# argumentcomputer/multi-stark

Hardware: AMD Instinct MI355X
Metric: prove_trace_rows_per_sec (higher is better)
Workload: dtype u64; 1 GPU; U32-add + byte-table lookup (benches/multi_stark.rs), 2^20 additions per proof, bench_config(): log_blowup 2, 100 queries, 10+10 PoW bits, GoldilocksBlake3Config; witness (traces + claims, 64-bit words) in pinned host memory at step start: upload, from_stage_1 on the device and read-back inside the timed region; the library narrows byte-valued traces on host threads INSIDE the step before they cro; rows_per_proof=1048832, proof_bytes=1100053, parallelism=single GPU

## Files before the change

bindings/rust/mstark_sys.rs:

```rust
#![allow(non_camel_case_types, dead_code)]

use std::os::raw::{c_char, c_void};

#[repr(C)] pub struct ms_ctx { _p: [u8; 0] }
#[repr(C)] pub struct ms_system { _p: [u8; 0] }
#[repr(C)] pub struct ms_witness { _p: [u8; 0] }
#[repr(C)] pub struct ms_mmcs { _p: [u8; 0] }
#[repr(C)] pub struct ms_challenger { _p: [u8; 0] }
#[repr(C)] pub struct ms_comm_rccl { _p: [u8; 0] }
#[repr(C)] pub struct ms_comm_local_group { _p: [u8; 0] }
#[repr(C)] pub struct ms_comm_local { _p: [u8; 0] }
#[repr(C)] pub struct ms_trace { _p: [u8; 0] }
#[repr(C)] pub struct msbb_system { _p: [u8; 0] }
#[repr(C)] pub struct msbb_witness { _p: [u8; 0] }
#[repr(C)] pub struct msbb_mmcs { _p: [u8; 0] }
#[repr(C)] pub struct msbb_challenger { _p: [u8; 0] }
#[repr(C)] pub struct msbb_trace { _p: [u8; 0] }

pub const MS_OK: i32 = 0;
pub const MS_ERR: i32 = -1;
pub const MS_ERR_NO_DEVICE: i32 = -2;
pub const MS_ERR_BUFFER: i32 = -3;
pub const MS_VERDICT_ACCEPT: i32 = 0;
pub const MS_VERDICT_INVALID_OPENING: i32 = 2;
pub const MS_VERDICT_INVALID_SHAPE: i32 = 3;
pub const MS_VERDICT_INVALID_SYSTEM: i32 = 4;
pub const MS_VERDICT_OOD_MISMATCH: i32 = 5;
pub const MS_VERDICT_UNBALANCED: i32 = 6;
pub const MS_CHECK_CONSTRAINT: u32 = 0x1;
pub const MS_CHECK_LOOKUPS: u32 = 0x2;
pub const MS_CHECK_CIRCUIT_WORDS: usize = 10;
pub const MS_LB_ENTRY_WORDS: usize = 8;
pub const MS_LB_CLAIMS: u64 = !0;
pub const MSBB_CHECK_CIRCUIT_WORDS: usize = 12;

#[repr(C)]
#[derive(Clone, Copy)]
pub struct ms_dev_matrix {
    pub ptr: *const c_void,
    pub height: u64,
    pub elem_bytes: u32,
    pub row_stride: i64,
    pub col_stride: i64,
}

#[repr(C)]
pub struct ms_comm {
    pub size: u32,
    pub rank: i32,
    pub world: i32,
    pub user: *mut c_void,
    pub all_to_all: Option<unsafe extern "C" fn(user: *mut c_void, send_dev: *const c_void, recv_dev: *mut c_void, bytes_per_peer: usize) -> i32>,
    pub all_gather: Option<unsafe extern "C" fn(user: *mut c_void, send_dev: *const c_void, recv_dev: *mut c_void, bytes: usize) -> i32>,
    pub all_to_all_start: Option<unsafe extern "C" fn(user: *mut c_void, send_dev: *const c_void, send_stride: usize, recv_dev: *mut c_void,
                                                      recv_stride: usize, bytes_per_peer: usize) -> i32>,
    pub all_to_all_wait: Option<unsafe extern "C" fn(user: *mut c_void) -> i32>,
    pub all_to_all_cols_start: Option<unsafe extern "C" fn(user: *mut c_void, send_dev: *const c_void, send_peer_stride: usize, send_col_stride: usize,
                                                           recv_dev: *mut c_void, recv_peer_stride: usize, recv_col_stride: usize, ncols: usize,
                                                           seg_bytes: usize) -> i32>,
    pub set_stream_ordered: Option<unsafe extern "C" fn(user: *mut c_void, hip_stream: *mut c_void) -> i32>,
    pub all_to_all_cols_start2: Option<unsafe extern "C" fn(user: *mut c_void, send_dev: *const c_void, send_peer_stride: usize, send_col_stride: usize,
                                                            recv_dev: *mut c_void, recv_peer_stride: usize, recv_col_stride: usize, ncols: usize,
                                                            seg_bytes: usize, flags: u32) -> i32>,
    pub scatter_cols_start: Option<unsafe extern "C" fn(user: *mut c_void, root: i32, send_dev: *const c_void, send_peer_stride: usize,
                                                        send_col_stride: usize, recv_dev: *mut c_void, recv_col_stride: usize, ncols: usize,
                                                        seg_bytes: usize) -> i32>,
    pub abort: Option<unsafe extern "C" fn(user: *mut c_void, why: *const c_char)>,
}
pub const MS_COMM_SKIP_SELF: u32 = 1;
pub const MS_KERNEL_QUOTIENT: u32 = 0x1;
pub const MS_KERNEL_QUOTIENT_INLINE: u32 = 0x2;
pub const MS_KERNEL_STAGE2: u32 = 0x4;
pub const MS_KERNEL_STAGE2_GROUPED: u32 = 0x8;
pub const MS_KERNEL_STAGE2_TRACE: u32 = 0x10;
pub const MS_KERNEL_STAGE2_GROUPS_SHIFT: u32 = 8;
pub const MS_KERNEL_STAGE2_GROUPS_MASK: u32 = 0x1f;

extern "C" {
    pub fn ms_last_error() -> *const c_char;
    pub fn ms_device_count() -> i32;
    pub fn ms_ctx_create(device: i32, out: *mut *mut ms_ctx) -> i32;
    pub fn ms_ctx_destroy(ctx: *mut ms_ctx);
    pub fn ms_ctx_sync(ctx: *mut ms_ctx) -> i32;
    pub fn ms_ctx_sync_count(ctx: *mut ms_ctx, out: *mut u64) -> i32;
    pub fn ms_ctx_trim(ctx: *mut ms_ctx) -> i32;
    pub fn ms_ctx_set_profile_mask(ctx: *mut ms_ctx, mask: u32) -> i32;
    pub fn ms_ctx_kernel_stats(ctx: *mut ms_ctx, kernel_id: i32, launches: *mut u64, ms: *mut f64, alg_bytes: *mut f64) -> i32;
    pub fn ms_ctx_reset_stats(ctx: *mut ms_ctx) -> i32;
    pub fn ms_ctx_kernel_units(ctx: *mut ms_ctx, kernel_id: i32, units: *mut f64) -> i32;
    pub fn ms_ctx_debug_fail_alloc(ctx: *mut ms_ctx, nth: i32) -> i32;
    pub fn ms_kernel_count() -> i32;
    pub fn ms_kernel_name(kernel_id: i32) -> *const c_char;
    pub fn ms_system_create(ctx: *mut ms_ctx, blob: *const u8, len: usize, out: *mut *mut ms_system) -> i32;
    pub fn ms_system_destroy(sys: *mut ms_system);
    pub fn ms_system_preprocessed_commit(sys: *const ms_system, out: *mut u8, cap: usize, n_digests: *mut usize) -> i32;
    pub fn ms_system_circuit_info(sys: *const ms_system, circuit: usize, out9: *mut u64) -> i32;
    pub fn ms_system_circuit_kernels(sys: *const ms_system, circuit: usize, flags: *mut u32) -> i32;
    pub fn ms_witness_create(sys: *mut ms_system, traces: *const *const u64, heights: *const u64, mult: *const *const u64,
                             args: *const *const u64, n_claims: usize, claim_offsets: *const u64, claim_data: *const u64,
                             out: *mut *mut ms_witness) -> i32;
    pub fn ms_witness_create_host(sys: *mut ms_system, traces: *const *const u64, heights: *const u64, n_claims: usize,
                                  claim_offsets: *const u64, claim_data: *const u64, pinned: *mut i32,
                                  out: *mut *mut ms_witness) -> i32;
    pub fn ms_claims_slice_range(sys: *mut ms_system, heights: *const u64, n_claims: usize, claim_offsets: *const u64, rank: i32, world: i32,
                                 first_elem: *mut u64, n_elems: *mut u64) -> i32;
    pub fn ms_witness_create_host_sliced(sys: *mut ms_system, traces: *const *const u64, heights: *const u64, n_claims: usize,
                                         claim_offsets: *const u64, data_first: u64, data_count: u64, data_slice: *const u64,
                                         head: *const u64, n_head: usize, pinned: *mut i32, out: *mut *mut ms_witness) -> i32;
    pub fn ms_witness_prefetch(w: *mut ms_witness, on: i32) -> i32;
    pub fn ms_witness_create_device(sys: *mut ms_system, traces: *const ms_dev_matrix, n_claims: usize, claim_offsets: *const u64,
                                    claim_data: *const u64, claims_on_device: i32, producer_stream: *mut c_void,
                                    out: *mut *mut ms_witness) -> i32;
    pub fn ms_witness_u32_add_bench(sys: *mut ms_system, num_adds: usize, a0: u32, b0: u32, out: *mut *mut ms_witness) -> i32;
    pub fn ms_witness_blake3_compressions(sys: *mut ms_system, n: usize, states_in: *const u32, states_out: *mut u32,
                                          out: *mut *mut ms_witness) -> i32;
    pub fn ms_blake3_compressions(data: *const u8, len: usize, states_in: *mut u32, cap_rows: usize, n: *mut usize, digest32: *mut u8) -> i32;
    pub fn ms_witness_trace(w: *mut ms_witness, circuit: usize, out: *mut u64, cap_words: usize, n_words: *mut usize) -> i32;
    pub fn ms_witness_destroy(w: *mut ms_witness);
    pub fn ms_prove(sys: *mut ms_system, w: *mut ms_witness, proof_out: *mut u8, cap: usize, proof_len: *mut usize, stage_ms: *mut f64) -> i32;
    pub fn ms_verify(sys: *mut ms_system, n_claims: usize, claim_offsets: *const u64, claim_data: *const u64, proof: *const u8,
                     proof_len: usize, verdict: *mut i32) -> i32;
    pub fn ms_verify_batch(sys: *mut ms_system, n_proofs: usize, n_claims: *const u64, claim_offsets: *const *const u64,
                           claim_data: *const *const u64, proofs: *const *const u8, proof_lens: *const u64, verdicts: *mut i32) -> i32;
    pub fn ms_prove_sharded(sys: *mut ms_system, w: *mut ms_witness, comm: *const ms_comm, owners: *const i32, proof_out: *mut u8,
                            cap: usize, proof_len: *mut usize, stage_ms: *mut f64) -> i32;
    pub fn ms_ctx_comm_progress(ctx: *mut ms_ctx, out: *mut c_char, cap: usize, seq: *mut u64, in_flight: *mut i32) -> i32;
    pub fn ms_comm_rccl_unique_id(out: *mut u8) -> i32;
    pub fn ms_comm_rccl_create(ctx: *mut ms_ctx, unique_id: *const u8, rank: i32, world: i32, out: *mut *mut ms_comm_rccl) -> i32;
    pub fn ms_comm_rccl_table(c: *mut ms_comm_rccl) -> *const ms_comm;
    pub fn ms_comm_rccl_bytes_moved(c: *mut ms_comm_rccl) -> u64;
    pub fn ms_comm_rccl_destroy(c: *mut ms_comm_rccl);
    pub fn ms_comm_local_group_create(world: i32, out: *mut *mut ms_comm_local_group) -> i32;
    pub fn ms_comm_local_group_abort(g: *mut ms_comm_local_group);
    pub fn ms_comm_local_group_destroy(g: *mut ms_comm_local_group);
    pub fn ms_comm_local_create(g: *mut ms_comm_local_group, ctx: *mut ms_ctx, rank: i32, out: *mut *mut ms_comm_local) -> i32;
    pub fn ms_comm_local_table(c: *mut ms_comm_local) -> *const ms_comm;
    pub fn ms_comm_local_bytes_moved(c: *mut ms_comm_local) -> u64;
    pub fn ms_comm_local_destroy(c: *mut ms_comm_local);
    pub fn ms_dft_batch(ctx: *mut ms_ctx, input: *const u64, h: usize, w: usize, inverse: i32, out: *mut u64) -> i32;
    pub fn ms_coset_lde_batch(ctx: *mut ms_ctx, input: *const u64, h: usize, w: usize, log_blowup: u32, out: *mut u64) -> i32;
    pub fn ms_quotient_lde(ctx: *mut ms_ctx, input: *const u64, log_n: u32, log_q: u32, log_blowup: u32, d: usize, out: *mut u64) -> i32;
    pub fn ms_mmcs_commit(ctx: *mut ms_ctx, n: usize, mats: *const *const u64, heights: *const u64, widths: *const u64, cap_height: u32,
                          cap_out: *mut u8, out: *mut *mut ms_mmcs) -> i32;
    pub fn ms_mmcs_open(m: *mut ms_mmcs, index: usize, vals_out: *mut u64, proof_out: *mut u8, n_siblings: *mut usize) -> i32;
    pub fn ms_mmcs_verify_batch(ctx: *mut ms_ctx, n_mats: usize, heights: *const u64, widths: *const u64, cap: *const u8, cap_height: u32,
                                n_openings: usize, indices: *const u64, vals: *const u64, siblings: *const u8, ok_out: *mut u8) -> i32;
    pub fn ms_mmcs_destroy(m: *mut ms_mmcs);
    pub fn ms_blake3(ctx: *mut ms_ctx, bytes: *const u8, len: usize, out32: *mut u8) -> i32;
    pub fn ms_challenger_create(params7: *const u64, out: *mut *mut ms_challenger) -> i32;
    pub fn ms_challenger_destroy(ch: *mut ms_challenger);
    pub fn ms_challenger_observe(ch: *mut ms_challenger, elems: *const u64, n: usize) -> i32;
    pub fn ms_challenger_observe_digests(ch: *mut ms_challenger, digests: *const u8, n: usize) -> i32;
    pub fn ms_challenger_sample_ext(ch: *mut ms_challenger, out2: *mut u64) -> i32;
    pub fn ms_challenger_sample_bits(ch: *mut ms_challenger, bits: u32, out: *mut u64) -> i32;
    pub fn ms_pcs_commit(ctx: *mut ms_ctx, log_blowup: u32, cap_height: u32, n: usize, evals: *const *const u64, heights: *const u64,
                         widths: *const u64, cap_out: *mut u8, out: *mut *mut ms_mmcs) -> i32;
    pub fn ms_pcs_open(ctx: *mut ms_ctx, params7: *const u64, n_rounds: usize, rounds: *const *mut ms_mmcs, n_points: *const u64,
                       points: *const u64, ch: *mut ms_challenger, opened_out: *mut u64, opened_cap_words: usize, fri_out: *mut u8,
                       fri_cap: usize, fri_len: *mut usize) -> i32;
    pub fn ms_pcs_verify(params7: *const u64, n_rounds: usize, caps: *const *const u8, cap_sizes: *const u64, n_mats: *const u64,
                         log_n: *const u64, widths: *const u64, n_points: *const u64, points: *const u64, opened: *const u64,
                         fri: *const u8, fri_len: usize, ch: *mut ms_challenger, accepted: *mut i32) -> i32;
    pub fn ms_trace_destroy(t: *mut ms_trace);
    pub fn ms_trace_info(t: *const ms_trace, out3: *mut u64) -> i32;
    pub fn ms_system_preprocessed_mmcs(sys: *mut ms_system, out: *mut *mut ms_mmcs) -> i32;
    pub fn ms_witness_commit_stage1(w: *mut ms_witness, cap_out: *mut u8, out: *mut *mut ms_mmcs) -> i32;
    pub fn ms_challenger_observe_claims(ch: *mut ms_challenger, w: *mut ms_witness) -> i32;
    pub fn ms_witness_check(w: *mut ms_witness, beta: *const u64, gamma: *const u64, verdict: *mut u32, circuits: *mut u64,
                            root_counts: *mut u64, root_first: *mut u64, roots_cap: usize) -> i32;
    pub fn ms_system_check_info(sys: *const ms_system, circuit: usize, out4: *mut u64) -> i32;
    pub fn ms_witness_lookup_balance(w: *mut ms_witness, summary: *mut u64, entries: *mut u64, entries_cap: usize, args_out: *mut u64,
                                     args_cap: usize, slot_counts: *mut u64, slots_cap: usize) -> i32;
    pub fn ms_witness_claims_accumulator(w: *mut ms_witness, beta: *const u64, gamma: *const u64, acc_out: *mut u64) -> i32;
    pub fn ms_stage2_build(w: *mut ms_witness, beta: *const u64, gamma: *const u64, acc_in: *const u64, accs_out: *mut u64,
                           traces_out: *mut *mut ms_trace) -> i32;
    pub fn ms_pcs_commit_traces(ctx: *mut ms_ctx, log_blowup: u32, cap_height: u32, n: usize, evals: *const *mut ms_trace,
                                cap_out: *mut u8, out: *mut *mut ms_mmcs) -> i32;
    pub fn ms_quotient(sys: *mut ms_system, circuit: usize, log_n: u32, s1: *mut ms_mmcs, s1_idx: usize, s2: *mut ms_mmcs,
                       s2_idx: usize, publics8: *const u64, alpha: *const u64, q_lde_out: *mut *mut ms_trace) -> i32;
    pub fn ms_pcs_commit_ldes(ctx: *mut ms_ctx, cap_height: u32, n: usize, ldes: *const *mut ms_trace, cap_out: *mut u8,
                              out: *mut *mut ms_mmcs) -> i32;
    pub fn ms_stage2_trace(ctx: *mut ms_ctx, height: usize, num_lookups: usize, mult: *const u64, arg_offsets: *const u64,
                           args: *const u64, beta: *const u64, gamma: *const u64, acc_in: *const u64, trace_out: *mut u64,
                           acc_out: *mut u64) -> i32;
    pub fn ms_claims_accumulator(ctx: *mut ms_ctx, n_claims: usize, claim_offsets: *const u64, claim_data: *const u64, beta: *const u64,
                                 gamma: *const u64, acc_out: *mut u64) -> i32;
    pub fn ms_quotient_values(sys: *mut ms_system, circuit: usize, publics8: *const u64, log_n: u32, log_q: u32, pre_q: *const u64,
                              s1_q: *const u64, s2_q: *const u64, alpha: *const u64, out: *mut u64) -> i32;
    pub fn ms_field_op(ctx: *mut ms_ctx, op: i32, a: *const u64, b: *const u64, n: usize, out: *mut u64) -> i32;

    pub fn msbb_system_create(ctx: *mut ms_ctx, blob: *const u8, len: usize, out: *mut *mut msbb_system) -> i32;
    pub fn msbb_system_destroy(sys: *mut msbb_system);
    pub fn msbb_system_preprocessed_commit(sys: *const msbb_system, out: *mut u32, cap_words: usize, n_digests: *mut usize) -> i32;
    pub fn msbb_system_circuit_info(sys: *const msbb_system, circuit: usize, out9: *mut u64) -> i32;
    pub fn msbb_system_circuit_kernels(sys: *const msbb_system, circuit: usize, flags: *mut u32) -> i32;
    pub fn msbb_witness_create(sys: *mut msbb_system, traces: *const *const u32, heights: *const u64, n_claims: usize,
                               claim_offsets: *const u64, claim_data: *const u32, out: *mut *mut msbb_witness) -> i32;
    pub fn msbb_witness_create_host(sys: *mut msbb_system, traces: *const *const u32, heights: *const u64, n_claims: usize,
                                    claim_offsets: *const u64, claim_data: *const u32, pinned: *mut i32, out: *mut *mut msbb_witness) -> i32;
    pub fn msbb_witness_create_device(sys: *mut msbb_system, traces: *const ms_dev_matrix, n_claims: usize, claim_offsets: *const u64,
                                      claim_data: *const u32, producer_stream: *mut c_void, out: *mut *mut msbb_witness) -> i32;
    pub fn msbb_witness_destroy(w: *mut msbb_witness);
    pub fn msbb_witness_check(w: *mut msbb_witness, beta: *const u32, gamma: *const u32, verdict: *mut u32, circuits: *mut u64,
                              root_counts: *mut u64, root_first: *mut u64, roots_cap: usize) -> i32;
    pub fn msbb_system_check_info(sys: *const msbb_system, circuit: usize, out4: *mut u64) -> i32;
    pub fn msbb_prove(sys: *mut msbb_system, w: *mut msbb_witness, proof_out: *mut u8, cap: usize, proof_len: *mut usize,
                      stage_ms: *mut f64) -> i32;
    pub fn msbb_verify(sys: *mut msbb_system, n_claims: usize, claim_offsets: *const u64, claim_data: *const u32, proof: *const u8,
                       proof_len: usize, verdict: *mut i32) -> i32;
    pub fn msbb_verify_batch(sys: *mut msbb_system, n_proofs: usize, n_claims: *const u64, claim_offsets: *const *const u64,
                             claim_data: *const *const u32, proofs: *const *const u8, proof_lens: *const u64, verdicts: *mut i32) -> i32;
    pub fn msbb_set_poseidon2(ctx: *mut ms_ctx, constants141: *const u32) -> i32;
    pub fn msbb_poseidon2_permute(ctx: *mut ms_ctx, states: *mut u32, n: usize) -> i32;
    pub fn msbb_dft_batch(ctx: *mut ms_ctx, input: *const u32, h: usize, w: usize, inverse: i32, out: *mut u32) -> i32;
    pub fn msbb_coset_lde_batch(ctx: *mut ms_ctx, input: *const u32, h: usize, w: usize, log_blowup: u32, out: *mut u32) -> i32;
    pub fn msbb_mmcs_commit(ctx: *mut ms_ctx, n: usize, mats: *const *const u32, heights: *const u64, widths: *const u64,
                            cap_height: u32, cap_out: *mut u32, out: *mut *mut msbb_mmcs) -> i32;
    pub fn msbb_mmcs_open(m: *mut msbb_mmcs, index: usize, vals_out: *mut u32, proof_out: *mut u32, n_siblings: *mut usize) -> i32;
    pub fn msbb_mmcs_verify_batch(ctx: *mut ms_ctx, n_mats: usize, heights: *const u64, widths: *const u64, cap: *const u32, cap_height: u32,
                                  n_openings: usize, indices: *const u64, vals: *const u32, siblings: *const u32, ok_out: *mut u8) -> i32;
    pub fn msbb_mmcs_destroy(m: *mut msbb_mmcs);
    pub fn msbb_field_op(ctx: *mut ms_ctx, op: i32, a: *const u32, b: *const u32, n: usize, out: *mut u32) -> i32;
    pub fn msbb_challenger_create(sys: *mut msbb_system, out: *mut *mut msbb_challenger) -> i32;
    pub fn msbb_challenger_destroy(ch: *mut msbb_challenger);
    pub fn msbb_challenger_observe(ch: *mut msbb_challenger, elems: *const u32, n: usize) -> i32;
    pub fn msbb_challenger_observe_digests(ch: *mut msbb_challenger, digests: *const u32, n: usize) -> i32;
    pub fn msbb_challenger_sample_ext(ch: *mut msbb_challenger, out4: *mut u32) -> i32;
    pub fn msbb_challenger_sample_bits(ch: *mut msbb_challenger, bits: u32, out: *mut u64) -> i32;
    pub fn msbb_challenger_observe_claims(ch: *mut msbb_challenger, w: *mut msbb_witness) -> i32;
    pub fn msbb_trace_destroy(t: *mut msbb_trace);
    pub fn msbb_trace_info(t: *const msbb_trace, out3: *mut u64) -> i32;
    pub fn msbb_system_preprocessed_mmcs(sys: *mut msbb_system, out: *mut *mut msbb_mmcs) -> i32;
    pub fn msbb_witness_commit_stage1(w: *mut msbb_witness, cap_out: *mut u32, out: *mut *mut msbb_mmcs) -> i32;
    pub fn msbb_witness_claims_accumulator(w: *mut msbb_witness, beta: *const u32, gamma: *const u32, acc_out: *mut u32) -> i32;
    pub fn msbb_stage2_build(w: *mut msbb_witness, beta: *const u32, gamma: *const u32, acc_in: *const u32, accs_out: *mut u32,
                             traces_out: *mut *mut msbb_trace) -> i32;
    pub fn msbb_pcs_commit_traces(sys: *mut msbb_system, n: usize, evals: *const *mut msbb_trace, cap_out: *mut u32, out: *mut *mut msbb_mmcs) -> i32;
    pub fn msbb_quotient(sys: *mut msbb_system, circuit: usize, log_n: u32, s1: *mut msbb_mmcs, s1_idx: usize, s2: *mut msbb_mmcs, s2_idx: usize,
                         publics16: *const u32, alpha: *const u32, q_lde_out: *mut *mut msbb_trace) -> i32;
    pub fn msbb_pcs_commit_ldes(sys: *mut msbb_system, n: usize, ldes: *const *mut msbb_trace, cap_out: *mut u32, out: *mut *mut msbb_mmcs) -> i32;
    pub fn msbb_pcs_open(sys: *mut msbb_system, n_rounds: usize, rounds: *const *mut msbb_mmcs, n_points: *const u64, points: *const u32,
                         ch: *mut msbb_challenger, opened_out: *mut u32, opened_cap_words: usize, fri_out: *mut u8, fri_cap: usize,
                         fri_len: *mut usize) -> i32;
}
```

include/mstark.h:

```cpp
#ifndef MSTARK_H
#define MSTARK_H

#include <stddef.h>
#include <stdint.h>

#ifdef __cplusplus
extern "C" {
#endif

typedef struct ms_ctx ms_ctx;
typedef struct ms_system ms_system;
typedef struct ms_witness ms_witness;
typedef struct ms_mmcs ms_mmcs;

enum {
  MS_OK = 0,
  MS_ERR = -1,
  MS_ERR_NO_DEVICE = -2,
  MS_ERR_BUFFER = -3
};

const char* ms_last_error(void);

int32_t ms_device_count(void);
int32_t ms_ctx_create(int32_t device, ms_ctx** out);
void ms_ctx_destroy(ms_ctx* ctx);
int32_t ms_ctx_sync(ms_ctx* ctx);
int32_t ms_ctx_sync_count(ms_ctx* ctx, uint64_t* out);
int32_t ms_ctx_trim(ms_ctx* ctx);
int32_t ms_ctx_set_profile_mask(ms_ctx* ctx, uint32_t mask);
int32_t ms_ctx_kernel_stats(ms_ctx* ctx, int32_t kernel_id, uint64_t* launches, double* ms, double* alg_bytes);
int32_t ms_ctx_kernel_units(ms_ctx* ctx, int32_t kernel_id, double* units);
int32_t ms_ctx_reset_stats(ms_ctx* ctx);
int32_t ms_ctx_debug_fail_alloc(ms_ctx* ctx, int32_t nth);
int32_t ms_kernel_count(void);
const char* ms_kernel_name(int32_t kernel_id);

int32_t ms_system_create(ms_ctx* ctx, const uint8_t* blob, size_t len, ms_system** out);
void ms_system_destroy(ms_system* sys);
int32_t ms_system_preprocessed_commit(const ms_system* sys, uint8_t* out, size_t cap, size_t* n_digests);
int32_t ms_system_circuit_info(const ms_system* sys, size_t circuit, uint64_t out9[9]);
#define MS_KERNEL_QUOTIENT 0x1u
#define MS_KERNEL_QUOTIENT_INLINE 0x2u
#define MS_KERNEL_STAGE2 0x4u
#define MS_KERNEL_STAGE2_GROUPED 0x8u
#define MS_KERNEL_STAGE2_TRACE 0x10u
#define MS_KERNEL_STAGE2_GROUPS_SHIFT 8
#define MS_KERNEL_STAGE2_GROUPS_MASK 0x1fu
int32_t ms_system_circuit_kernels(const ms_system* sys, size_t circuit, uint32_t* flags);

int32_t ms_witness_create(ms_system* sys, const uint64_t* const* traces, const uint64_t* heights,
                          const uint64_t* const* mult, const uint64_t* const* args, size_t n_claims,
                          const uint64_t* claim_offsets, const uint64_t* claim_data, ms_witness** out);
int32_t ms_witness_create_host(ms_system* sys, const uint64_t* const* traces, const uint64_t* heights, size_t n_claims,
                               const uint64_t* claim_offsets, const uint64_t* claim_data, int32_t* pinned ,
                               ms_witness** out);
int32_t ms_witness_prefetch(ms_witness* w, int32_t on);
typedef struct ms_dev_matrix {
  const void* ptr;
  uint64_t height;
  uint32_t elem_bytes;
  int64_t row_stride, col_stride;
} ms_dev_matrix;
int32_t ms_witness_create_device(ms_system* sys, const ms_dev_matrix* traces , size_t n_claims,
                                 const uint64_t* claim_offsets, const uint64_t* claim_data, int32_t claims_on_device,
                                 void* producer_stream , ms_witness** out);
int32_t ms_witness_u32_add_bench(ms_system* sys, size_t num_adds, uint32_t a0, uint32_t b0, ms_witness** out);
int32_t ms_witness_blake3_compressions(ms_system* sys, size_t n, const uint32_t* states_in, uint32_t* states_out, ms_witness** out);
int32_t ms_blake3_compressions(const uint8_t* data, size_t len, uint32_t* states_in, size_t cap_rows, size_t* n, uint8_t* digest32);
int32_t ms_witness_trace(ms_witness* w, size_t circuit, uint64_t* out, size_t cap_words, size_t* n_words);
void ms_witness_destroy(ms_witness* w);

#define MS_CHECK_CONSTRAINT 0x1u
#define MS_CHECK_LOOKUPS 0x2u
#define MS_CHECK_CIRCUIT_WORDS 10
int32_t ms_witness_check(ms_witness* w, const uint64_t beta[2], const uint64_t gamma[2], uint32_t* verdict,
                         uint64_t* circuits , uint64_t* root_counts ,
                         uint64_t* root_first , size_t roots_cap);
int32_t ms_system_check_info(const ms_system* sys, size_t circuit, uint64_t out4[4]);

#define MS_LB_ENTRY_WORDS 8
#define MS_LB_CLAIMS (~(uint64_t)0)
int32_t ms_witness_lookup_balance(ms_witness* w, uint64_t summary[4], uint64_t* entries, size_t entries_cap ,
                                  uint64_t* args_out, size_t args_cap , uint64_t* slot_counts ,
                                  size_t slots_cap);

int32_t ms_prove(ms_system* sys, ms_witness* w, uint8_t* proof_out, size_t cap, size_t* proof_len, double* stage_ms);

#define MS_VERDICT_ACCEPT 0
#define MS_VERDICT_INVALID_OPENING 2
#define MS_VERDICT_INVALID_SHAPE 3
#define MS_VERDICT_INVALID_SYSTEM 4
#define MS_VERDICT_OOD_MISMATCH 5
#define MS_VERDICT_UNBALANCED 6
int32_t ms_verify(ms_system* sys, size_t n_claims, const uint64_t* claim_offsets, const uint64_t* claim_data,
                  const uint8_t* proof, size_t proof_len, int32_t* verdict);
int32_t ms_verify_batch(ms_system* sys, size_t n_proofs, const uint64_t* n_claims, const uint64_t* const* claim_offsets,
                        const uint64_t* const* claim_data, const uint8_t* const* proofs, const uint64_t* proof_lens,
                        int32_t* verdicts);

typedef struct ms_comm {
  uint32_t size;
  int32_t rank, world;
  void* user;
  int32_t (*all_to_all)(void* user, const void* send_dev, void* recv_dev, size_t bytes_per_peer);
  int32_t (*all_gather)(void* user, const void* send_dev, void* recv_dev, size_t bytes);
  int32_t (*all_to_all_start)(void* user, const void* send_dev, size_t send_stride, void* recv_dev, size_t recv_stride,
                              size_t bytes_per_peer);
  int32_t (*all_to_all_wait)(void* user);
  int32_t (*all_to_all_cols_start)(void* user, const void* send_dev, size_t send_peer_stride, size_t send_col_stride, void* recv_dev,
                                   size_t recv_peer_stride, size_t recv_col_stride, size_t ncols, size_t seg_bytes);
  int32_t (*set_stream_ordered)(void* user, void* hip_stream);
  int32_t (*all_to_all_cols_start2)(void* user, const void* send_dev, size_t send_peer_stride, size_t send_col_stride, void* recv_dev,
                                    size_t recv_peer_stride, size_t recv_col_stride, size_t ncols, size_t seg_bytes, uint32_t flags);
  int32_t (*scatter_cols_start)(void* user, int32_t root, const void* send_dev, size_t send_peer_stride, size_t send_col_stride,
                                void* recv_dev, size_t recv_col_stride, size_t ncols, size_t seg_bytes);
  void (*abort)(void* user, const char* why);
} ms_comm;
#define MS_COMM_SKIP_SELF 1u
int32_t ms_prove_sharded(ms_system* sys, ms_witness* w, const ms_comm* comm, const int32_t* owners, uint8_t* proof_out, size_t cap,
                         size_t* proof_len, double* stage_ms);
int32_t ms_claims_slice_range(ms_system* sys, const uint64_t* heights, size_t n_claims, const uint64_t* claim_offsets, int32_t rank,
                              int32_t world, uint64_t* first_elem, uint64_t* n_elems);
int32_t ms_witness_create_host_sliced(ms_system* sys, const uint64_t* const* traces, const uint64_t* heights, size_t n_claims,
                                      const uint64_t* claim_offsets, uint64_t data_first, uint64_t data_count,
                                      const uint64_t* data_slice, const uint64_t* head, size_t n_head, int32_t* pinned,
                                      ms_witness** out);

int32_t ms_ctx_comm_progress(ms_ctx* ctx, char* out, size_t cap, uint64_t* seq, int32_t* in_flight);

#define MS_RCCL_UNIQUE_ID_BYTES 128
typedef struct ms_comm_rccl ms_comm_rccl;
int32_t ms_comm_rccl_unique_id(uint8_t out[MS_RCCL_UNIQUE_ID_BYTES]);
int32_t ms_comm_rccl_create(ms_ctx* ctx, const uint8_t unique_id[MS_RCCL_UNIQUE_ID_BYTES], int32_t rank, int32_t world,
                            ms_comm_rccl** out);
const ms_comm* ms_comm_rccl_table(ms_comm_rccl* c);
uint64_t ms_comm_rccl_bytes_moved(ms_comm_rccl* c);
void ms_comm_rccl_destroy(ms_comm_rccl* c);

typedef struct ms_comm_local_group ms_comm_local_group;
typedef struct ms_comm_local ms_comm_local;
int32_t ms_comm_local_group_create(int32_t world, ms_comm_local_group** out);
void ms_comm_local_group_abort(ms_comm_local_group* g);
void ms_comm_local_group_destroy(ms_comm_local_group* g);
int32_t ms_comm_local_create(ms_comm_local_group* g, ms_ctx* ctx, int32_t rank, ms_comm_local** out);
const ms_comm* ms_comm_local_table(ms_comm_local* c);
uint64_t ms_comm_local_bytes_moved(ms_comm_local* c);
void ms_comm_local_destroy(ms_comm_local* c);

int32_t ms_dft_batch(ms_ctx* ctx, const uint64_t* in, size_t h, size_t w, int32_t inverse, uint64_t* out);
int32_t ms_coset_lde_batch(ms_ctx* ctx, const uint64_t* in, size_t h, size_t w, uint32_t log_blowup, uint64_t* out);
int32_t ms_quotient_lde(ms_ctx* ctx, const uint64_t* in, uint32_t log_n, uint32_t log_q, uint32_t log_blowup, size_t D,
                        uint64_t* out);
int32_t ms_mmcs_commit(ms_ctx* ctx, size_t n, const uint64_t* const* mats, const uint64_t* heights,
                       const uint64_t* widths, uint32_t cap_height, uint8_t* cap_out, ms_mmcs** out);
int32_t ms_mmcs_open(ms_mmcs* m, size_t index, uint64_t* vals_out, uint8_t* proof_out, size_t* n_siblings);
void ms_mmcs_destroy(ms_mmcs* m);
int32_t ms_mmcs_verify_batch(ms_ctx* ctx, size_t n_mats, const uint64_t* heights, const uint64_t* widths, const uint8_t* cap,
                             uint32_t cap_height, size_t n_openings, const uint64_t* indices, const uint64_t* vals,
                             const uint8_t* siblings, uint8_t* ok_out);
int32_t ms_blake3(ms_ctx* ctx, const uint8_t* bytes, size_t len, uint8_t out32[32]);

typedef struct ms_challenger ms_challenger;
int32_t ms_challenger_create(const uint64_t params7[7], ms_challenger** out);
void ms_challenger_destroy(ms_challenger* ch);
int32_t ms_challenger_observe(ms_challenger* ch, const uint64_t* elems, size_t n);
int32_t ms_challenger_observe_digests(ms_challenger* ch, const uint8_t* digests, size_t n);
int32_t ms_challenger_sample_ext(ms_challenger* ch, uint64_t out2[2]);
int32_t ms_challenger_sample_bits(ms_challenger* ch, uint32_t bits, uint64_t* out);
int32_t ms_pcs_commit(ms_ctx* ctx, uint32_t log_blowup, uint32_t cap_height, size_t n, const uint64_t* const* evals,
                      const uint64_t* heights, const uint64_t* widths, uint8_t* cap_out, ms_mmcs** out);
int32_t ms_pcs_open(ms_ctx* ctx, const uint64_t params7[7], size_t n_rounds, ms_mmcs* const* rounds, const uint64_t* n_points,
                    const uint64_t* points, ms_challenger* ch, uint64_t* opened_out, size_t opened_cap_words, uint8_t* fri_out,
                    size_t fri_cap, size_t* fri_len);
int32_t ms_pcs_verify(const uint64_t params7[7], size_t n_rounds, const uint8_t* const* caps, const uint64_t* cap_sizes,
                      const uint64_t* n_mats, const uint64_t* log_n, const uint64_t* widths, const uint64_t* n_points,
                      const uint64_t* points, const uint64_t* opened, const uint8_t* fri, size_t fri_len, ms_challenger* ch,
                      int32_t* accepted);

typedef struct ms_trace ms_trace;
void ms_trace_destroy(ms_trace* t);
int32_t ms_trace_info(const ms_trace* t, uint64_t out3[3]);
int32_t ms_system_preprocessed_mmcs(ms_system* sys, ms_mmcs** out);
int32_t ms_witness_commit_stage1(ms_witness* w, uint8_t* cap_out, ms_mmcs** out);
int32_t ms_challenger_observe_claims(ms_challenger* ch, ms_witness* w);
int32_t ms_witness_claims_accumulator(ms_witness* w, const uint64_t beta[2], const uint64_t gamma[2], uint64_t acc_out[2]);
int32_t ms_stage2_build(ms_witness* w, const uint64_t beta[2], const uint64_t gamma[2], const uint64_t acc_in[2], uint64_t* accs_out,
                        ms_trace** traces_out);
int32_t ms_pcs_commit_traces(ms_ctx* ctx, uint32_t log_blowup, uint32_t cap_height, size_t n, ms_trace* const* evals, uint8_t* cap_out,
                             ms_mmcs** out);
int32_t ms_quotient(ms_system* sys, size_t circuit, uint32_t log_n, ms_mmcs* s1, size_t s1_idx, ms_mmcs* s2, size_t s2_idx,
                    const uint64_t publics8[8], const uint64_t alpha[2], ms_trace** q_lde_out);
int32_t ms_pcs_commit_ldes(ms_ctx* ctx, uint32_t cap_height, size_t n, ms_trace* const* ldes, uint8_t* cap_out, ms_mmcs** out);

int32_t ms_stage2_trace(ms_ctx* ctx, size_t height, size_t num_lookups, const uint64_t* mult,
                        const uint64_t* arg_offsets, const uint64_t* args, const uint64_t beta[2],
                        const uint64_t gamma[2], const uint64_t acc_in[2], uint64_t* trace_out, uint64_t acc_out[2]);
int32_t ms_claims_accumulator(ms_ctx* ctx, size_t n_claims, const uint64_t* claim_offsets, const uint64_t* claim_data,
                              const uint64_t beta[2], const uint64_t gamma[2], uint64_t acc_out[2]);
int32_t ms_quotient_values(ms_system* sys, size_t circuit, const uint64_t publics8[8], uint32_t log_n, uint32_t log_q,
                           const uint64_t* pre_q, const uint64_t* s1_q, const uint64_t* s2_q, const uint64_t alpha[2],
                           uint64_t* out);
int32_t ms_field_op(ms_ctx* ctx, int32_t op, const uint64_t* a, const uint64_t* b, size_t n, uint64_t* out);

#ifdef __cplusplus
}
#endif
#endif
```

multi-stark_amd/__init__.py:

```python
import ctypes as C
import os

import numpy as np

from . import frontend
from . import babybear
from .frontend import Params, bench_params, test_params, compile_circuit, system_blob, pack_claims

HERE = os.path.dirname(os.path.abspath(__file__))
LIB_PATH = os.path.join(HERE, "libmstark_hip.so")

u64p = C.POINTER(C.c_uint64)
u8p = C.POINTER(C.c_uint8)
_lib = None


class MstarkError(RuntimeError):
    pass


def lib():
    global _lib
    if _lib is None:
        if not os.path.exists(LIB_PATH):
            raise MstarkError("libmstark_hip.so is missing: run `python multi-stark_amd/build.py` (needs hipcc)")
        L = C.CDLL(LIB_PATH)
        L.ms_last_error.restype = C.c_char_p
        L.ms_kernel_name.restype = C.c_char_p
        _lib = L
    return _lib


def exported_symbols():
    return ["ms_last_error", "ms_device_count", "ms_ctx_create", "ms_ctx_destroy", "ms_ctx_sync", "ms_ctx_sync_count", "ms_ctx_trim", "ms_ctx_set_profile_mask",
            "ms_ctx_kernel_stats", "ms_ctx_kernel_units", "ms_ctx_reset_stats", "ms_ctx_debug_fail_alloc", "ms_kernel_count", "ms_kernel_name", "ms_system_create",
            "ms_system_destroy", "ms_system_preprocessed_commit", "ms_system_circuit_info", "ms_system_circuit_kernels", "ms_witness_create", "ms_witness_create_host", "ms_claims_slice_range", "ms_witness_create_host_sliced", "ms_witness_prefetch",
            "ms_witness_create_device", "ms_witness_u32_add_bench", "ms_witness_blake3_compressions", "ms_blake3_compressions", "ms_witness_trace", "ms_witness_destroy", "ms_prove", "ms_prove_sharded", "ms_ctx_comm_progress", "ms_comm_rccl_unique_id", "ms_comm_rccl_create",
            "ms_comm_rccl_table", "ms_comm_rccl_bytes_moved", "ms_comm_rccl_destroy", "ms_comm_local_group_create", "ms_comm_local_group_abort",
            "ms_comm_local_group_destroy", "ms_comm_local_create", "ms_comm_local_table", "ms_comm_local_bytes_moved", "ms_comm_local_destroy", "ms_verify", "ms_verify_batch", "ms_dft_batch", "ms_coset_lde_batch", "ms_quotient_lde", "ms_mmcs_commit",
            "ms_mmcs_open", "ms_mmcs_destroy", "ms_mmcs_verify_batch", "ms_blake3", "ms_pcs_commit", "ms_pcs_open", "ms_pcs_verify", "ms_challenger_create",
            "ms_challenger_destroy", "ms_challenger_observe", "ms_challenger_observe_digests", "ms_challenger_sample_ext",
            "ms_challenger_sample_bits", "ms_stage2_trace", "ms_claims_accumulator",
            "ms_quotient_values", "ms_field_op", "ms_trace_destroy", "ms_trace_info", "ms_system_preprocessed_mmcs",
            "ms_witness_commit_stage1", "ms_challenger_observe_claims", "ms_witness_claims_accumulator", "ms_stage2_build",
            "ms_pcs_commit_traces", "ms_quotient", "ms_pcs_commit_ldes", "ms_witness_check", "ms_system_check_info", "ms_witness_lookup_balance"]


KERNEL_QUOTIENT, KERNEL_QUOTIENT_INLINE, KERNEL_STAGE2, KERNEL_STAGE2_GROUPED, KERNEL_STAGE2_TRACE = 0x1, 0x2, 0x4, 0x8, 0x10


def kernel_groups(flags):
    return (flags >> 8) & 0x1F


def _check(rc):
    if rc != 0:
        raise MstarkError(lib().ms_last_error().decode() or ("mstark error %d" % rc))


def _p(a):
    return a.ctypes.data_as(u64p)


def _b(a):
    return a.ctypes.data_as(u8p)


def _u64(a):
    return np.ascontiguousarray(a, dtype=np.uint64)


class DevMatrix(C.Structure):
    _fields_ = [("ptr", C.c_void_p), ("height", C.c_uint64), ("elem_bytes", C.c_uint32), ("row_stride", C.c_int64), ("col_stride", C.c_int64)]


def _is_torch(obj):
    return type(obj).__module__.split(".")[0] == "torch" and hasattr(obj, "data_ptr")


def _device_array(obj, what):
    if _is_torch(obj):
        if not obj.is_cuda:
            raise MstarkError("%s: a CPU tensor has no device pointer (use System.witness)" % what)
        return int(obj.data_ptr()), tuple(int(x) for x in obj.shape), tuple(int(x) for x in obj.stride()), int(obj.element_size()), True
    cai = getattr(obj, "__cuda_array_interface__", None)
    if cai is None:
        raise MstarkError("%s: %s has no device pointer (expected a torch tensor on the GPU or __cuda_array_interface__)" % (what, type(obj).__name__))
    shape = tuple(int(x) for x in cai["shape"])
    item = np.dtype(cai["typestr"]).itemsize
    strides = cai.get("strides")
    if strides is None:
        strides, acc = [], item
        for n in reversed(shape):
            strides.insert(0, acc)
            acc *= max(n, 1)
    if any(int(b) % item for b in strides):
        raise MstarkError("%s: strides are not whole elements" % what)
    return int(cai["data"][0] or 0), shape, tuple(int(b) // item for b in strides), item, False


def _device_traces(traces, n_circuits, widths_of):
    if len(traces) != n_circuits:
        raise MstarkError("expected one trace per circuit")
    desc, seen_torch = [], None
    for i, t in enumerate(traces):
        what = "trace of circuit %d" % i
        if t is None or (not _is_torch(t) and not hasattr(t, "__cuda_array_interface__") and hasattr(t, "__len__") and len(t) == 0):
            desc.append(None)
            continue
        ptr, shape, strides, item, is_torch = _device_array(t, what)
        if len(shape) != 2:
            raise MstarkError("%s: expected a 2-D matrix, got %d dimension(s)" % (what, len(shape)))
        if is_torch and seen_torch is None:
            seen_torch = t
        desc.append((ptr, shape, strides, item))
    arr = (DevMatrix * max(n_circuits, 1))()
    heights = []
    for i, d in enumerate(desc):
        if d is None or d[1][0] == 0:
            arr[i] = DevMatrix(None, 0, 1, 1, 1)
            heights.append(0)
            continue
        ptr, (h, w), (rs, cs), item = d
        width = widths_of(i)
        if w != width:
            raise MstarkError("trace of circuit %d: width %d, the circuit's main_width is %d" % (i, w, width))
        arr[i] = DevMatrix(ptr or None, h, item, rs if h > 1 else max(w, 1), cs if w > 1 else 1)
        heights.append(h)
    return arr, heights, seen_torch


def _producer_stream(stream, torch_tensor):
    if stream is None:
        if torch_tensor is None:
            return None
        import torch

        stream = torch.cuda.current_stream(torch_tensor.device)
    handle = int(getattr(stream, "cuda_stream", stream))
    return C.c_void_p(handle) if handle else None


def device_count() -> int:
    return int(lib().ms_device_count())


class Context:

    def __init__(self, device=0):
        self.h = C.c_void_p()
        rc = lib().ms_ctx_create(C.c_int32(device), C.byref(self.h))
        if rc != 0:
            raise MstarkError("cannot create a HIP context: " + lib().ms_last_error().decode())

    def close(self):
        if getattr(self, "h", None):
            lib().ms_ctx_destroy(self.h)
            self.h = None

    def __del__(self):
        try:
            self.close()
        except Exception:
            pass

    def sync(self):
        _check(lib().ms_ctx_sync(self.h))

    def sync_count(self):
        n = C.c_uint64()
        _check(lib().ms_ctx_sync_count(self.h, C.byref(n)))
        return int(n.value)

    def trim(self):
        _check(lib().ms_ctx_trim(self.h))

    def comm_progress(self):
        buf = C.create_string_buffer(256)
        seq, fl = C.c_uint64(), C.c_int32()
        _check(lib().ms_ctx_comm_progress(self.h, buf, C.c_size_t(256), C.byref(seq), C.byref(fl)))
        return buf.value.decode(), int(seq.value), bool(fl.value)

    def debug_fail_alloc(self, nth):
        _check(lib().ms_ctx_debug_fail_alloc(self.h, C.c_int32(nth)))

    def kernel_names(self):
        return [lib().ms_kernel_name(C.c_int32(i)).decode() for i in range(lib().ms_kernel_count())]

    def set_profile(self, names):
        all_names = self.kernel_names()
        mask = 0
        for n in names:
            mask |= 1 << all_names.index(n)
        _check(lib().ms_ctx_set_profile_mask(self.h, C.c_uint32(mask)))

    def reset_stats(self):
        _check(lib().ms_ctx_reset_stats(self.h))

    def kernel_stats(self):
        out = {}
        for i, n in enumerate(self.kernel_names()):
            launches, ms, byts = C.c_uint64(), C.c_double(), C.c_double()
            _check(lib().ms_ctx_kernel_stats(self.h, C.c_int32(i), C.byref(launches), C.byref(ms), C.byref(byts)))
            units = C.c_double()
            _check(lib().ms_ctx_kernel_units(self.h, C.c_int32(i), C.byref(units)))
            out[n] = {"launches": launches.value, "ms": ms.value, "alg_bytes": byts.value, "units": units.value}
        return out

    def dft_batch(self, m, inverse=False):
        m = _u64(m)
        out = np.empty_like(m)
        _check(lib().ms_dft_batch(self.h, _p(m), C.c_size_t(m.shape[0]), C.c_size_t(m.shape[1]), C.c_int32(int(inverse)), _p(out)))
        return out

    def coset_lde_batch(self, m, log_blowup):
        m = _u64(m)
        out = np.empty((m.shape[0] << log_blowup, m.shape[1]), dtype=np.uint64)
        _check(lib().ms_coset_lde_batch(self.h, _p(m), C.c_size_t(m.shape[0]), C.c_size_t(m.shape[1]), C.c_uint32(log_blowup), _p(out)))
        return out

    def quotient_lde(self, q, log_n, log_q, log_blowup):
        q = _u64(q)
        D = q.shape[1]
        out = np.empty((1 << (log_n + log_blowup), D << log_q), dtype=np.uint64)
        _check(lib().ms_quotient_lde(self.h, _p(q), C.c_uint32(log_n), C.c_uint32(log_q), C.c_uint32(log_blowup), C.c_size_t(D), _p(out)))
        return out

    def blake3(self, data: bytes) -> bytes:
        buf = np.frombuffer(data, dtype=np.uint8) if data else np.zeros(1, dtype=np.uint8)
        out = np.zeros(32, dtype=np.uint8)
        _check(lib().ms_blake3(self.h, _b(buf), C.c_size_t(len(data)), _b(out)))
        return out.tobytes()

    def stage2_trace(self, mult, arg_offsets, args, beta, gamma, acc_in):
        mult, args, arg_offsets = _u64(mult), _u64(args), _u64(arg_offsets)
        h, L = mult.shape
        tr = np.zeros((h, max(L, 1) * 2), dtype=np.uint64)
        acc = np.zeros(2, dtype=np.uint64)
        _check(lib().ms_stage2_trace(self.h, C.c_size_t(h), C.c_size_t(L), _p(mult), _p(arg_offsets), _p(args), _p(_u64(beta)),
                                     _p(_u64(gamma)), _p(_u64(acc_in)), _p(tr), _p(acc)))
        return tr, (int(acc[0]), int(acc[1]))

    def claims_accumulator(self, claims_packed, beta, gamma):
        offs, data = claims_packed
        data = data if data.size else np.zeros(1, dtype=np.uint64)
        acc = np.zeros(2, dtype=np.uint64)
        _check(lib().ms_claims_accumulator(self.h, C.c_size_t(len(offs) - 1), _p(offs), _p(data), _p(_u64(beta)), _p(_u64(gamma)), _p(acc)))
        return int(acc[0]), int(acc[1])

    def field_op(self, op, a, b=None):
        a = _u64(a)
        bb = _u64(b) if b is not None else None
        out = np.empty_like(a)
        n = a.size // 2 if op >= 4 else a.size
        _check(lib().ms_field_op(self.h, C.c_int32(op), _p(a), _p(bb) if bb is not None else None, C.c_size_t(n), _p(out)))
        return out


class Mmcs:

    def __init__(self, ctx, mats, cap_height=0):
        self.ctx = ctx
        self.mats = [_u64(m) for m in mats]
        n = len(self.mats)
        ptrs = (u64p * n)(*[_p(m) for m in self.mats])
        hs = _u64([m.shape[0] for m in self.mats])
        ws = _u64([m.shape[1] for m in self.mats])
        maxh = int(hs.max())
        cap = np.zeros(32 * min(1 << cap_height, maxh), dtype=np.uint8)
        self.h = C.c_void_p()
        _check(lib().ms_mmcs_commit(ctx.h, C.c_size_t(n), ptrs, _p(hs), _p(ws), C.c_uint32(cap_height), _b(cap), C.byref(self.h)))
        self.cap = cap.tobytes()
        self.log_max = maxh.bit_length() - 1
        self.widths = ws

    def open(self, index):
        vals = np.zeros(int(self.widths.sum()), dtype=np.uint64)
        proof = np.zeros(32 * (self.log_max + 1), dtype=np.uint8)
        ns = C.c_size_t()
        _check(lib().ms_mmcs_open(self.h, C.c_size_t(index), _p(vals), _b(proof), C.byref(ns)))
        return vals, proof[: 32 * ns.value].tobytes()

    def verify_batch(self, indices, vals, siblings):
        hs = [m.shape[0] for m in self.mats]
        return mmcs_verify_batch(self.ctx, self.cap, len(self.cap) // 32, hs, self.widths, indices, vals, siblings)

    def __del__(self):
        if getattr(self, "h", None):
            lib().ms_mmcs_destroy(self.h)
            self.h = None


def mmcs_verify_batch(ctx, cap, cap_size, heights, widths, indices, vals, siblings):
    hs, ws = _u64(heights), _u64(widths)
    idx = _u64(indices)
    n = idx.size
    rw = int(ws.sum())
    cap_height = int(cap_size).bit_length() - 1
    if cap_size != 1 << cap_height or len(cap) != 32 * cap_size:
        raise MstarkError("a cap holds a power-of-two number of 32-byte digests")
    path = max(int(hs.max()).bit_length() - 1 - cap_height, 0) if hs.size else 0
    v = np.zeros(max(n * rw, 1), dtype=np.uint64)
    if n * rw:
        v[: n * rw] = np.concatenate([_u64(x).ravel() for x in vals]) if not isinstance(vals, np.ndarray) else _u64(vals).ravel()
    sib_bytes = b"".join(bytes(s) for s in siblings) if not isinstance(siblings, (bytes, bytearray, np.ndarray)) else bytes(siblings)
    if len(sib_bytes) != n * path * 32:
        raise MstarkError("expected %d sibling bytes per opening" % (path * 32))
    sib = np.frombuffer(sib_bytes + b"\0", dtype=np.uint8)
    capb = np.frombuffer(bytes(cap), dtype=np.uint8)
    ok = np.zeros(max(n, 1), dtype=np.uint8)
    _check(lib().ms_mmcs_verify_batch(ctx.h, C.c_size_t(hs.size), _p(hs), _p(ws), _b(capb), C.c_uint32(cap_height), C.c_size_t(n),
                                      _p(idx if n else np.zeros(1, dtype=np.uint64)), _p(v), _b(sib), _b(ok)))
    return ok[:n].copy()


class DeviceCommitment(Mmcs):

    def __init__(self, ctx, handle, cap: bytes, widths, log_max):
        self.ctx, self.h, self.cap = ctx, handle, cap
        self.widths = _u64(widths)
        self.log_max = log_max
        self.mats = []


class Trace:

    def __init__(self, handle):
        self.h = handle

    def info(self):
        o = np.zeros(3, dtype=np.uint64)
        _check(lib().ms_trace_info(self.h, _p(o)))
        return int(o[0]), int(o[1]), int(o[2])

    def __del__(self):
        if getattr(self, "h", None):
            lib().ms_trace_destroy(self.h)
            self.h = None


def _cap_buffer(cap_height, max_height):
    return np.zeros(32 * min(1 << cap_height, max_height), dtype=np.uint8)


def pcs_commit_traces(ctx, traces, log_blowup, cap_height=0):
    infos = [t.info() for t in traces]
    maxh = max(h for h, _, _ in infos) << log_blowup
    cap = _cap_buffer(cap_height, maxh)
    hs = (C.c_void_p * len(traces))(*[t.h for t in traces])
    out = C.c_void_p()
    _check(lib().ms_pcs_commit_traces(ctx.h, C.c_uint32(log_blowup), C.c_uint32(cap_height), C.c_size_t(len(traces)), hs, _b(cap), C.byref(out)))
    return DeviceCommitment(ctx, out, cap.tobytes(), [w for _, w, _ in infos], maxh.bit_length() - 1)


def pcs_commit_ldes(ctx, ldes, cap_height=0):
    infos = [t.info() for t in ldes]
    maxh = max(h for h, _, _ in infos)
    cap = _cap_buffer(cap_height, maxh)
    hs = (C.c_void_p * len(ldes))(*[t.h for t in ldes])
    out = C.c_void_p()
    _check(lib().ms_pcs_commit_ldes(ctx.h, C.c_uint32(cap_height), C.c_size_t(len(ldes)), hs, _b(cap), C.byref(out)))
    return DeviceCommitment(ctx, out, cap.tobytes(), [w for _, w, _ in infos], maxh.bit_length() - 1)


class PcsCommitment(Mmcs):

    def __init__(self, ctx, evals, log_blowup, cap_height=0):
        self.ctx = ctx
        self.mats = [_u64(m) for m in evals]
        n = len(self.mats)
        ptrs = (u64p * n)(*[_p(m) for m in self.mats])
        hs = _u64([m.shape[0] for m in self.mats])
        ws = _u64([m.shape[1] for m in self.mats])
        maxh = int(hs.max()) << log_blowup
        cap = np.zeros(32 * min(1 << cap_height, maxh), dtype=np.uint8)
        self.h = C.c_void_p()
        _check(lib().ms_pcs_commit(ctx.h, C.c_uint32(log_blowup), C.c_uint32(cap_height), C.c_size_t(n), ptrs, _p(hs), _p(ws), _b(cap),
                                   C.byref(self.h)))
        self.cap = cap.tobytes()
        self.log_max = maxh.bit_length() - 1
        self.widths = ws
        self.log_n = [int(h).bit_length() - 1 for h in hs]


class Challenger:

# ... 527 lines not shown
```

multi-stark_amd/csrc/capi.hip:

```cpp
#include <string>

#include "../../include/mstark.h"
#include "host.h"

using namespace msamd;

struct ms_ctx {
  Ctx ctx;
  int refs = 1;
  explicit ms_ctx(int dev) : ctx(dev) {}
};
static void ctx_unref(ms_ctx* c) {
  if (c && --c->refs == 0) delete c;
}
struct ms_system {
  ms_ctx* owner = nullptr;
  std::unique_ptr<HSystem> sys;
  int refs = 1;
};
static void system_unref(ms_system* s) {
  if (s && --s->refs == 0) {
    ms_ctx* c = s->owner;
    s->sys.reset();
    delete s;
// ... 820 lines not shown
  HIP_CHECK(hipSetDevice(ctx.device));
  need_device_witness(wit);
  const E2 beta_e = canonical_e2(beta, "beta"), gamma_e = canonical_e2(gamma, "gamma");
  E2 acc = canonical_e2(acc_in, "accumulator");
  size_t pos = 0;
  std::vector<std::unique_ptr<ms_trace, void (*)(ms_trace*)>> made;
  for (size_t ci = 0; ci < sys.circuits.size(); ci++) {
    const size_t n = wit.heights[ci];
    if (!n) continue;
    const HCircuit& c = sys.circuits[ci];
    DMat ev;
    ev.h = n;
    ev.w = c.stage2_width;
    ev.buf = DBuf<u64>(ctx, n * c.stage2_width);
    E2 tot;
    {
      DBuf<E2> d_tot(ctx, 1);
      stage2_circuit_async(ctx, sys, wit, ci, beta_e, gamma_e, ev.d(), d_tot.p);
      ctx.d2h(&tot, d_tot.p, sizeof(E2));
    }
    acc = e2_add(acc, tot);
    accs_out[2 * pos] = acc.c0;
    accs_out[2 * pos + 1] = acc.c1;
    made.emplace_back(new_trace(w->owner->owner, std::move(ev), log2_strict(n), 0), ms_trace_destroy);
    pos++;
  }
  for (size_t i = 0; i < made.size(); i++) traces_out[i] = made[i].release();
  return MS_OK;
  MS_CATCH
}

int32_t ms_pcs_commit_traces(ms_ctx* c, uint32_t log_blowup, uint32_t cap_height, size_t n, ms_trace* const* evals, uint8_t* cap_out,
                             ms_mmcs** out) {
  *out = nullptr;
  MS_TRY Ctx& ctx = c->ctx;
  HIP_CHECK(hipSetDevice(ctx.device));
  if (log_blowup < 1 || log_blowup > 8) throw std::runtime_error("log_blowup out of range");
  std::unique_ptr<ms_mmcs> m(new ms_mmcs());
  m->ctx = &ctx;
  std::vector<DMat> ldes;
  if (n == 0 || !evals) throw std::runtime_error("ms_pcs_commit_traces: no matrices");
  for (size_t i = 0; i < n; i++) {
    ms_trace* t = evals[i];
    if (!t || t->ctx != &ctx || t->kind != 0 || !t->m.d()) throw std::runtime_error("ms_pcs_commit_traces: not an evaluation handle of this context");
    if (t->log_n > NTT_MAX_LOG || t->log_n + log_blowup > TW_LOG) throw std::runtime_error("matrix too tall");
    for (size_t j = 0; j < i; j++)
      if (evals[j] == t) throw std::runtime_error("ms_pcs_commit_traces: the same handle twice");
  }
  for (size_t i = 0; i < n; i++) {
    ms_trace* t = evals[i];
    DMat lde;
    lde.h = t->m.h << log_blowup;
    lde.w = t->m.w;
    lde.buf = DBuf<u64>(ctx, lde.h * lde.w);
    coset_lde(ctx, t->m.d(), lde.d(), t->log_n, log_blowup, lde.w);
    t->m = DMat();
    ldes.push_back(std::move(lde));
  }
  commit_matrices(ctx, std::move(ldes), cap_height, m->data);
  std::vector<Digest> cap = merkle_cap(ctx, m->data.tree);
  for (size_t i = 0; i < cap.size(); i++) memcpy(cap_out + 32 * i, cap[i].b, 32);
  m->owner = c;
  c->refs++;
  *out = m.release();
  return MS_OK;
  MS_CATCH
}

int32_t ms_quotient(ms_system* sys, size_t ci, uint32_t log_n, ms_mmcs* s1, size_t s1_idx, ms_mmcs* s2, size_t s2_idx,
                    const uint64_t publics8[8], const uint64_t alpha[2], ms_trace** q_lde_out) {
  *q_lde_out = nullptr;
  MS_TRY HSystem& s = *sys->sys;
  Ctx& ctx = *s.ctx;
  HIP_CHECK(hipSetDevice(ctx.device));
  if (ci >= s.circuits.size()) throw std::runtime_error("circuit index out of range");
  const HCircuit& c = s.circuits[ci];
  const unsigned lb = (unsigned)s.params.log_blowup, log_q = log2_strict(c.quotient_degree());
  if (log_n > NTT_MAX_LOG || log_n + lb > TW_LOG) throw std::runtime_error("ms_quotient: log_n out of range");
  if (!s1 || !s2 || !publics8 || !alpha) throw std::runtime_error("ms_quotient: null argument");
  if (s1->ctx != &ctx || s2->ctx != &ctx) throw std::runtime_error("commitment belongs to another context");
  if (s1_idx >= s1->pd().ldes.size() || s2_idx >= s2->pd().ldes.size()) throw std::runtime_error("matrix index out of range");
  const DMat& m1 = s1->pd().ldes[s1_idx];
  const DMat& m2 = s2->pd().ldes[s2_idx];
  const size_t n = size_t(1) << log_n, nq = n << log_q;
  if (m1.h != (n << lb) || m2.h != (n << lb) || m1.w != c.main_width || m2.w != c.stage2_width)
    throw std::runtime_error("ms_quotient: the committed matrices do not have this circuit's shape");
  QuotientArgs qa;
  if (s.has_pre && s.pre_indices[ci] >= 0) {
    const DMat& pm = s.pre_data.ldes[s.pre_indices[ci]];
    if (pm.h != (n << lb)) throw std::runtime_error("main trace height must equal preprocessed trace height");
    qa.pre = pm.d();
    qa.pre_h = pm.h;
  }
  qa.s1 = m1.d();
  qa.s1_h = m1.h;
  qa.s2 = m2.d();
  qa.s2_h = m2.h;
  qa.log_n = log_n;
  qa.log_q = log_q;
  for (int k = 0; k < 8; k++) {
    if (publics8[k] >= GL_P) throw std::runtime_error("non-canonical public value");
    qa.publics[k] = publics8[k];
  }
  qa.alpha = canonical_e2(alpha, "alpha");
  DBuf<u64> qv(ctx, nq * 2);
  quotient_eval(ctx, c.prog, qa, qv.p);
  DMat lde;
  lde.h = n << lb;
  lde.w = 2 << log_q;
  lde.buf = DBuf<u64>(ctx, lde.h * lde.w);
  quotient_lde(ctx, qv.p, lde.d(), log_n, log_q, lb, 2);
  *q_lde_out = new_trace(sys->owner, std::move(lde), log_n, 1);
  return MS_OK;
  MS_CATCH
}

int32_t ms_pcs_commit_ldes(ms_ctx* c, uint32_t cap_height, size_t n, ms_trace* const* ldes, uint8_t* cap_out, ms_mmcs** out) {
  *out = nullptr;
  MS_TRY Ctx& ctx = c->ctx;
  HIP_CHECK(hipSetDevice(ctx.device));
  std::unique_ptr<ms_mmcs> m(new ms_mmcs());
  m->ctx = &ctx;
  std::vector<DMat> ms;
  for (size_t i = 0; i < n; i++) {
    ms_trace* t = ldes[i];
    if (!t || t->ctx != &ctx || t->kind != 1 || !t->m.d()) throw std::runtime_error("ms_pcs_commit_ldes: not an LDE handle of this context");
    ms.push_back(std::move(t->m));
    t->m = DMat();
  }
  commit_matrices(ctx, std::move(ms), cap_height, m->data);
  std::vector<Digest> cap = merkle_cap(ctx, m->data.tree);
  for (size_t i = 0; i < cap.size(); i++) memcpy(cap_out + 32 * i, cap[i].b, 32);
  m->owner = c;
  c->refs++;
  *out = m.release();
  return MS_OK;
  MS_CATCH
}

int32_t ms_blake3(ms_ctx* c, const uint8_t* bytes, size_t len, uint8_t out32[32]) {
  MS_TRY Ctx& ctx = c->ctx;
  HIP_CHECK(hipSetDevice(ctx.device));
  size_t pl = len & 7, nw = len >> 3;
  DBuf<uint8_t> pre(ctx, 8);
  DBuf<u64> words(ctx, std::max<size_t>(nw, 1));
  if (pl) ctx.h2d(pre.p, bytes, pl);
  if (nw) ctx.h2d(words.p, bytes + pl, nw * 8);
  Digest d = blake3_device(ctx, pre.p, pl, words.p, nw);
  memcpy(out32, d.b, 32);
  return MS_OK;
  MS_CATCH
}

int32_t ms_stage2_trace(ms_ctx* c, size_t height, size_t L, const uint64_t* mult, const uint64_t* arg_offsets,
                        const uint64_t* args, const uint64_t beta[2], const uint64_t gamma[2], const uint64_t acc_in[2],
                        uint64_t* trace_out, uint64_t acc_out[2]) {
  MS_TRY Ctx& ctx = c->ctx;
  HIP_CHECK(hipSetDevice(ctx.device));
  check_pow2(height);
  DLookups lk;
  lk.height = height;
  lk.num_lookups = L;
  std::vector<uint32_t> offs(L + 1);
  for (size_t i = 0; i <= L; i++) offs[i] = (uint32_t)arg_offsets[i];
  lk.args_width = offs[L];
  lk.arg_offsets = DBuf<uint32_t>(ctx, L + 1);
  ctx.h2d(lk.arg_offsets.p, offs.data(), (L + 1) * 4);
  lk.mult = DBuf<u64>(ctx, std::max<size_t>(height * L, 1));
  lk.args = DBuf<u64>(ctx, std::max<size_t>(height * lk.args_width, 1));
  if (L) ctx.h2d(lk.mult.p, mult, height * L * 8);
  if (lk.args_width) ctx.h2d(lk.args.p, args, height * lk.args_width * 8);
  size_t w2 = std::max<size_t>(L, 1) * 2;
  DBuf<u64> out(ctx, height * w2);
  E2 total = stage2_build(ctx, lk, e2(beta[0], beta[1]), e2(gamma[0], gamma[1]), out.p);
  E2 acc = e2_add(e2(acc_in[0], acc_in[1]), total);
  acc_out[0] = acc.c0;
  acc_out[1] = acc.c1;
  download_rowmajor(ctx, out.p, height, w2, true, trace_out);
  return MS_OK;
  MS_CATCH
}

int32_t ms_claims_accumulator(ms_ctx* c, size_t n_claims, const uint64_t* offs, const uint64_t* data, const uint64_t beta[2],
                              const uint64_t gamma[2], uint64_t acc_out[2]) {
  MS_TRY Ctx& ctx = c->ctx;
  HIP_CHECK(hipSetDevice(ctx.device));
  size_t tot = n_claims ? offs[n_claims] : 0;
  DBuf<u64> d_offs(ctx, n_claims + 1), d_data(ctx, std::max<size_t>(tot, 1));
  ctx.h2d(d_offs.p, offs, (n_claims + 1) * 8);
  if (tot) ctx.h2d(d_data.p, data, tot * 8);
  E2 a = claims_accumulator(ctx, d_data.p, d_offs.p, n_claims, e2(beta[0], beta[1]), e2(gamma[0], gamma[1]));
  acc_out[0] = a.c0;
  acc_out[1] = a.c1;
  return MS_OK;
  MS_CATCH
}

int32_t ms_quotient_values(ms_system* sys, size_t ci, const uint64_t publics8[8], uint32_t log_n, uint32_t log_q,
                           const uint64_t* pre_q, const uint64_t* s1_q, const uint64_t* s2_q, const uint64_t alpha[2],
                           uint64_t* out) {
  MS_TRY HSystem& s = *sys->sys;
  Ctx& ctx = *s.ctx;
  if (ci >= s.circuits.size()) throw std::runtime_error("circuit index out of range");
  const HCircuit& c = s.circuits[ci];
  size_t nq = size_t(1) << (log_n + log_q);
  DBuf<u64> pre, s1, s2;
  if (c.pre_width) pre = upload_colmajor(ctx, pre_q, nq, c.pre_width, true);
  s1 = upload_colmajor(ctx, s1_q, nq, c.main_width, true);
  s2 = upload_colmajor(ctx, s2_q, nq, c.stage2_width, true);
  QuotientArgs qa;
  qa.pre = pre.p;
  qa.s1 = s1.p;
  qa.s2 = s2.p;
  qa.pre_h = qa.s1_h = qa.s2_h = nq;
  qa.log_n = log_n;
  qa.log_q = log_q;
  memcpy(qa.publics, publics8, 64);
  qa.alpha = e2(alpha[0], alpha[1]);
  DBuf<u64> q(ctx, nq * 2);
  quotient_eval(ctx, c.prog, qa, q.p);
  download_rowmajor(ctx, q.p, nq, 2, true, out);
  return MS_OK;
  MS_CATCH
}

int32_t ms_field_op(ms_ctx* c, int32_t op, const uint64_t* a, const uint64_t* b, size_t n, uint64_t* out) {
  MS_TRY Ctx& ctx = c->ctx;
  HIP_CHECK(hipSetDevice(ctx.device));
  size_t words = op >= 4 ? 2 * n : n;
  DBuf<u64> da(ctx, words), db(ctx, words), dout(ctx, words);
  ctx.h2d(da.p, a, words * 8);
  if (b) ctx.h2d(db.p, b, words * 8);
  field_op(ctx, op, da.p, b ? db.p : da.p, n, dout.p);
  ctx.d2h(out, dout.p, words * 8);
  return MS_OK;
  MS_CATCH
}

}
```

multi-stark_amd/csrc/ctx.hip:

```cpp
#include <dlfcn.h>
#include <execinfo.h>
#include <signal.h>
#include <unistd.h>

#include <cstdlib>
#include <map>
#include <mutex>
#include <set>

#include "msamd.h"

namespace msamd {

namespace {
thread_local Ctx* tl_pending_ctx = nullptr;
std::mutex g_live_mu;
std::set<Ctx*> g_live;
}
namespace {
struct RoctxApi {
  int (*push)(const char*) = nullptr;
  int (*pop)() = nullptr;
  RoctxApi() {
    if (getenv("MSAMD_NO_ROCTX")) return;
// ... 263 lines not shown
  HIP_CHECK(hipMemset(tree_counter, 0, 256));
}

Ctx::~Ctx() {
  {
    std::lock_guard<std::mutex> lk(g_live_mu);
    g_live.erase(this);
  }
  (void)hipSetDevice(device);
  if (copy_stream) (void)hipStreamSynchronize(copy_stream);
  if (claims_stream) (void)hipStreamSynchronize(claims_stream);
  if (side_stream) (void)hipStreamSynchronize(side_stream);
  stream = main_stream;
  (void)hipStreamSynchronize(stream);
  for (auto& p : prof_pending) {
    (void)hipEventDestroy(p.a);
    (void)hipEventDestroy(p.b);
  }
  for (auto e : event_pool) (void)hipEventDestroy(e);
  for (auto& kv : pool_free) (void)hipFree(kv.second);
  for (auto& kv : pool_live) (void)hipFree(kv.first);
  for (auto& kv : pool_free_side) (void)hipFree(kv.second);
  for (auto& kv : side_live) (void)hipFree(kv.first);
  for (auto& kv : side_deferred) (void)hipFree(kv.second);
  for (auto e : side_ev)
    if (e) (void)hipEventDestroy(e);
  if (side_stream) (void)hipStreamDestroy(side_stream);
  for (auto& kv : lde_scales) (void)hipFree(kv.second);
  if (pinned) (void)hipHostFree(pinned);
  if (bounce) (void)hipHostFree(bounce);
  if (verify_stage) (void)hipHostFree(verify_stage);
  if (tw0) (void)hipFree(tw0);
  if (twc) (void)hipFree(twc);
  if (twf) (void)hipFree(twf);
  if (tree_counter) (void)hipFree(tree_counter);
  for (auto e : copy_ev)
    if (e) (void)hipEventDestroy(e);
  if (copy_stream) (void)hipStreamDestroy(copy_stream);
  if (claims_stream) (void)hipStreamDestroy(claims_stream);
  (void)hipStreamDestroy(stream);
}

void* Ctx::alloc(size_t bytes) {
  if (fail_alloc_countdown > 0 && --fail_alloc_countdown == 0) throw std::runtime_error("injected allocation failure (ms_ctx_debug_fail_alloc)");
  size_t sz = (bytes + 255) & ~size_t(255);
  if (sz == 0) sz = 256;
  const bool side = side_depth > 0;
  std::multimap<size_t, void*>& free_list = side ? pool_free_side : pool_free;
  auto it = free_list.find(sz);
  void* p = nullptr;
  if (it != free_list.end()) {
    p = it->second;
    free_list.erase(it);
  } else {
    hipError_t e = hipMalloc(&p, sz);
    if (e != hipSuccess) {
      (void)hipGetLastError();
      trim();
      HIP_CHECK(hipMalloc(&p, sz));
    }
    pool_bytes += sz;
  }
  if (side)
    side_live[p] = sz;
  else
    pool_live[p] = sz;
  return p;
}

void Ctx::release(void* p) {
  auto it = pool_live.find(p);
  if (it != pool_live.end()) {
    pool_free.emplace(it->second, p);
    pool_live.erase(it);
    return;
  }
  it = side_live.find(p);
  if (it == side_live.end()) return;
  if (side_forked)
    side_deferred.emplace_back(it->second, p);
  else
    pool_free_side.emplace(it->second, p);
  side_live.erase(it);
}

void Ctx::trim() {
  side_join();
  (void)hipStreamSynchronize(main_stream);
  for (auto& kv : pool_free) {
    (void)hipFree(kv.second);
    pool_bytes -= kv.first;
  }
  pool_free.clear();
  for (auto& kv : pool_free_side) {
    (void)hipFree(kv.second);
    pool_bytes -= kv.first;
  }
  pool_free_side.clear();
}

namespace {
__global__ void side_delay_k(unsigned long long ticks) {
  const unsigned long long t0 = wall_clock64();
  while (wall_clock64() - t0 < ticks) __builtin_amdgcn_s_sleep(32);
}
}

void Ctx::side_config() {
  side_enabled = !getenv("MSAMD_NO_SIDE_STREAM");
  const char* v = getenv("MSAMD_SIDE_MAX_LOG");
  side_max_log = v ? (unsigned)atoi(v) : 12u;
  if (side_max_log > 40) side_max_log = 40;
  const char* d = getenv("MSAMD_SIDE_DELAY_US");
  side_delay_us = d ? (unsigned)std::min(atoi(d), 20000) : 0u;
  d = getenv("MSAMD_MAIN_DELAY_US");
  main_delay_us = d ? (unsigned)std::min(atoi(d), 20000) : 0u;
  d = getenv("MSAMD_COPY_DELAY_US");
  copy_delay_us = d ? (unsigned)std::min(atoi(d), 20000) : 0u;
}

void Ctx::copy_delay() {
  if (!copy_delay_us) return;
  hipLaunchKernelGGL(side_delay_k, dim3(1), dim3(1), 0, copy_stream, (unsigned long long)copy_delay_us * 100ull);
  HIP_CHECK(hipGetLastError());
}

void Ctx::side_fork() {
  if (!side_enabled) return;
  if (side_forked) side_join();
  HIP_CHECK(hipEventRecord(side_ev[0], main_stream));
  HIP_CHECK(hipStreamWaitEvent(side_stream, side_ev[0], 0));
  side_forked = true;
  if (side_delay_us) {
    hipLaunchKernelGGL(side_delay_k, dim3(1), dim3(1), 0, side_stream, (unsigned long long)side_delay_us * 100ull);
    HIP_CHECK(hipGetLastError());
  }
  if (main_delay_us) {
    hipLaunchKernelGGL(side_delay_k, dim3(1), dim3(1), 0, main_stream, (unsigned long long)main_delay_us * 100ull);
    HIP_CHECK(hipGetLastError());
  }
}

void Ctx::side_join() {
  if (!side_forked) return;
  side_forked = false;
  hipError_t e = hipEventRecord(side_ev[1], side_stream);
  if (e == hipSuccess) e = hipStreamWaitEvent(main_stream, side_ev[1], 0);
  if (e != hipSuccess) {
    (void)hipGetLastError();
    (void)hipStreamSynchronize(side_stream);
  }
  for (auto& kv : side_deferred) pool_free_side.emplace(kv.first, kv.second);
  side_deferred.clear();
}

namespace {
struct FlagCopySeg {
  const uint8_t* src;
  uint32_t dst_off, n;
};
struct FlagCopyArgs {
  FlagCopySeg seg[24];
  uint32_t n_seg, seq;
  uint8_t* host_base;
  uint32_t* flag;
};
__global__ __launch_bounds__(256) void flag_copy_k(FlagCopyArgs a) {
  for (uint32_t s = 0; s < a.n_seg; s++) {
    const FlagCopySeg sg = a.seg[s];
    if (((sg.n | sg.dst_off) & 3u) == 0 && (reinterpret_cast<uintptr_t>(sg.src) & 3u) == 0) {
      const uint32_t* src = reinterpret_cast<const uint32_t*>(sg.src);
      uint32_t* dst = reinterpret_cast<uint32_t*>(a.host_base + sg.dst_off);
      for (uint32_t i = threadIdx.x; i < sg.n / 4; i += blockDim.x) dst[i] = src[i];
    } else {
      for (uint32_t i = threadIdx.x; i < sg.n; i += blockDim.x) a.host_base[sg.dst_off + i] = sg.src[i];
    }
  }
  __threadfence_system();
  __syncthreads();
  if (threadIdx.x == 0) __hip_atomic_store(a.flag, a.seq, __ATOMIC_RELEASE, __HIP_MEMORY_SCOPE_SYSTEM);
}
}

void Ctx::sync_and_deliver() {
  host_syncs++;
  side_join();
  hipStream_t stream = main_stream;
  bool done = false;
  size_t n_short = 0;
  for (auto& d : down_pending) n_short += d.copied ? 0 : 1;
  if (flag_host && !down_pending.empty() && n_short <= 24 && !down_direct && !getenv("MSAMD_NO_FLAG_SYNC")) {
    FlagCopyArgs a;
    memset(&a, 0, sizeof(a));
    size_t total = 0, k = 0;
    for (size_t i = 0; i < down_pending.size(); i++) {
      if (down_pending[i].copied) continue;
      a.seg[k].src = (const uint8_t*)down_pending[i].src;
      a.seg[k].dst_off = (uint32_t)down_pending[i].off;
      a.seg[k].n = (uint32_t)down_pending[i].n;
      total += down_pending[i].n;
      k++;
    }
    if (total <= (size_t(64) << 10)) {
      a.n_seg = (uint32_t)k;
      a.seq = ++flag_seq;
      a.host_base = pinned_dev + pinned_half;
      a.flag = flag_dev;
      hipLaunchKernelGGL(flag_copy_k, dim3(1), dim3(256), 0, stream, a);
      HIP_CHECK(hipGetLastError());
      volatile uint32_t* f = flag_host;
      for (uint64_t spins = 0;; spins++) {
        if (*f == a.seq) {
          done = true;
          break;
        }
        if ((spins & 0xFFFFF) == 0xFFFFF) {
          hipError_t q = hipStreamQuery(stream);
          if (q != hipErrorNotReady) {
            HIP_CHECK(q);
            done = *f == a.seq;
            break;
          }
        }
      }
      __atomic_thread_fence(__ATOMIC_ACQUIRE);
    }
  }
  if (!done) {
    for (auto& d : down_pending)
      if (!d.copied) HIP_CHECK(hipMemcpyAsync(pinned + pinned_half + d.off, d.src, d.n, hipMemcpyDeviceToHost, stream));
    HIP_CHECK(hipStreamSynchronize(stream));
  }
  for (auto& d : down_pending)
    if (d.dst) memcpy(d.dst, pinned + pinned_half + d.off, d.n);
  down_pending.clear();
  down_direct = false;
  down_used = 0;
  up_used = 0;
  if (side_depth > 0) side_fork();
}

void Ctx::bounce_h2d(void* dst, const void* src, size_t n, hipStream_t on) {
  hipStream_t s = on ? on : stream;
  if (!bounce) {
    HIP_CHECK(hipStreamSynchronize(s));
    HIP_CHECK(hipMemcpy(dst, src, n, hipMemcpyHostToDevice));
    return;
  }
  for (size_t off = 0; off < n; off += BOUNCE_BYTES) {
    const size_t m = std::min(BOUNCE_BYTES, n - off);
    memcpy(bounce, (const uint8_t*)src + off, m);
    HIP_CHECK(hipMemcpyAsync((uint8_t*)dst + off, bounce, m, hipMemcpyHostToDevice, s));
    HIP_CHECK(hipStreamSynchronize(s));
  }
}
void Ctx::bounce_d2h(void* dst, const void* src, size_t n) {
  if (!bounce) {
    HIP_CHECK(hipStreamSynchronize(stream));
    HIP_CHECK(hipMemcpy(dst, src, n, hipMemcpyDeviceToHost));
    return;
  }
  for (size_t off = 0; off < n; off += BOUNCE_BYTES) {
    const size_t m = std::min(BOUNCE_BYTES, n - off);
    HIP_CHECK(hipMemcpyAsync(bounce, (const uint8_t*)src + off, m, hipMemcpyDeviceToHost, stream));
    HIP_CHECK(hipStreamSynchronize(stream));
    memcpy((uint8_t*)dst + off, bounce, m);
  }
}

void Ctx::h2d(void* dst, const void* src, size_t n) {
  if (n == 0) return;
  if (pinned && n <= (size_t(1) << 20)) {
    size_t need = (n + 63) & ~size_t(63);
    if (up_used + need > pinned_half) sync_and_deliver();
    memcpy(pinned + up_used, src, n);
    HIP_CHECK(hipMemcpyAsync(dst, pinned + up_used, n, hipMemcpyHostToDevice, stream));
    up_used += need;
    return;
  }
  bounce_h2d(dst, src, n);
}

void Ctx::join_side_for_copy() {
  if (side_forked && side_depth == 0) {
    side_join();
    side_fork();
  }
}

void Ctx::d2h_queue(void* dst, const void* src, size_t n) {
  if (n == 0) return;
  size_t need = (n + 63) & ~size_t(63);
  if (!pinned || need > pinned_half) {
    join_side_for_copy();
    bounce_d2h(dst, src, n);
    return;
  }
  if (down_used + need > pinned_half) {
    bool view_pending = false;
    for (auto& d : down_pending) view_pending = view_pending || d.dst == nullptr;
    if (view_pending) {
      join_side_for_copy();
      bounce_d2h(dst, src, n);
      return;
    }
    sync_and_deliver();
// ... 89 lines not shown
```

multi-stark_amd/csrc/hash.hip:

```cpp
#include <algorithm>
#include <cstdlib>
#include <cstring>

#include "b3_dev.h"
#include "b3_quad.h"
#include "outer_dev.h"
#include "challenge_dev.h"
#include "fri_dev.h"
#include "msamd.h"
#include "tree_dev.h"

namespace msamd {

namespace {

struct RowIter {
  const MatRef* g;
  size_t H, row;
  unsigned mi;
  u32 c;
  const u64* cur;
  u32 w;
  size_t stride;
  __device__ __forceinline__ void init() {
// ... 373 lines not shown
};

template <bool INJ>
__device__ __forceinline__ void tree_level(u32* sh, u32 n, Digest* gout, const SubtreeParams& p, u32 glen, size_t gfirst) {
  const u32 t = threadIdx.x;
  if (INJ && p.inj_len == glen) {
    u32 d[8];
    const bool act = t < n;
    if (act) {
      u32 l[8], r[8], e[8], rh[8];
      lds_load_digest(sh, 2 * t, l);
      lds_load_digest(sh, 2 * t + 1, r);
      b3_compress_pair_root(l, r, e);
      if (p.inj_hashed)
        load_digest(p.inj_hashed + (gfirst + t), rh);
      else if (p.inj_multi)
        hash_row<true>(p.g, glen, gfirst + t, p.inj_w, rh);
      else
        hash_row<false>(p.g, glen, gfirst + t, p.inj_w, rh);
      b3_compress_pair_root(e, rh, d);
    }
    __syncthreads();
    if (act) {
      lds_store_digest(sh, t, d);
      store_digest(gout + t, d);
    }
    __syncthreads();
  } else {
    tree_level_plain(sh, n, gout);
  }
}

template <bool CH, bool INJ, bool FOLD>
__global__ __launch_bounds__(1024) void subtree_k(SubtreeParams p) {
  __shared__ __attribute__((aligned(16))) u32 sh[1024 * 8];
  __shared__ ChallengeShared cs;
  __shared__ u32 s_last;
  const u32 t = threadIdx.x, nb = gridDim.x;
  u32 b = blockIdx.x;
  Digest* lvl = p.child + p.len;
  u32 glen = p.len >> 1;
  u32 n;
  E2 hb = e2(0), rf = e2(0);
  if (FOLD) {
    const E2 beta = p.prev->beta;
    hb = e2_mul_base(beta, 0x7FFFFFFF80000001ULL);
    rf = e2_sqr(beta);
  }
  if (p.sub == 2048) {
    u32 l[8], r[8], d[8];
    const size_t c0 = size_t(b) * 2048 + 2 * t;
    if (FOLD) {
      u32 m[16];
      E2 o0 = fri_fold_one(p.fold, 2 * c0, hb, rf), o1 = fri_fold_one(p.fold, 2 * c0 + 1, hb, rf);
      p.fold.out[2 * c0] = o0;
      p.fold.out[2 * c0 + 1] = o1;
      fri_row_block(o0, o1, m);
      b3_iv(l);
      b3_compress(l, m, 0, 32, B3_CHUNK_START | B3_CHUNK_END | B3_ROOT);
      o0 = fri_fold_one(p.fold, 2 * c0 + 2, hb, rf);
      o1 = fri_fold_one(p.fold, 2 * c0 + 3, hb, rf);
      p.fold.out[2 * c0 + 2] = o0;
      p.fold.out[2 * c0 + 3] = o1;
      fri_row_block(o0, o1, m);
      b3_iv(r);
      b3_compress(r, m, 0, 32, B3_CHUNK_START | B3_CHUNK_END | B3_ROOT);
      store_digest(p.child + c0, l);
      store_digest(p.child + c0 + 1, r);
    } else {
      load_digest(p.child + c0, l);
      load_digest(p.child + c0 + 1, r);
    }
    b3_compress_pair_root(l, r, d);
    if (INJ && p.inj_len == glen) {
      u32 rh[8], e[8];
      if (p.inj_hashed)
        load_digest(p.inj_hashed + (size_t(b) * 1024 + t), rh);
      else if (p.inj_multi)
        hash_row<true>(p.g, glen, size_t(b) * 1024 + t, p.inj_w, rh);
      else
        hash_row<false>(p.g, glen, size_t(b) * 1024 + t, p.inj_w, rh);
      b3_compress_pair_root(d, rh, e);
#pragma unroll
      for (int k = 0; k < 8; k++) d[k] = e[k];
    }
    store_digest(lvl + size_t(b) * 1024 + t, d);
    lds_store_digest(sh, t, d);
    lvl += glen;
    glen >>= 1;
    n = 512;
  } else {
    if (t < p.sub) {
      u32 d[8];
      const size_t c0 = size_t(b) * p.sub + t;
      if (FOLD) {
        u32 m[16];
        const E2 o0 = fri_fold_one(p.fold, 2 * c0, hb, rf), o1 = fri_fold_one(p.fold, 2 * c0 + 1, hb, rf);
        p.fold.out[2 * c0] = o0;
        p.fold.out[2 * c0 + 1] = o1;
        fri_row_block(o0, o1, m);
        b3_iv(d);
        b3_compress(d, m, 0, 32, B3_CHUNK_START | B3_CHUNK_END | B3_ROOT);
        store_digest(p.child + c0, d);
      } else {
        load_digest(p.child + c0, d);
      }
      lds_store_digest(sh, t, d);
    }
    n = p.sub >> 1;
  }
  if (CH && t < 8) cs.st[t] = p.fc.state[t];
  __syncthreads();
#pragma unroll 1
  for (int phase = 0; phase < 2; phase++) {
    if (phase == 1) {
      if (nb == 1) break;
      Digest* roots = lvl - nb;
      if (t < 8) __hip_atomic_store(reinterpret_cast<u32*>(roots + b) + t, sh[t], __ATOMIC_RELAXED, __HIP_MEMORY_SCOPE_AGENT);
      asm volatile("s_waitcnt vmcnt(0)" ::: "memory");
      __syncthreads();
      if (t == 0) {
        const u32 ticket = __hip_atomic_fetch_add(p.counter, 1u, __ATOMIC_RELAXED, __HIP_MEMORY_SCOPE_AGENT);
        s_last = ticket == nb - 1 ? 1u : 0u;
      }
      __syncthreads();
      if (!s_last) return;
      const u32* rw = reinterpret_cast<const u32*>(roots);
      for (u32 i = t; i < nb * 8; i += 1024) sh[i] = __hip_atomic_load(rw + i, __ATOMIC_RELAXED, __HIP_MEMORY_SCOPE_AGENT);
      if (t == 0) __hip_atomic_store(p.counter, 0u, __ATOMIC_RELAXED, __HIP_MEMORY_SCOPE_AGENT);
      __syncthreads();
      b = 0;
      n = nb >> 1;
    }
#pragma unroll 1
    for (; n >= 1; n >>= 1) {
      tree_level<INJ>(sh, n, lvl + size_t(b) * n, p, glen, size_t(b) * n);
      lvl += glen;
      glen >>= 1;
    }
  }
  if (CH) {
    challenger_round<1024>(cs, sh, p.fc.pow_bits);
    if (t < 8) {
      p.fc.state[t] = cs.st[t];
      p.fc.rec->root[t] = sh[t];
    }
    if (t == 0) {
      p.fc.rec->witness = cs.wit;
      p.fc.rec->beta = cs.beta;
    }
  }
}

__device__ __forceinline__ u32 stream_byte(const uint8_t* __restrict__ prefix, size_t pl, const u64* __restrict__ words, size_t p) {
  if (p < pl) return prefix[p];
  size_t q = p - pl;
  return (u32)((words[q >> 3] >> (8 * (q & 7))) & 0xff);
}

__global__ __launch_bounds__(256) void chunk_cv_k(const uint8_t* __restrict__ prefix, size_t pl, const u64* __restrict__ words,
                                                  size_t len, size_t nchunks, size_t c0, size_t c1, Digest* out) {
  size_t ch = c0 + blockIdx.x * size_t(blockDim.x) + threadIdx.x;
  if (ch >= c1) return;
  size_t off = ch * 1024;
  size_t clen = len - off < 1024 ? len - off : 1024;
  u32 nblocks = clen == 0 ? 1 : (u32)((clen + 63) / 64);
  u32 cv[8];
  b3_iv(cv);
  const bool single = nchunks == 1;
  for (u32 b = 0; b < nblocks; b++) {
    u32 m[16];
    size_t boff = off + size_t(b) * 64;
    u32 bl = (u32)(clen - size_t(b) * 64 < 64 ? clen - size_t(b) * 64 : 64);
    if (bl == 64 && boff >= pl) {
      size_t q = boff - pl;
      const u64* w = words + (q >> 3);
      unsigned s = (unsigned)(q & 7) * 8;
      u64 cur = w[0];
#pragma unroll
      for (int k = 0; k < 8; k++) {
        u64 x;
        if (s == 0) {
          x = cur;
          if (k < 7) cur = w[k + 1];
        } else {
          u64 nxt = w[k + 1];
          x = (cur >> s) | (nxt << (64 - s));
          cur = nxt;
        }
        m[2 * k] = (u32)x;
        m[2 * k + 1] = (u32)(x >> 32);
      }
    } else {
#pragma unroll
      for (int i = 0; i < 16; i++) {
        u32 wv = 0;
        for (int k = 0; k < 4; k++) {
          u32 idx = 4 * i + k;
          u32 byte = idx < bl ? stream_byte(prefix, pl, words, boff + idx) : 0;
          wv |= byte << (8 * k);
        }
        m[i] = wv;
      }
    }
    u32 flags = (b == 0 ? B3_CHUNK_START : 0) | (b == nblocks - 1 ? (B3_CHUNK_END | (single ? B3_ROOT : 0)) : 0);
    b3_compress(cv, m, ch, bl, flags);
  }
  store_digest(out + ch, cv);
}

__global__ __launch_bounds__(64) void chunk_cv_prefix_k(const uint8_t* __restrict__ prefix, size_t pl, const u64* __restrict__ words,
                                                        size_t len, size_t nchunks, size_t c0, Digest* out) {
  __shared__ u32 sh[256];
  const size_t ch = c0 + blockIdx.x;
  const size_t off = ch * 1024;
  const size_t clen = len - off < 1024 ? len - off : 1024;
  for (u32 i = threadIdx.x; i < 256; i += 64) {
    u32 wv = 0;
#pragma unroll
    for (u32 k = 0; k < 4; k++) {
      const u32 idx = 4 * i + k;
      const u32 byte = idx < clen ? stream_byte(prefix, pl, words, off + idx) : 0;
      wv |= byte << (8 * k);
    }
    sh[i] = wv;
  }
  __syncthreads();
  if (threadIdx.x != 0) return;
  const u32 nblocks = clen == 0 ? 1 : (u32)((clen + 63) / 64);
  u32 cv[8];
  b3_iv(cv);
  const bool single = nchunks == 1;
  for (u32 b = 0; b < nblocks; b++) {
    u32 m[16];
#pragma unroll
    for (int i = 0; i < 16; i++) m[i] = sh[16 * b + i];
    const u32 bl = (u32)(clen - size_t(b) * 64 < 64 ? clen - size_t(b) * 64 : 64);
    const u32 flags = (b == 0 ? B3_CHUNK_START : 0) | (b == nblocks - 1 ? (B3_CHUNK_END | (single ? B3_ROOT : 0)) : 0);
    b3_compress(cv, m, ch, bl, flags);
  }
  store_digest(out + ch, cv);
}

__global__ __launch_bounds__(256) void cv_level_k(const Digest* __restrict__ prev, Digest* __restrict__ next, size_t n_prev,
                                                  u32 root_flag) {
  size_t n_next = (n_prev + 1) / 2;
  size_t i = blockIdx.x * size_t(blockDim.x) + threadIdx.x;
  if (i >= n_next) return;
  u32 l[8];
  load_digest(prev + 2 * i, l);
  if (2 * i + 1 < n_prev) {
    u32 r[8], o[8];
    load_digest(prev + 2 * i + 1, r);
    parent_cv(l, r, root_flag, o);
    store_digest(next + i, o);
  } else {
    store_digest(next + i, l);
  }
}

__global__ __launch_bounds__(1024) void cv_tail_k(const Digest* __restrict__ prev, Digest* __restrict__ out, u32 n, Digest* __restrict__ sib_out = nullptr) {
  __shared__ __attribute__((aligned(16))) u32 sh[2048 * 8];
  const u32 t = threadIdx.x;
  for (u32 i = t; i < n; i += 1024) {
    u32 d[8];
    load_digest(prev + i, d);
    lds_store_digest(sh, i, d);
  }
  __syncthreads();
  const u32 quad = t >> 2, c = t & 3;
  while (n > 1) {
    const u32 nn = (n + 1) / 2;
    const u32 flags = B3_PARENT | (n == 2 ? (u32)B3_ROOT : 0u);
    if (sib_out) {
      if (t < 8) reinterpret_cast<u32*>(sib_out)[t] = sh[8 + t];
      sib_out++;
    }
    u32 lo[4], hi[4];
#pragma unroll
    for (int ps = 0; ps < 4; ps++) {
      const u32 q = quad + 256 * ps;
      if (q < nn) {
        if (2 * q + 1 < n) {
          b3_quad_compress_iv<false>(sh + 16 * q, 64, flags, lo[ps], hi[ps]);
        } else {
          lo[ps] = sh[16 * q + c];
          hi[ps] = sh[16 * q + 4 + c];
        }
      }
    }
    __syncthreads();
#pragma unroll
    for (int ps = 0; ps < 4; ps++) {
      const u32 q = quad + 256 * ps;
      if (q < nn) {
        sh[8 * q + c] = lo[ps];
        sh[8 * q + 4 + c] = hi[ps];
      }
    }
    __syncthreads();
    n = nn;
  }
  if (t < 8) reinterpret_cast<u32*>(out)[t] = sh[t];
}

}

void merkle_alloc(Ctx& ctx, DTree& t, size_t maxh) {
  t.layer_off.clear();
  t.layer_len.clear();
  size_t tot = 0;
  for (size_t l = maxh;; l >>= 1) {
    t.layer_off.push_back(tot);
    t.layer_len.push_back(l);
    tot += l;
    if (l == 1) break;
  }
  t.digests = DBuf<Digest>(ctx, tot);
}

struct InjectAt {
  size_t first = 0;
  u32 total_w = 0;
  size_t count = 0;
};
static u32 subtree_children_per_group(size_t len) {
  if (len <= 1024) return (u32)len;
  size_t sub = len / 256;
  if (sub < 8) sub = 8;
  if (sub > 2048) sub = 2048;
  return (u32)sub;
}

static void build_levels(Ctx& ctx, DTree& t, const std::vector<InjectAt>& inj, const MatRef* drefs, const FriChallenge* fc = nullptr) {
  const size_t L = t.layer_len.size();
  size_t last_inject = 0;
  for (size_t li = 1; li < L; li++)
    if (inj[li].count) last_inject = li;
  size_t li = 1;
  const bool no_subtree = getenv("MSAMD_NO_SUBTREE") != nullptr;
  const char* sml = getenv("MSAMD_SUBTREE_MAX_LOG");
  const unsigned subtree_max_log = sml ? (unsigned)atoi(sml) : 20u;
  while (li < L) {
    const size_t child_len = t.layer_len[li - 1];
    Digest* child = t.base() + t.layer_off[li - 1];
    if (!no_subtree && child_len >= 2 && child_len <= (size_t(1) << std::min(subtree_max_log, 21u))) {
      size_t n_inj = 0, inj_li = 0;
      for (size_t k = li; k < L; k++)
        if (inj[k].count) {
          n_inj++;
          inj_li = k;
        }
      if (n_inj == 0 || (n_inj == 1 && !fc)) {
        SubtreeParams sp;
        memset(&sp, 0, sizeof(sp));
        sp.child = child;
        sp.len = (u32)child_len;
        sp.sub = subtree_children_per_group(child_len);
        sp.inj_len = n_inj ? (u32)t.layer_len[inj_li] : 0u;
        sp.g = n_inj ? drefs + inj[inj_li].first : nullptr;
        sp.inj_w = n_inj ? inj[inj_li].total_w : 0u;
        sp.inj_multi = n_inj && inj[inj_li].total_w > 128 ? 1u : 0u;
        DBuf<Digest> wide_cvs, wide_rows;
        if (sp.inj_multi && sp.inj_len <= 16384 && sp.inj_w >= 512 && !getenv("MSAMD_NO_WIDE_PREHASH")) {
          const size_t rows = sp.inj_len;
          const u32 nchunks = (sp.inj_w + 127) / 128;
          wide_cvs = DBuf<Digest>(ctx, rows * nchunks);
          wide_rows = DBuf<Digest>(ctx, rows);
          hipEvent_t evw = ctx.prof_begin(K_LEAF_HASH);
          hipLaunchKernelGGL(wide_rows_chunk_k, dim3((unsigned)((rows * nchunks + 255) / 256)), dim3(256), 0, ctx.stream, sp.g, rows, rows, sp.inj_w,
                             nchunks, wide_cvs.p);
          hipLaunchKernelGGL(wide_rows_merge_k, dim3((unsigned)((rows + 255) / 256)), dim3(256), 0, ctx.stream, wide_cvs.p, rows, nchunks, wide_rows.p);
          ctx.prof_end(K_LEAF_HASH, evw, 8.0 * sp.inj_w * rows);
          HIP_CHECK(hipGetLastError());
          sp.inj_hashed = wide_rows.p;
// ... 57 lines not shown
  }
  if (fc && L == 1 && li == 1) {
    hipLaunchKernelGGL(tree_tail_k<true>, dim3(1), dim3(1024), 0, ctx.stream, t.base(), 1u, *fc);
    fc = nullptr;
  }
  if (fc) throw std::runtime_error("build_levels: the tree never reached the single-workgroup tail");
  HIP_CHECK(hipGetLastError());
}

void merkle_top_challenge(Ctx& ctx, Digest* layer, size_t len, const FriChallenge& fc) {
  if (len < 2 || len > 1024 || (len & (len - 1))) throw std::runtime_error("merkle_top_challenge: 2 .. 1024 roots, a power of two");
  if (!fc.state || !fc.rec) throw std::runtime_error("merkle_top_challenge: challenger state missing");
  hipLaunchKernelGGL(tree_tail_k<true>, dim3(1), dim3(1024), 0, ctx.stream, layer, (u32)len, fc);
  HIP_CHECK(hipGetLastError());
}

void merkle_compress_plain(Ctx& ctx, DTree& t, const FriChallenge* fc) {
  std::vector<InjectAt> inj(t.layer_len.size());
  build_levels(ctx, t, inj, nullptr, fc);
}

bool fri_round_fusable(size_t rows) {
  const char* off = getenv("MSAMD_NO_FRI_FUSED");
  const char* ml = getenv("MSAMD_FRI_FUSED_MAX_LOG");
  const unsigned max_log = ml ? (unsigned)atoi(ml) : 21u;
  return !off && !getenv("MSAMD_NO_SUBTREE") && rows >= 4 && rows / 2 <= (size_t(1) << std::min(max_log, 21u));
}

void fri_round_fused(Ctx& ctx, DTree& t, const E2* cur, size_t rows, const FriTailRound* prev, const E2* roll_in, E2* out,
                     const FriChallenge& fc) {
  const size_t leaves = rows / 2;
  const unsigned lr = log2_strict(rows);
  if (lr + 1 > TW_LOG) throw std::runtime_error("FRI layer above 2^28 is not supported");
  if (!t.digests.p) merkle_alloc(ctx, t, leaves);
  SubtreeParams sp;
  memset(&sp, 0, sizeof(sp));
  sp.child = t.base();
  sp.len = (u32)leaves;
  sp.sub = subtree_children_per_group(leaves);
  sp.counter = tree_counter_slot(ctx);
  sp.fc = fc;
  sp.fold.cur = cur;
  sp.fold.roll = roll_in;
  sp.fold.out = out;
  sp.fold.t0i = ctx.tw0i;
  sp.fold.t1i = ctx.tw1i;
  sp.fold.log_rows = lr;
  sp.prev = prev;
  hipEvent_t ev = ctx.prof_begin(K_FRI_FOLD);
  hipLaunchKernelGGL((subtree_k<true, false, true>), dim3((unsigned)(leaves / sp.sub)), dim3(1024), 0, ctx.stream, sp);
  ctx.prof_end(K_FRI_FOLD, ev, 48.0 * rows + 64.0 * leaves);
  HIP_CHECK(hipGetLastError());
}

void merkle_build(Ctx& ctx, DTree& t) {
  size_t nm = t.mat_d.size();
  if (nm == 0) throw std::runtime_error("merkle_build: no matrices");
  std::vector<size_t> order(nm);
  for (size_t i = 0; i < nm; i++) {
    order[i] = i;
    if (t.mat_h[i] == 0 || (t.mat_h[i] & (t.mat_h[i] - 1))) throw std::runtime_error("merkle_build: heights must be powers of two");
    if (t.mat_w[i] == 0 || t.mat_w[i] > 0xFFFFFFFFu) throw std::runtime_error("merkle_build: bad width");
  }
  std::stable_sort(order.begin(), order.end(), [&](size_t a, size_t b) { return t.mat_h[a] > t.mat_h[b]; });
  size_t maxh = t.mat_h[order[0]];
  merkle_alloc(ctx, t, maxh);
  std::vector<MatRef> refs(nm);
  if (!t.mat_stride.empty() && t.mat_stride.size() != nm) throw std::runtime_error("merkle_build: one column stride per matrix expected");
  auto stride_of = [&](size_t i) { return t.mat_stride.empty() ? t.mat_h[i] : t.mat_stride[i]; };
  for (size_t k = 0; k < nm; k++) {
    if (stride_of(order[k]) < t.mat_h[order[k]]) throw std::runtime_error("merkle_build: column stride below the matrix height");
    refs[k] = MatRef{t.mat_d[order[k]], (uint32_t)t.mat_w[order[k]], 0, (uint64_t)stride_of(order[k])};
  }
  DBuf<MatRef> drefs(ctx, nm);
  ctx.h2d(drefs.p, refs.data(), nm * sizeof(MatRef));
  size_t pos = 0;
  auto take_group = [&](size_t height, size_t& first, u32& total_w, size_t& count) {
    first = pos;
    total_w = 0;
    count = 0;
    while (pos < nm && t.mat_h[order[pos]] == height) {
      total_w += (u32)t.mat_w[order[pos]];
      pos++;
      count++;
    }
  };
  size_t first, count;
  u32 tw;
  take_group(maxh, first, tw, count);
  {
    dim3 grid((unsigned)((maxh + 255) / 256));
    hipEvent_t ev = ctx.prof_begin(K_LEAF_HASH);
    if (tw <= 128 && count == 1 && !getenv("MSAMD_GENERIC_LEAF_HASH"))
      hipLaunchKernelGGL(leaf_hash_single_k, grid, dim3(256), 0, ctx.stream, t.mat_d[order[first]], maxh, stride_of(order[first]), tw, t.base());
    else if (tw <= 128)
      hipLaunchKernelGGL(leaf_hash_k<false>, grid, dim3(256), 0, ctx.stream, drefs.p + first, maxh, tw, t.base());
    else
      hipLaunchKernelGGL(leaf_hash_k<true>, grid, dim3(256), 0, ctx.stream, drefs.p + first, maxh, tw, t.base());
    ctx.prof_end(K_LEAF_HASH, ev, double(maxh) * (8.0 * tw + 32.0));
  }
  std::vector<InjectAt> inj(t.layer_len.size());
  for (size_t li = 1; li < t.layer_len.size(); li++) {
    take_group(t.layer_len[li], first, tw, count);
    inj[li].first = first;
    inj[li].total_w = tw;
    inj[li].count = count;
  }
  build_levels(ctx, t, inj, drefs.p);
  if (pos != nm) throw std::runtime_error("merkle_build: matrix height not reached");
  HIP_CHECK(hipGetLastError());
}

namespace {
__global__ __launch_bounds__(256) void tree_top_k(const Digest* __restrict__ roots, u32 n, Digest* __restrict__ out) {
  const u32 t = threadIdx.x;
  for (u32 i = t; i < n; i += blockDim.x) {
    u32 d[8];
    load_digest(roots + i, d);
    store_digest(out + i, d);
  }
  __syncthreads();
  u32 off = 0;
  for (u32 len = n; len > 1; len >>= 1) {
    for (u32 i = t; i < len / 2; i += blockDim.x) {
      u32 l[8], r[8], d[8];
      load_digest(out + off + 2 * i, l);
      load_digest(out + off + 2 * i + 1, r);
      b3_compress_pair_root(l, r, d);
      store_digest(out + off + len + i, d);
    }
    __syncthreads();
    off += len;
  }
}
}
void merkle_tree_top(Ctx& ctx, const Digest* d_roots, size_t n, Digest* d_out) {
  if (n == 0 || (n & (n - 1)) || n > (size_t(1) << 20)) throw std::runtime_error("merkle_tree_top: root count must be a power of two");
  hipLaunchKernelGGL(tree_top_k, dim3(1), dim3(256), 0, ctx.stream, d_roots, (u32)n, d_out);
  HIP_CHECK(hipGetLastError());
}

std::vector<Digest> merkle_cap(Ctx& ctx, const DTree& t) {
  size_t cl = t.cap_layer();
  std::vector<Digest> cap(t.layer_len[cl]);
  ctx.d2h(cap.data(), t.base() + t.layer_off[cl], cap.size() * sizeof(Digest));
  return cap;
}

size_t blake3_num_chunks(size_t prefix_len, size_t nwords) {
  size_t len = prefix_len + 8 * nwords;
  return len == 0 ? 1 : (len + 1023) / 1024;
}

void blake3_chunk_cvs(Ctx& ctx, const uint8_t* d_prefix, size_t prefix_len, const u64* d_words, size_t nwords, size_t c0, size_t c1,
                      Digest* cvs) {
  const size_t len = prefix_len + 8 * nwords, nchunks = blake3_num_chunks(prefix_len, nwords);
  if (c1 > nchunks) c1 = nchunks;
  if (c0 >= c1) return;
  const size_t pc = std::min(c1, (prefix_len + 1023) / 1024);
  if (c0 < pc) {
    hipLaunchKernelGGL(chunk_cv_prefix_k, dim3((unsigned)(pc - c0)), dim3(64), 0, ctx.stream, d_prefix, prefix_len, d_words, len, nchunks, c0, cvs);
    c0 = pc;
  }
  if (c0 < c1)
    hipLaunchKernelGGL(chunk_cv_k, dim3((unsigned)((c1 - c0 + 255) / 256)), dim3(256), 0, ctx.stream, d_prefix, prefix_len, d_words, len,
                       nchunks, c0, c1, cvs);
  HIP_CHECK(hipGetLastError());
}

struct ClaimsRootArgs {
  const uint8_t* prefix;
  const u64* words;
  size_t pl, len;
  const u32* cap;
  u32 cap_off, cap_bytes;
  const Digest* sib[32];
  u32 nchunks;
  Digest* out;
  ChallengeBG* bg;
  u32* state_out;
};
__global__ __launch_bounds__(64) void claims_root_k(ClaimsRootArgs a) {
  __shared__ u32 sh[256];
  __shared__ u32 pm[16];
  const u32 t = threadIdx.x, c = t & 3;
  const u32 clen = a.len < 1024 ? (u32)a.len : 1024u;
  for (u32 i = t; i < 256; i += 64) {
    u32 wv = 0;
#pragma unroll
    for (u32 k = 0; k < 4; k++) {
      const u32 idx = 4 * i + k;
      u32 byte = 0;
      if (idx < clen) {
        if (idx >= a.cap_off && idx - a.cap_off < a.cap_bytes) {
          const u32 q = idx - a.cap_off;
          byte = (a.cap[q >> 2] >> (8 * (q & 3))) & 0xff;
        } else {
          byte = stream_byte(a.prefix, a.pl, a.words, idx);
        }
      }
      wv |= byte << (8 * k);
    }
    sh[i] = wv;
  }
  __syncthreads();
  u32 lo = c == 0 ? B3_IV0 : c == 1 ? B3_IV1 : c == 2 ? B3_IV2 : B3_IV3;
  u32 hi = c == 0 ? B3_IV4 : c == 1 ? B3_IV5 : c == 2 ? B3_IV6 : B3_IV7;
  const u32 nblocks = (clen + 63) / 64;
  for (u32 b = 0; b < nblocks; b++) {
    const u32 bl = clen - 64 * b < 64 ? clen - 64 * b : 64;
    const u32 flags = (b == 0 ? (u32)B3_CHUNK_START : 0u) | (b == nblocks - 1 ? (u32)B3_CHUNK_END : 0u);
    b3_quad_compress_cv(sh + 16 * b, bl, flags, lo, hi);
  }
  for (u32 l = 0; (1u << l) < a.nchunks; l++) {
    if (t < 4) {
      pm[c] = lo;
      pm[4 + c] = hi;
    }
    if (t >= 8 && t < 16) pm[t] = reinterpret_cast<const u32*>(a.sib[l])[t - 8];
    __syncthreads();
    const bool last = (2u << l) >= a.nchunks;
    b3_quad_compress_iv<false>(pm, 64, B3_PARENT | (last ? (u32)B3_ROOT : 0u), lo, hi);
    __syncthreads();
  }
  if (t < 4) {
    u32* o = reinterpret_cast<u32*>(a.out);
    o[c] = lo;
    o[4 + c] = hi;
    pm[c] = lo;
    pm[4 + c] = hi;
  }
  if (a.bg) {
    __syncthreads();
    outer_beta_gamma_step(pm, a.bg, a.state_out);
  }
}

static const Digest* blake3_cv_tree(Ctx& ctx, Digest* cvs, size_t nchunks, DBuf<Digest>& scratch, Digest* out_dev) {
  scratch = DBuf<Digest>(ctx, (nchunks + 1) / 2);
  Digest* cur = cvs;
  Digest* nxt = scratch.p;
  size_t n = nchunks;
  while (n > 1) {
    if (n <= 2048) {
      hipLaunchKernelGGL(cv_tail_k, dim3(1), dim3(1024), 0, ctx.stream, (const Digest*)cur, nxt, (u32)n);
      std::swap(cur, nxt);
      break;
    }
    size_t nn = (n + 1) / 2;
    hipLaunchKernelGGL(cv_level_k, dim3((unsigned)((nn + 255) / 256)), dim3(256), 0, ctx.stream, cur, nxt, n,
                       n == 2 ? (u32)B3_ROOT : 0u);
    std::swap(cur, nxt);
    n = nn;
  }
  HIP_CHECK(hipGetLastError());
  if (out_dev) HIP_CHECK(hipMemcpyAsync(out_dev, cur, sizeof(Digest), hipMemcpyDeviceToDevice, ctx.stream));
  return cur;
}
Digest blake3_from_cvs(Ctx& ctx, Digest* cvs, size_t nchunks) {
  DBuf<Digest> b;
  const Digest* cur = blake3_cv_tree(ctx, cvs, nchunks, b, nullptr);
  Digest out;
  ctx.d2h(&out, cur, sizeof(Digest));
  return out;
}
void blake3_from_cvs_async(Ctx& ctx, Digest* cvs, size_t nchunks, Digest* out_dev) {
  DBuf<Digest> b;
  (void)blake3_cv_tree(ctx, cvs, nchunks, b, out_dev);
}

void blake3_late_chunk0_prepare(Ctx& ctx, const Digest* cvs, size_t nchunks, LateChunk0& lc) {
  if (nchunks < 2 || nchunks > (size_t(1) << 30)) throw std::runtime_error("blake3_late_chunk0: chunk count out of range");
  lc.levels = DBuf<Digest>(ctx, nchunks + 64);
  lc.sib.clear();
  const Digest* cur = cvs;
  Digest* nxt = lc.levels.p;
  size_t n = nchunks;
  while (n > 1) {
    if (n <= 2048) {
      Digest* tail_sib = nxt + 1;
      size_t m = n;
      while (m > 1) {
        lc.sib.push_back(tail_sib++);
        m = (m + 1) / 2;
      }
      hipLaunchKernelGGL(cv_tail_k, dim3(1), dim3(1024), 0, ctx.stream, cur, nxt, (u32)n, nxt + 1);
      break;
    }
    lc.sib.push_back(cur + 1);
    const size_t nn = (n + 1) / 2;
    hipLaunchKernelGGL(cv_level_k, dim3((unsigned)((nn + 255) / 256)), dim3(256), 0, ctx.stream, cur, nxt, n, 0u);
    cur = nxt;
    nxt += nn;
    n = nn;
  }
  HIP_CHECK(hipGetLastError());
  if (lc.sib.size() > 32) throw std::runtime_error("blake3_late_chunk0: too many levels");
}
void blake3_late_chunk0_finish(Ctx& ctx, const uint8_t* d_prefix, size_t prefix_len, const u64* d_words, size_t nwords, const Digest* d_cap,
                               size_t cap_off, size_t ncap, const LateChunk0& lc, size_t nchunks, Digest* out_dev, ChallengeBG* d_bg,
                               u32* d_state12) {
  if (prefix_len > 1024 || cap_off + 32 * ncap > prefix_len) throw std::runtime_error("blake3_late_chunk0: the prefix must lie inside chunk 0");
  ClaimsRootArgs a;
  memset(&a, 0, sizeof(a));
  a.prefix = d_prefix;
  a.words = d_words;
  a.pl = prefix_len;
  a.len = prefix_len + 8 * nwords;
  a.cap = reinterpret_cast<const u32*>(d_cap);
  a.cap_off = (u32)cap_off;
  a.cap_bytes = (u32)(32 * ncap);
  unsigned levels = 0;
  while ((size_t(1) << levels) < nchunks) levels++;
  if (lc.sib.size() != levels) throw std::runtime_error("blake3_late_chunk0: level count mismatch");
  for (unsigned l = 0; l < levels; l++) a.sib[l] = lc.sib[l];
  a.nchunks = (u32)nchunks;
  a.out = out_dev;
  a.bg = d_bg;
  a.state_out = d_state12;
  hipLaunchKernelGGL(claims_root_k, dim3(1), dim3(64), 0, ctx.stream, a);
  HIP_CHECK(hipGetLastError());
}

Digest blake3_device(Ctx& ctx, const uint8_t* d_prefix, size_t prefix_len, const u64* d_words, size_t nwords) {
  const size_t nchunks = blake3_num_chunks(prefix_len, nwords);
  DBuf<Digest> a(ctx, nchunks);
  blake3_chunk_cvs(ctx, d_prefix, prefix_len, d_words, nwords, 0, nchunks, a.p);
  return blake3_from_cvs(ctx, a.p, nchunks);
}

}
```

multi-stark_amd/csrc/msamd.h:

```cpp
#pragma once
#include <hip/hip_runtime.h>

#include <cstdint>
#include <cstring>
#include <map>
#include <mutex>
#include <stdexcept>
#include <string>
#include <vector>

#include "gl_dev.h"

namespace msamd {

#define HIP_CHECK(expr)                                                                                   \
  do {                                                                                                    \
    hipError_t _e = (expr);                                                                               \
    if (_e != hipSuccess)                                                                                 \
      throw std::runtime_error(std::string("HIP error: ") + hipGetErrorString(_e) + " at " + __FILE__ + ":" + \
                               std::to_string(__LINE__));                                                 \
  } while (0)

static constexpr unsigned TW_LOG = 28;
static constexpr unsigned TW_HALF = 14;
static constexpr unsigned NTT_MAX_LOG = 26;

struct Digest {
  uint8_t b[32];
};

enum KernelId : int {
  K_NTT_STRIDED = 0,
  K_NTT_CONTIG,
  K_NTT12_DIF,
  K_NTT12_DIT,
  K_NTT8S_DIF,
  K_NTT8S_DIT,
  K_LEAF_HASH,
  K_COMPRESS,
  K_STAGE2,
  K_QUOTIENT,
  K_BARY,
  K_DEEP,
  K_FRI_FOLD,
  K_TRANSPOSE,
  K_OTHER,
  K_WITNESS_CHECK,
  K_COUNT
};
const char* kernel_name(int id);

struct KernelStat {
  uint64_t launches = 0;
  double ms = 0;
  double alg_bytes = 0;
  double units = 0;
};

struct Ctx {
  int device = 0;
  hipStream_t stream = nullptr;
  hipStream_t copy_stream = nullptr;
  hipStream_t claims_stream = nullptr;
  hipStream_t main_stream = nullptr, side_stream = nullptr;
  hipEvent_t side_ev[2] = {nullptr, nullptr};
  bool side_forked = false;
  int side_depth = 0;
  bool side_enabled = true;
  unsigned side_max_log = 12;
  std::multimap<size_t, void*> pool_free_side;
  std::map<void*, size_t> side_live;
  std::vector<std::pair<size_t, void*>> side_deferred;
  void side_config();
  void side_fork();
  void side_join();
  unsigned side_delay_us = 0, main_delay_us = 0;
  unsigned copy_delay_us = 0;
  void copy_delay();
  void join_side_for_copy();
  hipEvent_t copy_ev[4] = {nullptr, nullptr, nullptr, nullptr};
  u64 *tw0 = nullptr, *tw1 = nullptr, *tw0i = nullptr, *tw1i = nullptr;
  u64 *twc = nullptr, *twci = nullptr;
  u64 *twc3 = nullptr, *twc3i = nullptr;
  u64 *twf = nullptr, *twfi = nullptr;
  u32* tree_counter = nullptr;
  std::multimap<size_t, void*> pool_free;
  std::map<void*, size_t> pool_live;
  size_t pool_bytes = 0;
  int fail_alloc_countdown = 0;
  uint8_t* pinned = nullptr;
  size_t pinned_half = 0, up_used = 0, down_used = 0;
  uint8_t* bounce = nullptr;
  static constexpr size_t BOUNCE_BYTES = size_t(4) << 20;
  uint8_t* verify_stage = nullptr;
  size_t verify_stage_cap = 0;
  void bounce_h2d(void* dst, const void* src, size_t n, hipStream_t on = nullptr);
  void bounce_d2h(void* dst, const void* src, size_t n);
  struct PendingD2H {
    void* dst;
    const void* src;
    size_t off, n;
    bool copied;
  };
  std::vector<PendingD2H> down_pending;
  bool down_direct = false;
  uint8_t* pinned_dev = nullptr;
  uint32_t *flag_host = nullptr, *flag_dev = nullptr;
  uint32_t flag_seq = 0;
  std::map<std::pair<unsigned, unsigned>, u64*> lde_scales;
  uint32_t prof_mask = 0;
  struct Pending {
    int id;
    hipEvent_t a, b;
    double bytes;
  };
  std::vector<Pending> prof_pending;
  std::vector<hipEvent_t> event_pool;
  KernelStat stats[K_COUNT];

  std::mutex comm_mu;
  std::string comm_what;
  uint64_t comm_seq = 0;
  uint64_t host_syncs = 0;
  bool comm_in_flight = false;

  explicit Ctx(int dev);
  ~Ctx();
  void* alloc(size_t bytes);
  void release(void* p);
  void trim();
  void sync() { sync_and_deliver(); }
  void sync_and_deliver();
  void h2d(void* dst, const void* src, size_t n);
  void d2h(void* dst, const void* src, size_t n);
  void d2h_queue(void* dst, const void* src, size_t n);
  const uint8_t* d2h_queue_staged(const void* src, size_t n);
  std::vector<uint8_t> host_scratch2;
  std::vector<uint8_t> host_scratch;
  const u64* lde_scale(unsigned log_n, unsigned log_blowup);
  bool prof_on(int id) const { return (prof_mask >> id) & 1u; }
  hipEvent_t prof_begin(int id);
  void prof_end(int id, hipEvent_t a, double bytes);
  void prof_collect();
};

inline u32* tree_counter_slot(Ctx& ctx) { return ctx.tree_counter + (ctx.side_depth > 0 ? 32 : 0); }

struct RoctxRange {
  bool on = false;
  explicit RoctxRange(const char* name);
  ~RoctxRange();
  void next(const char* name);
};

struct SideScope {
  Ctx& ctx;
  bool on;
  SideScope(Ctx& c, bool use) : ctx(c), on(use && c.side_forked) {
    if (on) {
      ctx.side_depth++;
      ctx.stream = ctx.side_stream;
    }
  }
  ~SideScope() {
    if (on && --ctx.side_depth == 0) ctx.stream = ctx.main_stream;
  }
};

int host_range_pin(const void* p, size_t bytes);
void host_range_unpin(const void* p);
void abandon_pending();

template <class T>
struct DBuf {
  Ctx* ctx = nullptr;
  T* p = nullptr;
  size_t n = 0;
  DBuf() {}
  DBuf(Ctx& c, size_t count) : ctx(&c), n(count) { p = count ? (T*)c.alloc(count * sizeof(T)) : nullptr; }
  DBuf(const DBuf&) = delete;
  DBuf& operator=(const DBuf&) = delete;
  DBuf(DBuf&& o) noexcept : ctx(o.ctx), p(o.p), n(o.n) { o.p = nullptr; }
  DBuf& operator=(DBuf&& o) noexcept {
    if (this != &o) {
      reset();
      ctx = o.ctx;
      p = o.p;
      n = o.n;
      o.p = nullptr;
    }
    return *this;
  }
  void reset() {
    if (p && ctx) ctx->release(p);
    p = nullptr;
  }
  ~DBuf() { reset(); }
};

struct DMat {
  DBuf<u64> buf;
  size_t h = 0, w = 0;
  u64* d() const { return buf.p; }
};

struct NttSrc {
  const u64* src = nullptr;
  unsigned src_div = 1;
  const u64* scale = nullptr;
};
void ntt_dif(Ctx& ctx, u64* data, unsigned logn, size_t ncols, bool inverse, const NttSrc* from = nullptr, u64 out_mul = 1);
void ntt_dit(Ctx& ctx, u64* data, unsigned logn, size_t ncols, bool inverse, u64 out_mul = 1);
void transpose_in(Ctx& ctx, const u64* rowmajor, u64* colmajor, size_t h, size_t w, bool bitrev_rows);
void transpose_out(Ctx& ctx, const u64* colmajor, u64* rowmajor, size_t h, size_t w, bool bitrev_rows);
void pull_widen_words(const uint8_t* host_packed, unsigned bytes, size_t count, u64* out, hipStream_t stream);
void lde_from_coeffs(Ctx& ctx, const u64* coef, u64* lde, unsigned logn, unsigned log_blowup, size_t w);
void coset_lde(Ctx& ctx, u64* evals_bitrev, u64* lde, unsigned logn, unsigned log_blowup, size_t w);
void quotient_lde(Ctx& ctx, u64* qvals_bitrev, u64* lde, unsigned logn, unsigned logq, unsigned log_blowup, size_t D);

struct MatRef {
  const u64* d;
  uint32_t w;
  uint32_t pad;
  uint64_t stride;
};
struct DTree {
  std::vector<const u64*> mat_d;
  std::vector<size_t> mat_h, mat_w;
  std::vector<size_t> mat_stride;
  DBuf<Digest> digests;
  Digest* ext = nullptr;
  Digest* base() const { return ext ? ext : digests.p; }
  std::vector<size_t> layer_off, layer_len;
  unsigned cap_height = 0;
  size_t max_height() const { return layer_len.empty() ? 0 : layer_len[0]; }
  size_t cap_layer() const {
    size_t L = layer_len.size();
    size_t ch = cap_height < L - 1 ? cap_height : L - 1;
    return L - 1 - ch;
  }
};
void merkle_build(Ctx& ctx, DTree& t);
void merkle_alloc(Ctx& ctx, DTree& t, size_t max_height);
struct FriChallenge;
void merkle_compress_plain(Ctx& ctx, DTree& t, const FriChallenge* fc = nullptr);
std::vector<Digest> merkle_cap(Ctx& ctx, const DTree& t);
void merkle_tree_top(Ctx& ctx, const Digest* d_roots, size_t n, Digest* d_out);
Digest blake3_device(Ctx& ctx, const uint8_t* d_prefix, size_t prefix_len, const u64* d_words, size_t nwords);
size_t blake3_num_chunks(size_t prefix_len, size_t nwords);
void blake3_chunk_cvs(Ctx& ctx, const uint8_t* d_prefix, size_t prefix_len, const u64* d_words, size_t nwords, size_t c0, size_t c1,
                      Digest* cvs);
Digest blake3_from_cvs(Ctx& ctx, Digest* cvs, size_t nchunks);
void blake3_from_cvs_async(Ctx& ctx, Digest* cvs, size_t nchunks, Digest* out_dev);
struct ChallengeBG;
struct LateChunk0 {
  DBuf<Digest> levels;
  std::vector<const Digest*> sib;
  void reset() {
    levels.reset();
    sib.clear();
  }
};
void blake3_late_chunk0_prepare(Ctx& ctx, const Digest* cvs, size_t nchunks, LateChunk0& lc);
void blake3_late_chunk0_finish(Ctx& ctx, const uint8_t* d_prefix, size_t prefix_len, const u64* d_words, size_t nwords, const Digest* d_cap,
                               size_t cap_off, size_t ncap, const LateChunk0& lc, size_t nchunks, Digest* out_dev,
                               ChallengeBG* d_bg = nullptr ,
                               u32* d_state12 = nullptr);

struct JitKernel;
struct DLookups {
  size_t height = 0, num_lookups = 0, args_width = 0;
  DBuf<u64> mult, args;
  DBuf<uint32_t> arg_offsets;
};
E2 stage2_build(Ctx& ctx, const DLookups& lk, E2 beta, E2 gamma, u64* out_colmajor_bitrev, const JitKernel* jit = nullptr);
void stage2_build_async(Ctx& ctx, const DLookups& lk, E2 beta, E2 gamma, u64* out_colmajor_bitrev, E2* total_dev,
                        const JitKernel* jit = nullptr);
struct ChallengeBG;
DBuf<ChallengeBG> challenge_bg_upload(Ctx& ctx, E2 beta, E2 gamma);
void stage2_build_dyn(Ctx& ctx, const DLookups& lk, const ChallengeBG* ch, u64* out_colmajor_bitrev, E2* total_dev, const JitKernel* jit = nullptr);
void stage2_from_trace_dyn(Ctx& ctx, const JitKernel& trace_jit, const u64* d_trace, const u64* d_pre, size_t n, size_t num_lookups,
                           size_t args_width, const ChallengeBG* ch, u64* out_colmajor_bitrev, E2* total_dev);
void claims_accumulator_dyn(Ctx& ctx, const u64* d_claim_data, const u64* d_claim_offsets, size_t n_claims, const ChallengeBG* ch, E2* out_dev);
void stage2_from_trace_async(Ctx& ctx, const JitKernel& trace_jit, const u64* d_trace, const u64* d_pre, size_t n, size_t num_lookups,
                             size_t args_width, E2 beta, E2 gamma, u64* out_colmajor_bitrev, E2* total_dev);
void claims_accumulator_async(Ctx& ctx, const u64* d_claim_data, const u64* d_claim_offsets, size_t n_claims, E2 beta, E2 gamma,
                              E2* out_dev);
E2 claims_accumulator(Ctx& ctx, const u64* d_claim_data, const u64* d_claim_offsets, size_t n_claims, E2 beta, E2 gamma);
size_t claims_transcript_words(Ctx& ctx, const u64* d_claim_data, const u64* d_claim_offsets, size_t n_claims,
                               size_t total_elems, u64* d_words);

void claims_transcript_words_slice(Ctx& ctx, const u64* d_data_abs, const u64* d_offs_first, size_t first, size_t count, size_t n_total,
                                   u64* d_words_abs);

struct JitKernel {
  void* module = nullptr;
  void* function = nullptr;
  bool inline_tables = false;
  unsigned groups = 0;
  JitKernel() {}
  JitKernel(const JitKernel&) = delete;
  JitKernel& operator=(const JitKernel&) = delete;
  JitKernel(JitKernel&& o) noexcept : module(o.module), function(o.function), inline_tables(o.inline_tables), groups(o.groups) {
    o.module = o.function = nullptr;
  }
  JitKernel& operator=(JitKernel&& o) noexcept {
    std::swap(module, o.module);
    std::swap(function, o.function);
    std::swap(inline_tables, o.inline_tables);
    std::swap(groups, o.groups);
    return *this;
  }
  ~JitKernel();
};
struct DProgram {
  JitKernel jit;
  DBuf<uint32_t> code;
  DBuf<u64> consts;
  size_t n_instr = 0, n_slots = 0;
  DBuf<uint32_t> zero_slots;
  DBuf<uint32_t> lookup_slots;
  size_t n_zeros = 0, n_lookups = 0, constraint_count = 0;
  size_t main_w = 0, pre_w = 0, s2_w = 0;
  DBuf<uint32_t> wave_code;
  DBuf<uint32_t> wave_zero_pos;
  DBuf<uint32_t> wave_lookups;
  DBuf<uint32_t> wave_lookup_off;
  size_t wave_steps = 0, wave_leaf_steps = 0;
};
struct QDyn;
struct QuotientArgs {
  const u64 *pre = nullptr, *s1 = nullptr, *s2 = nullptr;
  size_t pre_h = 0, s1_h = 0, s2_h = 0;
  unsigned log_n = 0, log_q = 0;
  u64 publics[8];
  E2 alpha;
  const QDyn* dyn = nullptr;
  const E2* alpha_rev = nullptr;
};
u64 quotient_inj_norm(unsigned log_n);

struct OuterTarget {
  QDyn* dyn;
  E2* alpha_rev;
  unsigned log_n;
  size_t k;
};
bool outer_fits(size_t ncap, size_t na);
void outer_beta_gamma(Ctx& ctx, const Digest* d_digest, ChallengeBG* d_bg, u32* d_state12);
void outer_alpha(Ctx& ctx, const u32* d_state12, const Digest* d_cap, size_t ncap, const E2* d_tot, size_t na, const ChallengeBG* d_bg,
                 const std::vector<OuterTarget>& targets, E2* d_accs, E2* d_alpha, u32* d_state8, DBuf<uint8_t>& keep);
void outer_zeta(Ctx& ctx, const u32* d_state8, const Digest* d_cap, size_t ncap, const u32* d_lds, size_t n_ld, E2* d_points,
                u32* d_state_out = nullptr );
void outer_joint_totals(Ctx& ctx, const E2* d_all, size_t world, size_t na, const std::vector<int>& src_rank, E2* d_tot);
void quotient_eval(Ctx& ctx, const DProgram& prog, const QuotientArgs& a, u64* out);

void inv_denoms(Ctx& ctx, E2 z, unsigned log_h, E2* out, E2* xout = nullptr, size_t n_x = 0);
void inv_denoms_rows(Ctx& ctx, E2 z, unsigned log_h, E2* out, E2* xout, size_t n_x, size_t row0, size_t rows);
void inv_denoms_rows_dev(Ctx& ctx, const E2* z_dev, unsigned log_h, E2* out, E2* xout, size_t n_x, size_t row0, size_t rows);
void inv_denoms_dev(Ctx& ctx, const E2* z_dev, unsigned log_h, E2* out, E2* xout = nullptr, size_t n_x = 0);
void bary_sums_async(Ctx& ctx, const u64* mat, size_t mat_h, size_t w, unsigned log_h, const E2* xden0, const E2* xden1,
                     int npoints, E2* out_dev, bool second_is_next = false);
struct BarySpec {
  const u64* mat;
  size_t mat_h, w;
  unsigned log_h;
  const E2 *xden0, *xden1;
  int npoints;
  E2* out_dev;
  bool second_is_next;
};
void bary_sums_batch(Ctx& ctx, const std::vector<BarySpec>& specs, DBuf<E2>& partial_keep);
void bary_finish(const E2* sums, size_t w, unsigned log_h, const E2* zs, int npoints, E2* out );
struct DeepMat {
  const u64* d;
  uint32_t w;
  uint32_t npoints;
  uint32_t pt[2];
  E2 coeff[2];
  uint64_t coeff7[2];
  uint64_t stride;
};
struct DeepPoints {
  uint32_t n;
  uint32_t pad;
  const E2* den[2];
  E2 K[2];
  uint32_t shift[2];
};
void deep_reduce(Ctx& ctx, const std::vector<DeepMat>& mats, const DeepPoints& pts, size_t height, const E2* alpha_pows_dev, E2* ro,
                 const E2* alpha_pows_host = nullptr, Digest* fri_leaves = nullptr ,
                 const DeepMat* mats_dev = nullptr ,
                 size_t row0 = 0, size_t full_height = 0 );
void fri_fold(Ctx& ctx, const E2* cur, size_t rows, E2 beta, const E2* roll_in , E2* out, size_t row0 = 0, size_t rows_total = 0);
static const unsigned FRI_MAX_LOG_ARITY = 6;
void fri_tree_build(Ctx& ctx, DTree& t, const E2* cur, size_t rows, const FriChallenge* fc = nullptr, unsigned log_arity = 1);
struct GatherReq {
  const void* base;
  uint64_t stride;
  uint64_t index;
  uint32_t count;
  uint32_t kind;
  uint64_t out_off;
};
void gather_rows(Ctx& ctx, const std::vector<GatherReq>& reqs, uint8_t* host_out, size_t out_bytes);
struct GatherSeg {
  const void* base;
  uint64_t stride;
  uint32_t count;
  uint32_t kind;
  uint32_t shift;
  uint32_t flip;
  uint64_t out_off;
};
void gather_queries(Ctx& ctx, const std::vector<GatherSeg>& segs, const std::vector<uint64_t>& indices, size_t bytes_per_query,
                    uint8_t* host_out);
void gather_queries_launch(Ctx& ctx, const std::vector<GatherSeg>& segs, GatherSeg* segs_dev, const u64* indices_dev, size_t n_queries,
                           size_t bytes_per_query, uint8_t* out_dev, unsigned owner_shift = 0, uint32_t owner = ~uint32_t(0));
void fri_query_challenge(Ctx& ctx, const uint32_t* state_dev, const E2* final_dev, unsigned pow_bits, uint32_t n_queries,
                         unsigned log_max_height, u64* out_dev);
// ... 29 lines not shown
```

multi-stark_amd/csrc/prover.hip:

```cpp
#include <algorithm>
#include <chrono>
#include <cstdio>
#include <cstdlib>

#include <sys/resource.h>
#include <unistd.h>

#include <atomic>
#include <condition_variable>
#include <functional>
#include <mutex>
#include <thread>

#include "host.h"
#include "ingest.h"
#include "lookup_params.h"
#include "open_plan.h"
#include "quotient_params.h"

namespace msamd {

namespace {
void load_block(const uint8_t* p, size_t len, u32 w[16]) {
  uint8_t buf[64];
// ... 685 lines not shown
        if (--busy_ == 0) done_cv_.notify_all();
      }
    }
  }
  std::vector<std::thread> threads_;
  std::mutex mu_, job_mu_;
  std::condition_variable cv_, done_cv_;
  uint64_t gen_ = 0;
  int busy_ = 0;
  const u64* in_ = nullptr;
  uint8_t* out_ = nullptr;
  unsigned pb_ = 1;
  size_t cnt_ = 0, per_chunk_ = 0, nsub_ = 1;
  std::atomic<uint8_t> state_[MAX_CHUNKS * MAX_SUB];
  std::thread::id caller_;
  unsigned straggle_us_ = 0;
  std::atomic<size_t> next_{0};
  std::atomic<u64> acc_{0};
  std::atomic<int> left_[MAX_CHUNKS];
};
}

void HWitness::pin(const void* p, size_t bytes) {
  if (!p || !bytes) return;
  const int r = host_range_pin(p, bytes);
  if (r == 1)
    registered.push_back(const_cast<void*>(p));
  else if (r == 0)
    pinned = false;
}
HWitness::~HWitness() {
  if (!host_resident) return;
  if (sys && sys->ctx) {
    (void)hipSetDevice(sys->ctx->device);
    (void)hipStreamSynchronize(sys->ctx->copy_stream);
    (void)hipStreamSynchronize(sys->ctx->claims_stream);
    if (sys->ctx->side_stream) (void)hipStreamSynchronize(sys->ctx->side_stream);
    (void)hipStreamSynchronize(sys->ctx->main_stream);
  }
  for (auto& st : stage)
    for (auto& e : st.ev)
      if (e) (void)hipEventDestroy(e);
  bool any_packed = false;
  for (uint8_t* p : h_packed) any_packed = any_packed || p != nullptr;
  if (any_packed)
    if (PackPool* pool = PackPool::get(sys && sys->ctx ? sys->ctx->device : 0)) pool->quiesce();
  for (void* p : registered) host_range_unpin(p);
  for (uint8_t* p : h_packed)
    if (p) (void)hipHostFree(p);
  (void)hipGetLastError();
}

std::unique_ptr<HWitness> witness_create_host(HSystem& sys, const u64* const* traces, const u64* heights, size_t n_claims,
                                              const u64* claim_offsets, const u64* claim_data, size_t data_first, size_t data_count,
                                              const u64* head, size_t n_head) {
  Ctx& ctx = *sys.ctx;
  HIP_CHECK(hipSetDevice(ctx.device));
  std::unique_ptr<HWitness> w(new HWitness());
  w->sys = &sys;
  w->host_resident = true;
  const size_t C = sys.circuits.size();
  w->traces.resize(C);
  w->lookups.resize(C);
  w->h_traces.assign(C, nullptr);
  w->h_mult.resize(C);
  w->h_args.resize(C);
  w->pack_bytes.assign(C, 0);
  w->h_packed.assign(C, nullptr);
  size_t pack_min = size_t(4) << 20;
  if (const char* e = getenv("MSAMD_PACK_MIN_BYTES")) pack_min = (size_t)atoll(e);
  const bool may_pack = !getenv("MSAMD_NO_PACK") && PackPool::get(ctx.device) != nullptr;
  for (size_t ci = 0; ci < C; ci++) {
    const HCircuit& c = sys.circuits[ci];
    const size_t h = heights[ci];
    w->heights.push_back(h);
    if (h == 0) continue;
    if (h & (h - 1)) throw std::runtime_error("trace height must be a power of two");
    if (log2_strict(h) > NTT_MAX_LOG || log2_strict(h) + sys.params.log_blowup > TW_LOG)
      throw std::runtime_error("trace height exceeds the supported maximum");
    if (c.pre_width && h != c.pre_height) throw std::runtime_error("main trace height must equal preprocessed trace height");
    if (!traces[ci]) {
      w->has_remote = true;
      continue;
    }
    const size_t cnt = h * c.main_width;
    u64 seen = 0;
    for (size_t i = 0; i < cnt; i++) {
      if (traces[ci][i] >= GL_P) throw std::runtime_error("non-canonical trace value");
      seen |= traces[ci][i];
    }
    w->h_traces[ci] = traces[ci];
    w->pin(traces[ci], cnt * 8);
    if (may_pack && cnt * 8 >= pack_min && (seen >> 32) == 0) {
      const unsigned pb = (seen >> 8) == 0 ? 1 : (seen >> 16) == 0 ? 2 : 4;
      void* hp = nullptr;
      if (hipHostMalloc(&hp, cnt * pb, hipHostMallocDefault) == hipSuccess) {
        w->pack_bytes[ci] = pb;
        w->h_packed[ci] = (uint8_t*)hp;
      } else {
        (void)hipGetLastError();
      }
    }
    DLookups& lk = w->lookups[ci];
    lk.height = h;
    lk.num_lookups = c.num_lookups;
    lk.args_width = c.args_width;
    if (c.num_lookups == 0) continue;
    std::vector<uint32_t> offs(1, 0);
    for (auto& l : c.lookups) offs.push_back(offs.back() + (uint32_t)l.second.size());
    lk.arg_offsets = DBuf<uint32_t>(ctx, offs.size());
    ctx.h2d(lk.arg_offsets.p, offs.data(), offs.size() * 4);
    unsigned threads = 64;
    const bool fits = c.prefix_on_device && c.prefix_prog.n_slots * threads * 8 <= 64 * 1024 && !getenv("MSAMD_HOST_LOOKUP_VALUES");
    if (!fits) {
      host_lookup_values(c, traces[ci], h, w->h_mult[ci], w->h_args[ci]);
      w->pin(w->h_mult[ci].data(), w->h_mult[ci].size() * 8);
      w->pin(w->h_args[ci].data(), w->h_args[ci].size() * 8);
    }
  }
  if (claim_offsets[0] != 0) throw std::runtime_error("claim offsets must start at 0");
  for (size_t i = 0; i < n_claims; i++)
    if (claim_offsets[i + 1] < claim_offsets[i]) throw std::runtime_error("claim offsets must be non-decreasing");
  const size_t tot = n_claims ? (size_t)claim_offsets[n_claims] : 0;
  w->claim_offsets.assign(claim_offsets, claim_offsets + n_claims + 1);
  w->claim_elems_total = tot;
  if (data_count == ~size_t(0)) {
    w->claim_data.assign(claim_data, claim_data + tot);
  } else {
    if (data_first > tot || data_count > tot - data_first) throw std::runtime_error("claims slice outside the claims' data");
    const size_t need_head = std::min<size_t>(tot, 130);
    if (n_head < need_head || (need_head && !head)) throw std::runtime_error("claims slice: the first 130 elements are needed on every rank");
    w->claims_partial = true;
    w->has_remote = true;
    w->claim_elem0 = data_first;
    w->claim_data.assign(claim_data, claim_data + data_count);
    w->claim_head.assign(head, head + need_head);
    for (u64 x : w->claim_head)
      if (x >= GL_P) throw std::runtime_error("non-canonical claim value");
  }
  for (u64 x : w->claim_data)
    if (x >= GL_P) throw std::runtime_error("non-canonical claim value");
  w->pin(w->claim_offsets.data(), (n_claims + 1) * 8);
  w->pin(w->claim_data.data(), w->claim_data.size() * 8);
  ctx.sync();
  return w;
}

namespace {
struct HostUpload {
  HWitness& w;
  Ctx& ctx;
  bool on = false;
  bool skip_claims = false;
  HostUpload(HWitness& wit, Ctx& c) : w(wit), ctx(c) {}
  bool fused(size_t ci) const {
    const HCircuit& c = w.sys->circuits[ci];
    return w.host_resident && c.stage2_trace_jit.function && w.h_mult[ci].empty();
  }
  void issue(HWitness::Staged& st) {
    HSystem& sys = *w.sys;
    const size_t C = sys.circuits.size();
    for (auto& e : st.ev)
      if (!e) HIP_CHECK(hipEventCreateWithFlags(&e, hipEventDisableTiming));
    st.clear();
    st.traces.resize(C);
    st.mult.resize(C);
    st.args.resize(C);
    HIP_CHECK(hipEventRecord(ctx.copy_ev[3], ctx.stream));
    HIP_CHECK(hipStreamWaitEvent(ctx.copy_stream, ctx.copy_ev[3], 0));
    ctx.side_config();
    ctx.copy_delay();
    HIP_CHECK(hipStreamWaitEvent(ctx.claims_stream, ctx.copy_ev[3], 0));
    const size_t n_claims = w.claim_offsets.size() - 1, tot = w.claim_data.size();
    auto from_caller = [&](void* dst, const void* src, size_t bytes, hipStream_t s) {
      if (w.pinned)
        HIP_CHECK(hipMemcpyAsync(dst, src, bytes, hipMemcpyHostToDevice, s));
      else
        ctx.bounce_h2d(dst, src, bytes, s);
    };
    for (size_t ci = 0; ci < C; ci++) {
      const HCircuit& c = sys.circuits[ci];
      const size_t h = w.heights[ci];
      if (!h || !w.h_traces[ci]) continue;
      const size_t cnt = h * c.main_width;
      st.traces[ci] = DBuf<u64>(ctx, cnt);
      const unsigned pb = w.pack_bytes[ci];
      PackPool* pool = pb && !w.prefetch ? PackPool::get(ctx.device) : nullptr;
      bool sent = false;
      if (pool) {
        static const size_t n_chunks = getenv("MSAMD_PACK_CHUNKS") ? (size_t)atoi(getenv("MSAMD_PACK_CHUNKS")) : 8;
        PackPool::Job job(*pool, w.h_traces[ci], w.h_packed[ci], pb, cnt, n_chunks);
        sent = true;
        for (size_t k = 0; k < pool->n_chunks; k++) {
          if (!pool->wait_chunk(k)) {
            sent = false;
            break;
          }
          if (k == 0) g_probes.mark("narrow upload: first chunk ready");
          const size_t b = pool->chunk_begin(k), e = pool->chunk_begin(k + 1);
          pull_widen_words(w.h_packed[ci] + b * pb, pb, e - b, st.traces[ci].p + b, ctx.copy_stream);
        }
        g_probes.mark("narrow upload: last chunk queued");
      }
      if (!sent) from_caller(st.traces[ci].p, w.h_traces[ci], cnt * 8, ctx.copy_stream);
    }
    HIP_CHECK(hipEventRecord(st.ev[0], ctx.copy_stream));
    st.has_host_lookups = false;
    for (size_t ci = 0; ci < C; ci++) {
      const HCircuit& c = sys.circuits[ci];
      const size_t h = w.heights[ci];
      if (!h || !c.num_lookups || !w.h_traces[ci]) continue;
      if (fused(ci)) continue;
      st.mult[ci] = DBuf<u64>(ctx, h * c.num_lookups);
      st.args[ci] = DBuf<u64>(ctx, std::max<size_t>(h * c.args_width, 1));
      if (!w.h_mult[ci].empty()) {
        st.has_host_lookups = true;
        from_caller(st.mult[ci].p, w.h_mult[ci].data(), w.h_mult[ci].size() * 8, ctx.copy_stream);
        if (!w.h_args[ci].empty()) from_caller(st.args[ci].p, w.h_args[ci].data(), w.h_args[ci].size() * 8, ctx.copy_stream);
      }
    }
    if (!skip_claims) {
      st.claim_offsets = DBuf<u64>(ctx, n_claims + 1);
      st.claim_data = DBuf<u64>(ctx, std::max<size_t>(tot, 1));
      from_caller(st.claim_offsets.p, w.claim_offsets.data(), (n_claims + 1) * 8, ctx.copy_stream);
      if (tot) from_caller(st.claim_data.p, w.claim_data.data(), tot * 8, ctx.copy_stream);
    }
    HIP_CHECK(hipEventRecord(st.ev[2], ctx.copy_stream));
    for (size_t ci = 0; ci < C; ci++) {
      const HCircuit& c = sys.circuits[ci];
      const size_t h = w.heights[ci];
      if (!h || !c.num_lookups || !w.h_mult[ci].empty() || fused(ci) || !w.h_traces[ci]) continue;
      if (!lookup_values_device(ctx, c.prefix_prog, st.traces[ci].p, c.pre_width ? c.d_preprocessed.p : nullptr, h, c.main_width, c.pre_width,
                                c.args_width, st.mult[ci].p, st.args[ci].p, ctx.copy_stream))
        throw std::runtime_error("host-resident witness: lookup prefix does not fit the device sweep");
    }
    HIP_CHECK(hipEventRecord(st.ev[1], ctx.copy_stream));
    st.valid = true;
  }
  void start() {
    if (!w.host_resident) return;
    on = true;
    if (w.prefetch && w.stage[w.cur ^ 1].valid)
      w.cur ^= 1;
    else
      issue(w.stage[w.cur]);
    HWitness::Staged& st = w.stage[w.cur];
    for (size_t ci = 0; ci < st.traces.size(); ci++) {
      w.traces[ci] = std::move(st.traces[ci]);
      w.lookups[ci].mult = std::move(st.mult[ci]);
      w.lookups[ci].args = std::move(st.args[ci]);
    }
    w.d_claim_offsets = std::move(st.claim_offsets);
    w.d_claim_data = std::move(st.claim_data);
    st.valid = false;
    if (w.prefetch) issue(w.stage[w.cur ^ 1]);
  }
  void wait_traces() {
    if (on) HIP_CHECK(hipStreamWaitEvent(ctx.stream, w.stage[w.cur].ev[0], 0));
  }
  void lookup_values() {
    if (!on) return;
    HIP_CHECK(hipStreamWaitEvent(ctx.stream, w.stage[w.cur].ev[1], 0));
    if (ctx.side_forked && ctx.stream != ctx.side_stream) HIP_CHECK(hipStreamWaitEvent(ctx.side_stream, w.stage[w.cur].ev[1], 0));
  }
  void wait_claims() {
    if (on) HIP_CHECK(hipStreamWaitEvent(ctx.stream, w.stage[w.cur].ev[2], 0));
  }
  ~HostUpload() {
    if (!on) return;
    (void)hipStreamSynchronize(ctx.copy_stream);
    (void)hipStreamSynchronize(ctx.claims_stream);
    for (auto& t : w.traces) t.reset();
    for (auto& lk : w.lookups) {
      lk.mult.reset();
      lk.args.reset();
    }
    w.d_claim_offsets.reset();
    w.d_claim_data.reset();
  }
};
}

namespace {
struct PW {
  std::vector<uint8_t> b;
  void u8(uint8_t x) { b.push_back(x); }
  void u64_(u64 x) {
    size_t o = b.size();
    b.resize(o + 8);
    memcpy(&b[o], &x, 8);
  }
  void ext(E2 e) {
    u64_(e.c0);
    u64_(e.c1);
  }
  void raw(const void* p, size_t n) {
    const uint8_t* q = (const uint8_t*)p;
    b.insert(b.end(), q, q + n);
  }
  void cap(const std::vector<Digest>& c) {
    u64_(c.size());
    for (auto& d : c) raw(d.b, 32);
  }
};
typedef std::vector<std::vector<std::vector<E2>>> OpenedRound;
void write_round(PW& w, const OpenedRound& r) {
  w.u64_(r.size());
  for (auto& m : r) {
    w.u64_(m.size());
    for (auto& pt : m) {
      w.u64_(pt.size());
      for (auto& e : pt) w.ext(e);
    }
  }
}

struct OpenRound {
  PcsData* data;
  std::vector<std::vector<E2>> points;
};

struct SymbolicPoints {
  const E2* d_points = nullptr;
  size_t n = 0;
  std::function<void(std::vector<E2>& values)> resolve;
  std::vector<int> next_log;
};

struct PhaseTrace {
  Ctx& ctx;
  bool on;
  double t;
  explicit PhaseTrace(Ctx& c) : ctx(c), on(getenv("MSAMD_TRACE") != nullptr), t(0) {
    if (on) {
      ctx.sync();
      t = now_ms();
    }
  }
  void mark(const char* what) {
    if (!on) return;
    ctx.sync();
    double n = now_ms();
    fprintf(stderr, "[msamd] %-22s %8.3f ms\n", what, n - t);
    t = n;
  }
};

u64 grind(Ctx& ctx, Challenger& ch, unsigned bits) {
  if (bits == 0) return 0;
  u64 w = 0;
  if (bits >= 4 && grind_device(ctx, ch.input, bits, &w)) {
    ch.observe(w);
    if (ch.sample_bits(bits) != 0) throw std::runtime_error("grind: device witness rejected by the host challenger");
    return w;
  }
  return ch.grind(bits);
}

struct InputShape {
  std::vector<std::vector<size_t>> widths;
  std::vector<size_t> nsib;
};
struct InputGather {
  std::function<void(const u64* d_indices, size_t nq)> queue;
  std::function<void(const std::vector<uint64_t>& indices, size_t qbytes, uint8_t* out)> fetch;
};
void add_gather_seg(std::vector<GatherSeg>& segs, size_t& out_off, const void* base, u64 stride, uint32_t count, uint32_t kind,
                    uint32_t shift, uint32_t flip) {
  GatherSeg q;
  q.base = base;
  q.stride = stride;
  q.count = count;
  q.kind = kind;
  q.shift = shift;
  q.flip = flip;
  q.out_off = out_off;
  segs.push_back(q);
  out_off += kind == 0 || kind == 3 ? size_t(count) * 8 : kind == 1 ? 32 : 16;
}
struct FriHead {
  unsigned n_rounds = 0;
  unsigned log_max_height = 0;
  std::vector<std::vector<Digest>> commits;
  std::vector<u64> pow;
  std::vector<size_t> nsib;
  bool on_device = false;
  DBuf<uint32_t> d_state;
  DBuf<FriTailRound> d_recs;
  size_t qbytes() const {
    size_t b = 0;
    for (size_t n : nsib) b += 16 + 32 * n;
    return b;
  }
};
void fri_prove(HSystem& sys, Challenger& ch, std::vector<DBuf<E2>>& inputs, unsigned log_gmax, const std::vector<GatherSeg>& input_segs,
               size_t input_qbytes, const InputShape& shape, const InputGather* remote, PW& fri_bytes, PhaseTrace& tr,
               FriHead* head = nullptr, DTree* round0 = nullptr);

void pcs_open(HSystem& sys, std::vector<OpenRound>& rounds, Challenger& ch, std::vector<OpenedRound>& opened, PW& fri_bytes,
              const SymbolicPoints* sym = nullptr) {
  Ctx& ctx = *sys.ctx;
  const Params& prm = sys.params;
  const unsigned lb = (unsigned)prm.log_blowup;
  size_t gmax = 0, gw = 0;
  for (auto& r : rounds)
    for (auto& m : r.data->ldes) {
      gmax = std::max(gmax, m.h);
      gw = std::max(gw, m.w);
    }
  if (!gmax) throw std::runtime_error("pcs_open: no matrices");
  const unsigned log_gmax = log2_strict(gmax);
  PhaseTrace tr(ctx);

  const bool allow_next = !getenv("MSAMD_NO_NEXT_SHIFT");
  std::vector<std::vector<char>> is_next(rounds.size());
  for (size_t ri = 0; ri < rounds.size(); ri++) {
    auto& r = rounds[ri];
    is_next[ri].assign(r.data->ldes.size(), 0);
    for (size_t mi = 0; allow_next && mi < r.data->ldes.size(); mi++) {
      auto& pts = r.points[mi];
      const unsigned lh = log2_strict(r.data->ldes[mi].h);
// ... 511 lines not shown
  }
  tr.mark("fri_commit_phase");
  g_probes.mark("FRI rounds replayed");
  const bool host_trace = getenv("MSAMD_TRACE_HOST") != nullptr;
  const double t_sync = host_trace ? now_ms() : 0;
  if (fin.size() != stop) throw std::runtime_error("FRI: unexpected final length");
  std::vector<E2> final_poly(final_len);
  {
    unsigned lf = (unsigned)prm.log_final_poly_len;
    std::vector<E2> ev(final_len);
    for (size_t i = 0; i < final_len; i++) ev[bitrev64(i, lf)] = fin[i];
    u64 winv = gl_inv(gl_two_adic_generator(lf)), ninv = gl_inv((u64)final_len);
    for (size_t k = 0; k < final_len; k++) {
      E2 s = e2(0);
      u64 wk = gl_pow(winv, k), cur = 1;
      for (size_t j = 0; j < final_len; j++) {
        s = e2_add(s, e2_mul_base(ev[j], cur));
        cur = gl_mul(cur, wk);
      }
      final_poly[k] = e2_mul_base(s, ninv);
      ch.observe_ext(final_poly[k]);
    }
  }
  u64 query_pow = 0;
  std::vector<uint64_t> indices(nq);
  if (dev_query) {
    query_pow = dq[0];
    if (prm.query_pow_bits) {
      ch.observe(query_pow);
      if (ch.sample_bits((unsigned)prm.query_pow_bits) != 0) throw std::runtime_error("FRI: device query witness rejected by the host challenger");
    }
    for (size_t i = 0; i < nq; i++) {
      indices[i] = ch.sample_bits(log_max_height);
      if (indices[i] != dq[1 + i]) throw std::runtime_error("FRI: device query indices diverged from the host transcript");
    }
    tr.mark("final_poly+grind+gather");
    g_probes.mark("query indices replayed");
  } else {
    query_pow = grind(ctx, ch, (unsigned)prm.query_pow_bits);
    for (auto& ix : indices) ix = ch.sample_bits(log_max_height);
    tr.mark("final_poly+grind");
    if (g_vec.size() < qbytes * nq) g_vec.resize(qbytes * nq);
    gather_queries(ctx, segs, indices, qbytes, g_vec.data());
    g = g_vec.data();
    tr.mark("query_gather");
  }

  std::vector<uint8_t> input_g;
  const size_t remote_qbytes = input_qbytes + (head ? head->qbytes() : 0);
  if (remote) {
    input_g.resize(remote_qbytes * nq);
    remote->fetch(indices, remote_qbytes, input_g.data());
    tr.mark("remote_input_openings");
  }

  PW& w = fri_bytes;
  w.b.reserve(w.b.size() + nq * (qbytes + remote_qbytes + 64 * (trees.size() + head_rounds + shape.widths.size() * 4 + 8)) + 4096);
  w.u64_(commits.size() + head_rounds);
  if (head)
    for (auto& c : head->commits) w.cap(c);
  for (auto& c : commits) w.cap(c);
  w.u64_(pow_w.size() + head_rounds);
  if (head)
    for (u64 x : head->pow) w.u64_(x);
  for (u64 x : pow_w) w.u64_(x);
  w.u64_(indices.size());
  size_t pos = 0;
  for (size_t qi = 0; qi < indices.size(); qi++) {
    const uint8_t* ip = remote ? &input_g[qi * remote_qbytes] : &g[pos];
    w.u64_(shape.widths.size());
    for (size_t ri = 0; ri < shape.widths.size(); ri++) {
      w.u64_(shape.widths[ri].size());
      for (size_t mw : shape.widths[ri]) {
        w.u64_(mw);
        w.raw(ip, mw * 8);
        ip += mw * 8;
      }
      const size_t ns = shape.nsib[ri];
      w.u64_(ns);
      w.raw(ip, ns * 32);
      ip += ns * 32;
    }
    if (!remote) pos += input_qbytes;
    w.u64_(trees.size() + head_rounds);
    for (unsigned hr = 0; hr < head_rounds; hr++) {
      w.u8(1);
      w.u64_(1);
      w.raw(ip, 16);
      ip += 16;
      w.u64_(head->nsib[hr]);
      w.raw(ip, head->nsib[hr] * 32);
      ip += head->nsib[hr] * 32;
    }
    uint64_t index_i = indices[qi] >> head_rounds;
    for (size_t i = 0; i < trees.size(); i++) {
      const unsigned la = arities[i];
      w.u8((uint8_t)la);
      w.u64_((size_t(1) << la) - 1);
      if (la == 1) {
        w.raw(&g[pos], 16);
        pos += 16;
      } else {
        const size_t own = index_i & ((size_t(1) << la) - 1);
        w.raw(&g[pos], own * 16);
        w.raw(&g[pos + (own + 1) * 16], ((size_t(1) << la) - 1 - own) * 16);
        pos += size_t(16) << la;
      }
      index_i >>= la;
      size_t ns = n_siblings(trees[i]);
      w.u64_(ns);
      w.raw(&g[pos], ns * 32);
      pos += ns * 32;
    }
  }
  w.u64_(final_poly.size());
  for (auto& e : final_poly) w.ext(e);
  w.u64_(query_pow);
  g_probes.mark("FriProof bytes written");
  if (host_trace) fprintf(stderr, "[msamd] host work after the FRI read-back: %.1f us (transcript replay + FriProof bytes)\n", 1e3 * (now_ms() - t_sync));
}
}

void stage2_circuit_dyn(Ctx& ctx, const HSystem& sys, const HWitness& wit, size_t ci, const ChallengeBG* bg, u64* out, E2* total_dev) {
  const HCircuit& c = sys.circuits[ci];
  const DLookups& lk = wit.lookups[ci];
  if (c.num_lookups && !lk.mult.p) {
    if (!c.stage2_trace_jit.function || !wit.traces[ci].p) throw std::runtime_error("stage 2: this circuit has neither lookup values nor a fused kernel");
    stage2_from_trace_dyn(ctx, c.stage2_trace_jit, wit.traces[ci].p, c.pre_width ? c.d_preprocessed.p : nullptr, wit.heights[ci], c.num_lookups,
                          c.args_width, bg, out, total_dev);
    return;
  }
  stage2_build_dyn(ctx, lk, bg, out, total_dev, &c.stage2_jit);
}
void stage2_circuit_async(Ctx& ctx, const HSystem& sys, const HWitness& wit, size_t ci, E2 beta, E2 gamma, u64* out, E2* total_dev) {
  DBuf<ChallengeBG> bg = challenge_bg_upload(ctx, beta, gamma);
  stage2_circuit_dyn(ctx, sys, wit, ci, bg.p, out, total_dev);
}

void observe_claims(Ctx& ctx, Challenger& ch, HWitness& wit) {
  const size_t n_claims = wit.claim_offsets.size() - 1;
  const size_t claim_elems = wit.claim_data.size();
  const size_t claim_words = 1 + n_claims + claim_elems;
  if (claim_words <= 8192) {
    ch.observe((u64)n_claims);
    for (size_t i = 0; i < n_claims; i++) {
      size_t a = wit.claim_offsets[i], b = wit.claim_offsets[i + 1];
      ch.observe((u64)(b - a));
      for (size_t k = a; k < b; k++) ch.observe(wit.claim_data[k]);
    }
    return;
  }
  DBuf<uint8_t> d_prefix(ctx, ch.input.size());
  ctx.h2d(d_prefix.p, ch.input.data(), ch.input.size());
  DBuf<u64> d_words(ctx, claim_words);
  claims_transcript_words(ctx, wit.d_claim_data.p, wit.d_claim_offsets.p, n_claims, claim_elems, d_words.p);
  Digest d = blake3_device(ctx, d_prefix.p, ch.input.size(), d_words.p, claim_words);
  ch.flush_with(d);
}

std::vector<uint8_t> prove(HSystem& sys, HWitness& wit, StageMs* times) {
  Ctx& ctx = *sys.ctx;
  HIP_CHECK(hipSetDevice(ctx.device));
  const Params& prm = sys.params;
  const unsigned lb = (unsigned)prm.log_blowup;
  const size_t C = sys.circuits.size();
  if (wit.sys != &sys || wit.heights.size() != C) throw std::runtime_error("witness does not belong to this system");
  if (wit.has_remote) throw std::runtime_error("this witness lacks traces that another rank computes: use ms_prove_sharded");
  double t_begin = now_ms(), t0;
  g_probes.start();
  auto lap = [&](int slot) {
    if (times) {
      ctx.sync();
      times->v[slot] = now_ms() - t0;
    }
  };

  RoctxRange whole("stark/prove");
  HostUpload up(wit, ctx);
  up.start();
  g_probes.mark("uploads issued");
  Challenger ch(sys.seed);
  ch.observe((u64)C);
  for (auto& c : sys.circuits) {
    ch.observe((u64)c.constraint_count);
    ch.observe((u64)c.max_constraint_degree);
    ch.observe((u64)c.pre_height);
    ch.observe((u64)c.pre_width);
    ch.observe((u64)c.main_width);
    ch.observe((u64)c.stage2_width);
  }
  std::vector<uint8_t> active(C);
  std::vector<size_t> aidx;
  std::vector<int> apos(C, -1);
  for (size_t i = 0; i < C; i++) {
    active[i] = wit.heights[i] > 0;
    ch.observe(active[i] ? 1 : 0);
    if (active[i]) {
      apos[i] = (int)aidx.size();
      aidx.push_back(i);
    }
  }
  if (aidx.empty()) throw std::runtime_error("cannot prove with every circuit deactivated (all traces empty)");
  const size_t NA = aidx.size();
  std::vector<unsigned> log_degrees;
  for (size_t ci : aidx) log_degrees.push_back(log2_strict(wit.heights[ci]));
  std::vector<char> on_side(NA, 0);
  std::vector<size_t> order;
  ctx.side_config();
  {
    bool any_long = false, any_short = false;
    for (size_t pos = 0; pos < NA; pos++) (log_degrees[pos] <= ctx.side_max_log ? any_short : any_long) = true;
    const bool use_side = ctx.side_enabled && any_long && any_short;
    for (size_t pos = 0; pos < NA; pos++) on_side[pos] = use_side && log_degrees[pos] <= ctx.side_max_log;
    for (int pass = 0; pass < 2; pass++)
      for (size_t pos = 0; pos < NA; pos++)
        if ((int)on_side[pos] == pass) order.push_back(pos);
  }
  const bool use_side = order.size() && on_side[order.back()];
  struct SideSession {
    Ctx& c;
    ~SideSession() { c.side_join(); }
  } side_session{ctx};
  auto fork_side = [&]() {
    if (use_side && !ctx.side_forked) ctx.side_fork();
  };

  const size_t n_claims = wit.claim_offsets.size() - 1;
  const size_t claim_elems = wit.claim_data.size();
  const size_t claim_words = 1 + n_claims + claim_elems;
  const bool device_claims = claim_words > 8192;
  const bool early_claims = device_claims && ctx.side_enabled;
  size_t max_lde_log = 0;
  for (unsigned ld : log_degrees) max_lde_log = std::max<size_t>(max_lde_log, ld + lb);
  const size_t ncap = size_t(1) << std::min<size_t>((size_t)prm.cap_height, max_lde_log);
  std::vector<Digest> s1_cap;
  size_t cap_off = 0, prefix_chunks = 0, nchunks = 0;
  DBuf<u64> d_words;
  DBuf<Digest> d_cvs;
  const bool dev_outer = device_claims && outer_fits(ncap, NA) && !getenv("MSAMD_HOST_TRANSCRIPT");
  OuterDev od;
  DBuf<ChallengeBG> d_bg;
  if (device_claims) {
    s1_cap.assign(ncap, Digest());
    if (sys.has_pre) ch.observe_cap(sys.pre_commit);
    cap_off = ch.input.size();
    ch.observe_cap(s1_cap);
    for (unsigned ld : log_degrees) ch.observe(ld);
    nchunks = blake3_num_chunks(ch.input.size(), claim_words);
    prefix_chunks = std::min(nchunks, (ch.input.size() + 1023) / 1024);
  }
  const bool late_chunk0 = device_claims && prefix_chunks == 1 && nchunks >= 2 && !getenv("MSAMD_OLD_CLAIMS_TREE");
  LateChunk0 late0;
  DBuf<uint8_t> d_prefix;
  auto claims_chunks = [&]() {
    up.wait_claims();
    d_words = DBuf<u64>(ctx, claim_words);
    claims_transcript_words(ctx, wit.d_claim_data.p, wit.d_claim_offsets.p, n_claims, claim_elems, d_words.p);
    d_cvs = DBuf<Digest>(ctx, nchunks);
    blake3_chunk_cvs(ctx, nullptr, ch.input.size(), d_words.p, claim_words, prefix_chunks, nchunks, d_cvs.p);
    d_prefix = DBuf<uint8_t>(ctx, ch.input.size());
    ctx.h2d(d_prefix.p, ch.input.data(), ch.input.size());
    if (late_chunk0) blake3_late_chunk0_prepare(ctx, d_cvs.p, nchunks, late0);
  };

  t0 = now_ms();
  RoctxRange phase("stark/stage1_commit");
  PcsData s1;
  {
    std::vector<DMat> ldes(NA);
    up.wait_traces();
    fork_side();
    for (size_t pos : order) {
      const size_t ci = aidx[pos];
      SideScope sc(ctx, on_side[pos]);
      ldes[pos] = lde_of_host_matrix(ctx, wit.traces[ci].p, wit.heights[ci], sys.circuits[ci].main_width, lb);
    }
    ctx.side_join();
    if (early_claims) {
      ctx.side_fork();
      SideScope sc(ctx, true);
      claims_chunks();
    }
    commit_matrices(ctx, std::move(ldes), (unsigned)prm.cap_height, s1);
  }
  g_probes.mark("stage 1 queued");
  up.wait_claims();
  if (!device_claims) {
    s1_cap = merkle_cap(ctx, s1.tree);
    lap(0);
    if (sys.has_pre) ch.observe_cap(sys.pre_commit);
    ch.observe_cap(s1_cap);
    for (unsigned ld : log_degrees) ch.observe(ld);
    ch.observe((u64)n_claims);
    for (size_t i = 0; i < n_claims; i++) {
      size_t a = wit.claim_offsets[i], b = wit.claim_offsets[i + 1];
      ch.observe((u64)(b - a));
      for (size_t k = a; k < b; k++) ch.observe(wit.claim_data[k]);
    }
  } else {
    lap(0);
    const size_t cl = s1.tree.cap_layer();
    if (s1.tree.layer_len[cl] != ncap) throw std::runtime_error("stage-1 cap size differs from the transcript's placeholder");
    const Digest* d_cap = s1.tree.base() + s1.tree.layer_off[cl];
    if (!early_claims) claims_chunks();
    ctx.side_join();
    od.digest = DBuf<Digest>(ctx, 1);
    if (dev_outer) {
      od.state = DBuf<u32>(ctx, 28);
      d_bg = DBuf<ChallengeBG>(ctx, 1);
    }
    if (late_chunk0) {
      blake3_late_chunk0_finish(ctx, d_prefix.p, ch.input.size(), d_words.p, claim_words, d_cap, cap_off, ncap, late0, nchunks, od.digest.p,
                                dev_outer ? d_bg.p : nullptr, dev_outer ? od.state.p : nullptr);
    } else {
      HIP_CHECK(hipMemcpyAsync(d_prefix.p + cap_off, d_cap, ncap * sizeof(Digest), hipMemcpyDeviceToDevice, ctx.stream));
      blake3_chunk_cvs(ctx, d_prefix.p, ch.input.size(), d_words.p, claim_words, 0, prefix_chunks, d_cvs.p);
      blake3_from_cvs_async(ctx, d_cvs.p, nchunks, od.digest.p);
    }
    ctx.d2h_queue(s1_cap.data(), d_cap, ncap * sizeof(Digest));
    if (dev_outer) {
      if (!late_chunk0) outer_beta_gamma(ctx, od.digest.p, d_bg.p, od.state.p);
      ctx.d2h_queue(&od.h_digest, od.digest.p, sizeof(Digest));
      ctx.d2h_queue(od.h_bg, d_bg.p, 2 * sizeof(E2));
      g_probes.mark("claims digest + beta/gamma queued");
    } else {
      Digest d;
      ctx.d2h(&d, od.digest.p, sizeof(Digest));
      g_probes.mark("sync 1 (cap + claims digest)");
      ch.flush_with(d);
    }
    d_words.reset();
    d_cvs.reset();
    late0.reset();
    d_prefix.reset();
  }
  E2 beta = e2(0), gamma = e2(0), alpha = e2(0), zeta = e2(0);
  if (!dev_outer) {
    tx_beta_gamma(ch, beta, gamma);
    d_bg = challenge_bg_upload(ctx, beta, gamma);
  }
  DBuf<E2> d_tot(ctx, NA + 1);
  std::vector<E2> h_tot(NA + 1);
  const bool claims_on_device = n_claims > 256 || dev_outer;
  const bool claims_beside = claims_on_device && ctx.side_enabled && !getenv("MSAMD_CLAIMS_ACC_MAIN");
  auto claims_sum_launch = [&]() {
    if (claims_beside && !ctx.side_forked) ctx.side_fork();
    SideScope sc(ctx, claims_beside);
    claims_accumulator_dyn(ctx, wit.d_claim_data.p, wit.d_claim_offsets.p, n_claims, d_bg.p, d_tot.p);
  };
  if (claims_on_device) {
    if (!claims_beside) claims_sum_launch();
  } else {
    E2 acc0 = e2(0);
    for (size_t i = 0; i < n_claims; i++) {
      E2 f = e2(0);
      for (size_t k = wit.claim_offsets[i + 1]; k-- > wit.claim_offsets[i];) f = e2_add(e2_mul(f, gamma), e2(wit.claim_data[k]));
      acc0 = e2_add(acc0, e2_inv(e2_add(beta, f)));
    }
    ctx.h2d(d_tot.p, &acc0, sizeof(E2));
  }

  t0 = now_ms();
  phase.next("stark/lookup_construction");
  up.lookup_values();
  std::vector<DBuf<u64>> s2_evals(NA);
  fork_side();
  for (size_t pos : order) {
    size_t ci = aidx[pos];
    const HCircuit& c = sys.circuits[ci];
    size_t n = wit.heights[ci];
    SideScope sc(ctx, on_side[pos]);
    s2_evals[pos] = DBuf<u64>(ctx, n * c.stage2_width);
    stage2_circuit_dyn(ctx, sys, wit, ci, d_bg.p, s2_evals[pos].p, d_tot.p + 1 + pos);
  }
  if (claims_beside) claims_sum_launch();
  lap(1);
  t0 = now_ms();
  phase.next("stark/stage2_commit");
  PcsData s2;
  {
    std::vector<DMat> ldes(NA);
    fork_side();
    for (size_t pos : order) {
      const HCircuit& c = sys.circuits[aidx[pos]];
      size_t n = wit.heights[aidx[pos]];
      SideScope sc(ctx, on_side[pos]);
      DMat lde;
      lde.h = n << lb;
      lde.w = c.stage2_width;
      lde.buf = DBuf<u64>(ctx, lde.h * lde.w);
      coset_lde(ctx, s2_evals[pos].p, lde.d(), log_degrees[pos], lb, lde.w);
      s2_evals[pos].reset();
      ldes[pos] = std::move(lde);
    }
    ctx.side_join();
    commit_matrices(ctx, std::move(ldes), (unsigned)prm.cap_height, s2);
  }
  ctx.d2h_queue(h_tot.data(), d_tot.p, (NA + 1) * sizeof(E2));
  g_probes.mark("stage 2 queued");
  auto dev_cap = [&](const DTree& t) -> const Digest* {
    const size_t cl = t.cap_layer();
    if (t.layer_len[cl] != ncap) throw std::runtime_error("a commitment's cap size differs from the stage-1 cap");
    return t.base() + t.layer_off[cl];
  };
  std::vector<Digest> s2_cap, q_cap;
  E2 acc_initial = e2(0);
  std::vector<E2> accs;
  auto host_alpha = [&]() {
    acc_initial = h_tot[0];
    accs.clear();
    E2 acc = acc_initial;
    for (size_t pos = 0; pos < NA; pos++) {
      acc = e2_add(acc, h_tot[1 + pos]);
      accs.push_back(acc);
    }
    alpha = tx_alpha(ch, s2_cap, accs);
  };
  if (dev_outer) {
    s2_cap.assign(ncap, Digest());
    accs.assign(NA, e2(0));
    const Digest* d_cap = dev_cap(s2.tree);
    ctx.d2h_queue(s2_cap.data(), d_cap, ncap * sizeof(Digest));
    od.accs = DBuf<E2>(ctx, NA + 1);
    od.alpha = DBuf<E2>(ctx, 1);
    od.qdyn.resize(NA);
    std::vector<OuterTarget> targets(NA);
    for (size_t pos = 0; pos < NA; pos++) {
      const size_t k = sys.circuits[aidx[pos]].prog.constraint_count;
      od.qdyn[pos] = DBuf<uint8_t>(ctx, sizeof(QDyn) + std::max<size_t>(k, 1) * sizeof(E2));
      targets[pos].dyn = reinterpret_cast<QDyn*>(od.qdyn[pos].p);
      targets[pos].alpha_rev = reinterpret_cast<E2*>(od.qdyn[pos].p + sizeof(QDyn));
      targets[pos].log_n = log_degrees[pos];
      targets[pos].k = k;
    }
    outer_alpha(ctx, od.state.p, d_cap, ncap, d_tot.p, NA, d_bg.p, targets, od.accs.p, od.alpha.p, od.state.p + 12, od.circuits);
    ctx.d2h_queue(&od.h_alpha, od.alpha.p, sizeof(E2));
    lap(2);
  } else {
    s2_cap = merkle_cap(ctx, s2.tree);
    g_probes.mark("sync 2 (stage-2 cap)");
    lap(2);
    host_alpha();
  }

  t0 = now_ms();
  phase.next("stark/quotient");
  PcsData qd;
  {
    std::vector<DMat> qldes(NA);
    fork_side();
    for (size_t pos : order) {
      size_t ci = aidx[pos];
      const HCircuit& c = sys.circuits[ci];
      SideScope sc(ctx, on_side[pos]);
      unsigned log_n = log_degrees[pos], log_q = log2_strict(c.quotient_degree());
      size_t n = size_t(1) << log_n, nq = n << log_q;
      QuotientArgs qa = fill_quotient_args(sys, ci, s1.ldes[pos], s2.ldes[pos], log_n, log_q, dev_outer ? od.qdyn[pos].p : nullptr);
      if (!dev_outer) quotient_publics(qa, beta, gamma, pos ? accs[pos - 1] : acc_initial, accs[pos], alpha);
      DBuf<u64> qv(ctx, nq * 2);
      quotient_eval(ctx, c.prog, qa, qv.p);
      DMat lde;
      lde.h = n << lb;
      lde.w = 2 << log_q;
      lde.buf = DBuf<u64>(ctx, lde.h * lde.w);
      quotient_lde(ctx, qv.p, lde.d(), log_n, log_q, lb, 2);
      qldes[pos] = std::move(lde);
    }
    ctx.side_join();
    commit_matrices(ctx, std::move(qldes), (unsigned)prm.cap_height, qd);
  }
  g_probes.mark("quotient queued");
  E2 pt_zeta = e2(0);
  std::vector<E2> pt_next(NA);
  SymbolicPoints sym;
  if (dev_outer) {
    q_cap.assign(ncap, Digest());
    const Digest* d_cap = dev_cap(qd.tree);
    ctx.d2h_queue(q_cap.data(), d_cap, ncap * sizeof(Digest));
    zeta_placeholders(ctx, od, log_degrees, d_cap, ncap, od.state.p + 20, pt_zeta, pt_next);
    const size_t n_ld = od.uniq_ld.size();
    sym.d_points = od.points.p;
    sym.n = 1 + n_ld;
    sym.next_log.assign(1 + n_ld, -1);
    for (size_t k = 0; k < n_ld; k++) sym.next_log[1 + k] = (int)od.uniq_ld[k];
    lap(3);
    t0 = now_ms();
    phase.next("stark/fri_open");
  } else {
    q_cap = merkle_cap(ctx, qd.tree);
    g_probes.mark("sync 3 (quotient cap)");
    lap(3);
    t0 = now_ms();
    phase.next("stark/fri_open");
    zeta = tx_zeta(ch, q_cap);
    pt_zeta = zeta;
    for (size_t pos = 0; pos < NA; pos++) pt_next[pos] = e2_mul_base(zeta, gl_two_adic_generator(log_degrees[pos]));
  }
  std::vector<OpenRound> rounds(3);
  rounds[0].data = &s1;
  rounds[1].data = &s2;
  rounds[2].data = &qd;
  for (size_t pos = 0; pos < NA; pos++) {
    rounds[0].points.push_back({pt_zeta, pt_next[pos]});
    rounds[1].points.push_back({pt_zeta, pt_next[pos]});
    rounds[2].points.push_back({pt_zeta});
  }
  if (sys.has_pre) {
    OpenRound r0;
    r0.data = &sys.pre_data;
    for (size_t ci = 0; ci < C; ci++) {
      if (sys.pre_indices[ci] < 0) continue;
      if (apos[ci] >= 0) {
        r0.points.push_back({pt_zeta, pt_next[apos[ci]]});
      } else {
        r0.points.push_back({});
      }
    }
    rounds.push_back(std::move(r0));
  }
  PW w;
  {
    size_t vals = 0;
    for (size_t pos = 0; pos < NA; pos++) {
      const HCircuit& c = sys.circuits[aidx[pos]];
      vals += 2 * (c.main_width + c.stage2_width + c.pre_width + 2) + 2 * c.quotient_degree() + 16;
    }
    w.b.reserve(16 * vals + 64 * (NA + 8) + 32 * (s1_cap.size() + s2_cap.size() + q_cap.size()) + 8192);
  }
  auto write_header = [&](PW& h) {
    h.u64_(C);
    for (auto a : active) h.u8(a);
    h.cap(s1_cap);
    h.cap(s2_cap);
    h.cap(q_cap);
    h.u64_(accs.size());
    for (auto& a : accs) h.ext(a);
    h.u64_(log_degrees.size());
    for (unsigned ld : log_degrees) h.u8((uint8_t)ld);
  };
  write_header(w);
  const size_t header_len = w.b.size();
  sym.resolve = [&](std::vector<E2>& values) {
    ch.flush_with(od.h_digest);
    tx_beta_gamma(ch, beta, gamma);
    host_alpha();
    zeta = tx_zeta(ch, q_cap);
    values = replayed_points(od, beta, gamma, alpha, zeta);
    PW h;
    write_header(h);
    if (h.b.size() != header_len) throw std::runtime_error("proof header changed length");
    memcpy(w.b.data(), h.b.data(), header_len);
    g_probes.mark("transcript replayed");
  };
  std::vector<OpenedRound> opened;
  pcs_open(sys, rounds, ch, opened, w, dev_outer ? &sym : nullptr);
  lap(4);
  write_round(w, opened[2]);
  w.u8(sys.has_pre ? 1 : 0);
  if (sys.has_pre) write_round(w, opened[3]);
  write_round(w, opened[0]);
  write_round(w, opened[1]);
  ctx.prof_collect();
  if (times) times->v[5] = now_ms() - t_begin;
  g_probes.mark("proof bytes complete");
  g_probes.print();
  if (getenv("MSAMD_TRACE_HOST")) fprintf(stderr, "[msamd] prove(): %.1f us in all\n", 1e3 * (now_ms() - t_begin));
  return std::move(w.b);
}

#include "prover_sharded.inc"

void pcs_open_standalone(Ctx& ctx, const Params& prm, const std::vector<PcsData*>& data, const std::vector<std::vector<std::vector<E2>>>& points,
                         Challenger& ch, std::vector<E2>& opened_flat, std::vector<uint8_t>& fri_bytes) {
  HIP_CHECK(hipSetDevice(ctx.device));
  HSystem sys;
  sys.ctx = &ctx;
  sys.params = prm;
  if (prm.max_log_arity < 1 || prm.max_log_arity > FRI_MAX_LOG_ARITY) throw std::runtime_error("max_log_arity must be 1 .. 6 (a FRI row is hashed as one BLAKE3 chunk)");
  if (prm.log_blowup < 1 || prm.log_blowup > 8) throw std::runtime_error("log_blowup out of range");
  if (prm.commit_pow_bits > 40 || prm.query_pow_bits > 40) throw std::runtime_error("proof-of-work bits out of range");
  std::vector<OpenRound> rounds;
  for (size_t r = 0; r < data.size(); r++) {
    if (points[r].size() != data[r]->ldes.size()) throw std::runtime_error("pcs_open: one list of points per matrix expected");
    for (auto& m : data[r]->ldes)
      if (log2_strict(m.h) < prm.log_blowup) throw std::runtime_error("pcs_open: a committed matrix is shorter than the blowup");
    rounds.push_back(OpenRound{data[r], points[r]});
  }
  std::vector<OpenedRound> opened;
  PW fri;
  pcs_open(sys, rounds, ch, opened, fri);
  opened_flat.clear();
  for (auto& orr : opened)
    for (auto& m : orr)
      for (auto& pt : m) opened_flat.insert(opened_flat.end(), pt.begin(), pt.end());
  fri_bytes = std::move(fri.b);
  ctx.sync();
}

}
```

Measured before the change: 162.9 million rows/s.

## Hash claims directly from offsets/data without materializing transcript words; reschedule claims on side stream

Adds a ClaimsSrc source that lets the BLAKE3 chunk kernels read claim transcript words straight from claim offsets and data, with a search and a sequential walker. This removes the separate claims_transcript_words kernel and its buffer. It also changes the stage-1 schedule so the claims chunk hashing runs on the side stream concurrently with the trace LDEs, using a new side_pass instead of a full join. The cost is extra index arithmetic and a binary search inside the hash kernels. It also adds a test C API and probe timing.

```diff
diff --git a/bindings/rust/mstark_sys.rs b/bindings/rust/mstark_sys.rs
--- a/bindings/rust/mstark_sys.rs
+++ b/bindings/rust/mstark_sys.rs
@@ -147,6 +147,8 @@
                                 n_openings: usize, indices: *const u64, vals: *const u64, siblings: *const u8, ok_out: *mut u8) -> i32;
     pub fn ms_mmcs_destroy(m: *mut ms_mmcs);
     pub fn ms_blake3(ctx: *mut ms_ctx, bytes: *const u8, len: usize, out32: *mut u8) -> i32;
+    pub fn ms_blake3_claims(ctx: *mut ms_ctx, prefix: *const u8, prefix_len: usize, n_claims: usize, offsets: *const u64, data: *const u64,
+                            mode: i32, out32: *mut u8) -> i32;
     pub fn ms_challenger_create(params7: *const u64, out: *mut *mut ms_challenger) -> i32;
     pub fn ms_challenger_destroy(ch: *mut ms_challenger);
     pub fn ms_challenger_observe(ch: *mut ms_challenger, elems: *const u64, n: usize) -> i32;
diff --git a/include/mstark.h b/include/mstark.h
--- a/include/mstark.h
+++ b/include/mstark.h
@@ -160,6 +160,8 @@
                              uint32_t cap_height, size_t n_openings, const uint64_t* indices, const uint64_t* vals,
                              const uint8_t* siblings, uint8_t* ok_out);
 int32_t ms_blake3(ms_ctx* ctx, const uint8_t* bytes, size_t len, uint8_t out32[32]);
+int32_t ms_blake3_claims(ms_ctx* ctx, const uint8_t* prefix, size_t prefix_len, size_t n_claims, const uint64_t* offsets,
+                         const uint64_t* data, int32_t mode, uint8_t out32[32]);
 
 typedef struct ms_challenger ms_challenger;
 int32_t ms_challenger_create(const uint64_t params7[7], ms_challenger** out);
diff --git a/multi-stark_amd/__init__.py b/multi-stark_amd/__init__.py
--- a/multi-stark_amd/__init__.py
+++ b/multi-stark_amd/__init__.py
@@ -38,7 +38,7 @@
             "ms_witness_create_device", "ms_witness_u32_add_bench", "ms_witness_blake3_compressions", "ms_blake3_compressions", "ms_witness_trace", "ms_witness_destroy", "ms_prove", "ms_prove_sharded", "ms_ctx_comm_progress", "ms_comm_rccl_unique_id", "ms_comm_rccl_create",
             "ms_comm_rccl_table", "ms_comm_rccl_bytes_moved", "ms_comm_rccl_destroy", "ms_comm_local_group_create", "ms_comm_local_group_abort",
             "ms_comm_local_group_destroy", "ms_comm_local_create", "ms_comm_local_table", "ms_comm_local_bytes_moved", "ms_comm_local_destroy", "ms_verify", "ms_verify_batch", "ms_dft_batch", "ms_coset_lde_batch", "ms_quotient_lde", "ms_mmcs_commit",
-            "ms_mmcs_open", "ms_mmcs_destroy", "ms_mmcs_verify_batch", "ms_blake3", "ms_pcs_commit", "ms_pcs_open", "ms_pcs_verify", "ms_challenger_create",
+            "ms_mmcs_open", "ms_mmcs_destroy", "ms_mmcs_verify_batch", "ms_blake3", "ms_blake3_claims", "ms_pcs_commit", "ms_pcs_open", "ms_pcs_verify", "ms_challenger_create",
             "ms_challenger_destroy", "ms_challenger_observe", "ms_challenger_observe_digests", "ms_challenger_sample_ext",
             "ms_challenger_sample_bits", "ms_stage2_trace", "ms_claims_accumulator",
             "ms_quotient_values", "ms_field_op", "ms_trace_destroy", "ms_trace_info", "ms_system_preprocessed_mmcs",
@@ -232,6 +232,18 @@
         _check(lib().ms_blake3(self.h, _b(buf), C.c_size_t(len(data)), _b(out)))
         return out.tobytes()
 
+    def blake3_claims(self, prefix: bytes, offsets, data, mode=0) -> bytes:
+        pre = np.frombuffer(prefix, dtype=np.uint8) if prefix else np.zeros(1, dtype=np.uint8)
+        offs = np.ascontiguousarray(offsets, dtype=np.uint64)
+        dat = np.ascontiguousarray(data, dtype=np.uint64)
+        if dat.size == 0:
+            dat = np.zeros(1, dtype=np.uint64)
+        out = np.zeros(32, dtype=np.uint8)
+        u64p = C.POINTER(C.c_uint64)
+        _check(lib().ms_blake3_claims(self.h, _b(pre), C.c_size_t(len(prefix)), C.c_size_t(offs.size - 1), offs.ctypes.data_as(u64p),
+                                      dat.ctypes.data_as(u64p), C.c_int32(mode), _b(out)))
+        return out.tobytes()
+
     def stage2_trace(self, mult, arg_offsets, args, beta, gamma, acc_in):
         mult, args, arg_offsets = _u64(mult), _u64(args), _u64(arg_offsets)
         h, L = mult.shape
diff --git a/multi-stark_amd/csrc/capi.hip b/multi-stark_amd/csrc/capi.hip
--- a/multi-stark_amd/csrc/capi.hip
+++ b/multi-stark_amd/csrc/capi.hip
@@ -996,6 +996,44 @@
   MS_CATCH
 }
 
+int32_t ms_blake3_claims(ms_ctx* c, const uint8_t* prefix, size_t prefix_len, size_t n_claims, const uint64_t* offsets, const uint64_t* data,
+                         int32_t mode, uint8_t out32[32]) {
+  MS_TRY Ctx& ctx = c->ctx;
+  HIP_CHECK(hipSetDevice(ctx.device));
+  if (!offsets || !out32 || (prefix_len && !prefix) || mode < 0 || mode > 2) throw std::runtime_error("ms_blake3_claims: bad argument");
+  if (offsets[0] != 0) throw std::runtime_error("claim offsets must start at 0");
+  for (size_t i = 0; i < n_claims; i++)
+    if (offsets[i + 1] < offsets[i]) throw std::runtime_error("claim offsets must be non-decreasing");
+  const size_t elems = (size_t)offsets[n_claims];
+  if (elems && !data) throw std::runtime_error("ms_blake3_claims: null data");
+  DBuf<uint8_t> pre(ctx, std::max<size_t>(prefix_len, 1));
+  DBuf<u64> d_offs(ctx, n_claims + 1), d_data(ctx, std::max<size_t>(elems, 1));
+  if (prefix_len) ctx.h2d(pre.p, prefix, prefix_len);
+  ctx.h2d(d_offs.p, offsets, (n_claims + 1) * 8);
+  if (elems) ctx.h2d(d_data.p, data, elems * 8);
+  const ClaimStream cl{d_data.p, d_offs.p, n_claims, elems};
+  Digest d;
+  if (mode == 2) {
+    DBuf<u64> words(ctx, cl.nwords());
+    claims_transcript_words(ctx, d_data.p, d_offs.p, n_claims, elems, words.p);
+    d = blake3_device(ctx, pre.p, prefix_len, words.p, cl.nwords());
+  } else if (mode == 1) {
+    const size_t nchunks = blake3_num_chunks(prefix_len, cl.nwords());
+    if (prefix_len > 1024 || nchunks < 2) throw std::runtime_error("ms_blake3_claims: mode 1 needs the prefix inside chunk 0 and two chunks or more");
+    DBuf<Digest> cvs(ctx, nchunks), out(ctx, 1);
+    LateChunk0 late;
+    blake3_chunk_cvs(ctx, pre.p, prefix_len, cl, 1, nchunks, cvs.p);
+    blake3_late_chunk0_prepare(ctx, cvs.p, nchunks, late);
+    blake3_late_chunk0_finish(ctx, pre.p, prefix_len, cl, nullptr, 0, 0, late, nchunks, out.p);
+    ctx.d2h(&d, out.p, sizeof(Digest));
+  } else {
+    d = blake3_device(ctx, pre.p, prefix_len, cl);
+  }
+  memcpy(out32, d.b, 32);
+  return MS_OK;
+  MS_CATCH
+}
+
 int32_t ms_stage2_trace(ms_ctx* c, size_t height, size_t L, const uint64_t* mult, const uint64_t* arg_offsets,
                         const uint64_t* args, const uint64_t beta[2], const uint64_t gamma[2], const uint64_t acc_in[2],
                         uint64_t* trace_out, uint64_t acc_out[2]) {
diff --git a/multi-stark_amd/csrc/ctx.hip b/multi-stark_amd/csrc/ctx.hip
--- a/multi-stark_amd/csrc/ctx.hip
+++ b/multi-stark_amd/csrc/ctx.hip
@@ -439,6 +439,12 @@
   }
   for (auto& kv : side_deferred) pool_free_side.emplace(kv.first, kv.second);
   side_deferred.clear();
+}
+
+void Ctx::side_pass() {
+  if (!side_forked) return;
+  HIP_CHECK(hipEventRecord(side_ev[2], side_stream));
+  HIP_CHECK(hipStreamWaitEvent(main_stream, side_ev[2], 0));
 }
 
 namespace {
diff --git a/multi-stark_amd/csrc/hash.hip b/multi-stark_amd/csrc/hash.hip
--- a/multi-stark_amd/csrc/hash.hip
+++ b/multi-stark_amd/csrc/hash.hip
@@ -549,14 +549,120 @@
   }
 }
 
-__device__ __forceinline__ u32 stream_byte(const uint8_t* __restrict__ prefix, size_t pl, const u64* __restrict__ words, size_t p) {
+struct WordsSrc {
+  const u64* words;
+  size_t nwords;
+  __device__ __forceinline__ u64 word(size_t q) const { return q < nwords ? words[q] : 0; }
+  struct Walk {
+    const u64* w;
+    size_t left;
+    __device__ __forceinline__ u64 next() {
+      if (!left) return 0;
+      left--;
+      return *w++;
+    }
+  };
+  __device__ __forceinline__ Walk walk(size_t q) const { return Walk{words + q, q < nwords ? nwords - q : 0}; }
+  __device__ __forceinline__ void stage(size_t q0, u32 nw, u64* lds, u32 lane) const {
+    for (u32 j = lane; j < nw; j += 64) lds[j] = word(q0 + j);
+  }
+};
+
+struct ClaimsSrc {
+  const u64* data;
+  const u64* offs;
+  size_t n, nwords;
+  __device__ __forceinline__ size_t pos(size_t i) const { return 1 + i + (size_t)offs[i]; }
+  __device__ size_t find(size_t q) const {
+    size_t lo = 0, hi = n - 1;
+    size_t g = (size_t)((double)(q - 1) * (double)n / (double)(nwords - 1));
+    if (g > hi) g = hi;
+    if (pos(g) <= q) {
+      if (g == hi || pos(g + 1) > q) return g;
+      lo = g + 1;
+    } else {
+      if (pos(g - 1) <= q) return g - 1;
+      hi = g - 1;
+    }
+    while (lo < hi) {
+      const size_t mid = lo + (hi - lo + 1) / 2;
+      if (pos(mid) <= q)
+        lo = mid;
+      else
+        hi = mid - 1;
+    }
+    return lo;
+  }
+  __device__ u64 word(size_t q) const {
+    if (q >= nwords) return 0;
+    if (q == 0) return (u64)n;
+    const size_t i = find(q), o = (size_t)offs[i], st = 1 + i + o;
+    return q == st ? offs[i + 1] - (u64)o : data[o + (q - st - 1)];
+  }
+  struct Walk {
+    const u64* data;
+    const u64* offs;
+    size_t n, nwords;
+    size_t q, i, start, nxt, nxt2;
+    __device__ __forceinline__ u64 next() {
+      u64 x = 0;
+      if (q < nwords) {
+        if (q == 0)
+          x = (u64)n;
+        else if (q == start)
+          x = (u64)(nxt - start - 1);
+        else
+          x = data[(start - 1 - i) + (q - start - 1)];
+      }
+      q++;
+      if (q == nxt && i + 1 < n) {
+        i++;
+        start = nxt;
+        nxt = nxt2;
+        nxt2 = i + 2 <= n ? 1 + (i + 2) + (size_t)offs[i + 2] : ~size_t(0);
+      }
+      return x;
+    }
+  };
+  __device__ Walk walk(size_t q) const {
+    Walk w{data, offs, n, nwords, q, 0, 1, ~size_t(0), ~size_t(0)};
+    if (n == 0) return w;
+    if (q >= 1 && q < nwords) w.i = find(q);
+    w.start = pos(w.i);
+    w.nxt = pos(w.i + 1);
+    if (w.i + 2 <= n) w.nxt2 = pos(w.i + 2);
+    return w;
+  }
+  __device__ void stage(size_t q0, u32 nw, u64* lds, u32 lane) const {
+    const size_t qe = q0 + nw < nwords ? q0 + nw : nwords;
+    for (u32 j = lane; j < nw; j += 64)
+      if (q0 + j >= qe) lds[j] = 0;
+    if (q0 >= qe) return;
+    if (q0 == 0 && lane == 0) lds[0] = (u64)n;
+    if (n == 0) return;
+    const size_t i0 = q0 >= 1 ? find(q0) : 0;
+    for (size_t i = i0 + lane; i < n; i += 64) {
+      const size_t o = (size_t)offs[i], st = 1 + i + o;
+      if (st >= qe) break;
+      const size_t len = (size_t)offs[i + 1] - o;
+      if (st >= q0) lds[st - q0] = (u64)len;
+      size_t k0 = q0 > st + 1 ? q0 - st - 1 : 0;
+      size_t k1 = qe - st - 1 < len ? qe - st - 1 : len;
+      for (size_t k = k0; k < k1; k++) lds[st + 1 + k - q0] = data[o + k];
+    }
+  }
+};
+constexpr u32 STAGE_WORDS = 129;
+
+__device__ __forceinline__ u32 staged_byte(const uint8_t* __restrict__ prefix, size_t pl, const u64* lds, size_t q0, size_t p) {
   if (p < pl) return prefix[p];
-  size_t q = p - pl;
-  return (u32)((words[q >> 3] >> (8 * (q & 7))) & 0xff);
-}
-
-__global__ __launch_bounds__(256) void chunk_cv_k(const uint8_t* __restrict__ prefix, size_t pl, const u64* __restrict__ words,
-                                                  size_t len, size_t nchunks, size_t c0, size_t c1, Digest* out) {
+  const size_t q = p - pl;
+  return (u32)((lds[(q >> 3) - q0] >> (8 * (q & 7))) & 0xff);
+}
+
+template <class Src>
+__global__ __launch_bounds__(256) void chunk_cv_k(const uint8_t* __restrict__ prefix, size_t pl, Src src, size_t len, size_t nchunks, size_t c0,
+                                                  size_t c1, Digest* out) {
   size_t ch = c0 + blockIdx.x * size_t(blockDim.x) + threadIdx.x;
   if (ch >= c1) return;
   size_t off = ch * 1024;
@@ -565,23 +671,23 @@
   u32 cv[8];
   b3_iv(cv);
   const bool single = nchunks == 1;
+  const bool behind = off >= pl;
+  typename Src::Walk wk = src.walk(behind ? (off - pl) >> 3 : 0);
+  const unsigned s = behind ? (unsigned)((off - pl) & 7) * 8 : 0;
+  u64 cur = behind ? wk.next() : 0;
   for (u32 b = 0; b < nblocks; b++) {
     u32 m[16];
     size_t boff = off + size_t(b) * 64;
     u32 bl = (u32)(clen - size_t(b) * 64 < 64 ? clen - size_t(b) * 64 : 64);
-    if (bl == 64 && boff >= pl) {
-      size_t q = boff - pl;
-      const u64* w = words + (q >> 3);
-      unsigned s = (unsigned)(q & 7) * 8;
-      u64 cur = w[0];
+    if (behind) {
 #pragma unroll
       for (int k = 0; k < 8; k++) {
         u64 x;
         if (s == 0) {
           x = cur;
-          if (k < 7) cur = w[k + 1];
+          if (k < 7 || b + 1 < nblocks) cur = wk.next();
         } else {
-          u64 nxt = w[k + 1];
+          u64 nxt = wk.next();
           x = (cur >> s) | (nxt << (64 - s));
           cur = nxt;
         }
@@ -594,7 +700,11 @@
         u32 wv = 0;
         for (int k = 0; k < 4; k++) {
           u32 idx = 4 * i + k;
-          u32 byte = idx < bl ? stream_byte(prefix, pl, words, boff + idx) : 0;
+          u32 byte = 0;
+          if (idx < bl) {
+            const size_t p = boff + idx;
+            byte = p < pl ? prefix[p] : (u32)((src.word((p - pl) >> 3) >> (8 * ((p - pl) & 7))) & 0xff);
+          }
           wv |= byte << (8 * k);
         }
         m[i] = wv;
@@ -606,18 +716,23 @@
   store_digest(out + ch, cv);
 }
 
-__global__ __launch_bounds__(64) void chunk_cv_prefix_k(const uint8_t* __restrict__ prefix, size_t pl, const u64* __restrict__ words,
-                                                        size_t len, size_t nchunks, size_t c0, Digest* out) {
+template <class Src>
+__global__ __launch_bounds__(64) void chunk_cv_prefix_k(const uint8_t* __restrict__ prefix, size_t pl, Src src, size_t len, size_t nchunks,
+                                                        size_t c0, Digest* out) {
   __shared__ u32 sh[256];
+  __shared__ u64 wd[STAGE_WORDS];
   const size_t ch = c0 + blockIdx.x;
   const size_t off = ch * 1024;
   const size_t clen = len - off < 1024 ? len - off : 1024;
+  const size_t q0 = off > pl ? (off - pl) >> 3 : 0;
+  src.stage(q0, STAGE_WORDS, wd, threadIdx.x);
+  __syncthreads();
   for (u32 i = threadIdx.x; i < 256; i += 64) {
     u32 wv = 0;
 #pragma unroll
     for (u32 k = 0; k < 4; k++) {
       const u32 idx = 4 * i + k;
-      const u32 byte = idx < clen ? stream_byte(prefix, pl, words, off + idx) : 0;
+      const u32 byte = idx < clen ? staged_byte(prefix, pl, wd, q0, off + idx) : 0;
       wv |= byte << (8 * k);
     }
     sh[i] = wv;
@@ -981,25 +1096,34 @@
   return len == 0 ? 1 : (len + 1023) / 1024;
 }
 
-void blake3_chunk_cvs(Ctx& ctx, const uint8_t* d_prefix, size_t prefix_len, const u64* d_words, size_t nwords, size_t c0, size_t c1,
-                      Digest* cvs) {
+template <class Src>
+static void chunk_cvs_launch(Ctx& ctx, const uint8_t* d_prefix, size_t prefix_len, Src src, size_t c0, size_t c1, Digest* cvs) {
+  const size_t nwords = src.nwords;
   const size_t len = prefix_len + 8 * nwords, nchunks = blake3_num_chunks(prefix_len, nwords);
   if (c1 > nchunks) c1 = nchunks;
   if (c0 >= c1) return;
   const size_t pc = std::min(c1, (prefix_len + 1023) / 1024);
   if (c0 < pc) {
-    hipLaunchKernelGGL(chunk_cv_prefix_k, dim3((unsigned)(pc - c0)), dim3(64), 0, ctx.stream, d_prefix, prefix_len, d_words, len, nchunks, c0, cvs);
+    hipLaunchKernelGGL(chunk_cv_prefix_k<Src>, dim3((unsigned)(pc - c0)), dim3(64), 0, ctx.stream, d_prefix, prefix_len, src, len, nchunks, c0, cvs);
     c0 = pc;
   }
   if (c0 < c1)
-    hipLaunchKernelGGL(chunk_cv_k, dim3((unsigned)((c1 - c0 + 255) / 256)), dim3(256), 0, ctx.stream, d_prefix, prefix_len, d_words, len,
-                       nchunks, c0, c1, cvs);
+    hipLaunchKernelGGL(chunk_cv_k<Src>, dim3((unsigned)((c1 - c0 + 255) / 256)), dim3(256), 0, ctx.stream, d_prefix, prefix_len, src, len, nchunks,
+                       c0, c1, cvs);
   HIP_CHECK(hipGetLastError());
 }
-
+void blake3_chunk_cvs(Ctx& ctx, const uint8_t* d_prefix, size_t prefix_len, const u64* d_words, size_t nwords, size_t c0, size_t c1,
+                      Digest* cvs) {
+  chunk_cvs_launch(ctx, d_prefix, prefix_len, WordsSrc{d_words, nwords}, c0, c1, cvs);
+}
+void blake3_chunk_cvs(Ctx& ctx, const uint8_t* d_prefix, size_t prefix_len, const ClaimStream& cl, size_t c0, size_t c1, Digest* cvs) {
+  chunk_cvs_launch(ctx, d_prefix, prefix_len, ClaimsSrc{cl.data, cl.offs, cl.n, cl.nwords()}, c0, c1, cvs);
+}
+
+template <class Src>
 struct ClaimsRootArgs {
   const uint8_t* prefix;
-  const u64* words;
+  Src src;
   size_t pl, len;
   const u32* cap;
   u32 cap_off, cap_bytes;
@@ -1009,11 +1133,15 @@
   ChallengeBG* bg;
   u32* state_out;
 };
-__global__ __launch_bounds__(64) void claims_root_k(ClaimsRootArgs a) {
+template <class Src>
+__global__ __launch_bounds__(64) void claims_root_k(ClaimsRootArgs<Src> a) {
   __shared__ u32 sh[256];
   __shared__ u32 pm[16];
+  __shared__ u64 wd[STAGE_WORDS];
   const u32 t = threadIdx.x, c = t & 3;
   const u32 clen = a.len < 1024 ? (u32)a.len : 1024u;
+  a.src.stage(0, STAGE_WORDS, wd, t);
+  __syncthreads();
   for (u32 i = t; i < 256; i += 64) {
     u32 wv = 0;
 #pragma unroll
@@ -1025,7 +1153,7 @@
           const u32 q = idx - a.cap_off;
           byte = (a.cap[q >> 2] >> (8 * (q & 3))) & 0xff;
         } else {
-          byte = stream_byte(a.prefix, a.pl, a.words, idx);
+          byte = staged_byte(a.prefix, a.pl, wd, 0, idx);
         }
       }
       wv |= byte << (8 * k);
@@ -1126,16 +1254,16 @@
   HIP_CHECK(hipGetLastError());
   if (lc.sib.size() > 32) throw std::runtime_error("blake3_late_chunk0: too many levels");
 }
-void blake3_late_chunk0_finish(Ctx& ctx, const uint8_t* d_prefix, size_t prefix_len, const u64* d_words, size_t nwords, const Digest* d_cap,
-                               size_t cap_off, size_t ncap, const LateChunk0& lc, size_t nchunks, Digest* out_dev, ChallengeBG* d_bg,
-                               u32* d_state12) {
+template <class Src>
+static void late_chunk0_finish(Ctx& ctx, const uint8_t* d_prefix, size_t prefix_len, Src src, const Digest* d_cap, size_t cap_off, size_t ncap,
+                               const LateChunk0& lc, size_t nchunks, Digest* out_dev, ChallengeBG* d_bg, u32* d_state12) {
   if (prefix_len > 1024 || cap_off + 32 * ncap > prefix_len) throw std::runtime_error("blake3_late_chunk0: the prefix must lie inside chunk 0");
-  ClaimsRootArgs a;
+  ClaimsRootArgs<Src> a;
   memset(&a, 0, sizeof(a));
   a.prefix = d_prefix;
-  a.words = d_words;
+  a.src = src;
   a.pl = prefix_len;
-  a.len = prefix_len + 8 * nwords;
+  a.len = prefix_len + 8 * src.nwords;
   a.cap = reinterpret_cast<const u32*>(d_cap);
   a.cap_off = (u32)cap_off;
   a.cap_bytes = (u32)(32 * ncap);
@@ -1147,8 +1275,18 @@
   a.out = out_dev;
   a.bg = d_bg;
   a.state_out = d_state12;
-  hipLaunchKernelGGL(claims_root_k, dim3(1), dim3(64), 0, ctx.stream, a);
+  hipLaunchKernelGGL(claims_root_k<Src>, dim3(1), dim3(64), 0, ctx.stream, a);
   HIP_CHECK(hipGetLastError());
+}
+void blake3_late_chunk0_finish(Ctx& ctx, const uint8_t* d_prefix, size_t prefix_len, const u64* d_words, size_t nwords, const Digest* d_cap,
+                               size_t cap_off, size_t ncap, const LateChunk0& lc, size_t nchunks, Digest* out_dev, ChallengeBG* d_bg,
+                               u32* d_state12) {
+  late_chunk0_finish(ctx, d_prefix, prefix_len, WordsSrc{d_words, nwords}, d_cap, cap_off, ncap, lc, nchunks, out_dev, d_bg, d_state12);
+}
+void blake3_late_chunk0_finish(Ctx& ctx, const uint8_t* d_prefix, size_t prefix_len, const ClaimStream& cl, const Digest* d_cap, size_t cap_off,
+                               size_t ncap, const LateChunk0& lc, size_t nchunks, Digest* out_dev, ChallengeBG* d_bg, u32* d_state12) {
+  late_chunk0_finish(ctx, d_prefix, prefix_len, ClaimsSrc{cl.data, cl.offs, cl.n, cl.nwords()}, d_cap, cap_off, ncap, lc, nchunks, out_dev, d_bg,
+                     d_state12);
 }
 
 Digest blake3_device(Ctx& ctx, const uint8_t* d_prefix, size_t prefix_len, const u64* d_words, size_t nwords) {
@@ -1157,5 +1295,11 @@
   blake3_chunk_cvs(ctx, d_prefix, prefix_len, d_words, nwords, 0, nchunks, a.p);
   return blake3_from_cvs(ctx, a.p, nchunks);
 }
-
-}
+Digest blake3_device(Ctx& ctx, const uint8_t* d_prefix, size_t prefix_len, const ClaimStream& cl) {
+  const size_t nchunks = blake3_num_chunks(prefix_len, cl.nwords());
+  DBuf<Digest> a(ctx, nchunks);
+  blake3_chunk_cvs(ctx, d_prefix, prefix_len, cl, 0, nchunks, a.p);
+  return blake3_from_cvs(ctx, a.p, nchunks);
+}
+
+}
diff --git a/multi-stark_amd/csrc/msamd.h b/multi-stark_amd/csrc/msamd.h
--- a/multi-stark_amd/csrc/msamd.h
+++ b/multi-stark_amd/csrc/msamd.h
@@ -63,7 +63,7 @@
   hipStream_t copy_stream = nullptr;
   hipStream_t claims_stream = nullptr;
   hipStream_t main_stream = nullptr, side_stream = nullptr;
-  hipEvent_t side_ev[2] = {nullptr, nullptr};
+  hipEvent_t side_ev[3] = {nullptr, nullptr, nullptr};
   bool side_forked = false;
   int side_depth = 0;
   bool side_enabled = true;
@@ -74,6 +74,7 @@
   void side_config();
   void side_fork();
   void side_join();
+  void side_pass();
   unsigned side_delay_us = 0, main_delay_us = 0;
   unsigned copy_delay_us = 0;
   void copy_delay();
@@ -250,6 +251,14 @@
 size_t blake3_num_chunks(size_t prefix_len, size_t nwords);
 void blake3_chunk_cvs(Ctx& ctx, const uint8_t* d_prefix, size_t prefix_len, const u64* d_words, size_t nwords, size_t c0, size_t c1,
                       Digest* cvs);
+struct ClaimStream {
+  const u64* data;
+  const u64* offs;
+  size_t n, elems;
+  size_t nwords() const { return 1 + n + elems; }
+};
+void blake3_chunk_cvs(Ctx& ctx, const uint8_t* d_prefix, size_t prefix_len, const ClaimStream& claims, size_t c0, size_t c1, Digest* cvs);
+Digest blake3_device(Ctx& ctx, const uint8_t* d_prefix, size_t prefix_len, const ClaimStream& claims);
 Digest blake3_from_cvs(Ctx& ctx, Digest* cvs, size_t nchunks);
 void blake3_from_cvs_async(Ctx& ctx, Digest* cvs, size_t nchunks, Digest* out_dev);
 struct ChallengeBG;
@@ -266,6 +275,9 @@
                                size_t cap_off, size_t ncap, const LateChunk0& lc, size_t nchunks, Digest* out_dev,
                                ChallengeBG* d_bg = nullptr ,
                                u32* d_state12 = nullptr);
+void blake3_late_chunk0_finish(Ctx& ctx, const uint8_t* d_prefix, size_t prefix_len, const ClaimStream& claims, const Digest* d_cap,
+                               size_t cap_off, size_t ncap, const LateChunk0& lc, size_t nchunks, Digest* out_dev,
+                               ChallengeBG* d_bg = nullptr, u32* d_state12 = nullptr);
 
 struct JitKernel;
 struct DLookups {
diff --git a/multi-stark_amd/csrc/prover.hip b/multi-stark_amd/csrc/prover.hip
--- a/multi-stark_amd/csrc/prover.hip
+++ b/multi-stark_amd/csrc/prover.hip
@@ -861,7 +861,34 @@
   Ctx& ctx;
   bool on = false;
   bool skip_claims = false;
+  hipEvent_t t_tree = nullptr, t_claims = nullptr;
   HostUpload(HWitness& wit, Ctx& c) : w(wit), ctx(c) {}
+  void plain_copy(void* dst, const void* src, size_t bytes, hipStream_t s) {
+    if (w.pinned)
+      HIP_CHECK(hipMemcpyAsync(dst, src, bytes, hipMemcpyHostToDevice, s));
+    else
+      ctx.bounce_h2d(dst, src, bytes, s);
+  }
+  void claims_arrived(HWitness::Staged& st) {
+    HIP_CHECK(hipEventRecord(st.ev[2], ctx.copy_stream));
+    if (g_probes.on) {
+      if (!t_claims) HIP_CHECK(hipEventCreate(&t_claims));
+      HIP_CHECK(hipEventRecord(t_claims, ctx.copy_stream));
+    }
+  }
+  void mark_tree_start() {
+    if (!on || !g_probes.on) return;
+    if (!t_tree) HIP_CHECK(hipEventCreate(&t_tree));
+    HIP_CHECK(hipEventRecord(t_tree, ctx.stream));
+  }
+  void report_claims_arrival() {
+    if (!t_tree || !t_claims) return;
+    float ms = 0;
+    if (hipEventSynchronize(t_claims) == hipSuccess && hipEventSynchronize(t_tree) == hipSuccess &&
+        hipEventElapsedTime(&ms, t_tree, t_claims) == hipSuccess)
+      fprintf(stderr, "[msamd]   claims on the device (ev[2]) %+.1f us against the start of the stage-1 tree\n", 1e3 * ms);
+    (void)hipGetLastError();
+  }
   bool fused(size_t ci) const {
     const HCircuit& c = w.sys->circuits[ci];
     return w.host_resident && c.stage2_trace_jit.function && w.h_mult[ci].empty();
@@ -881,12 +908,7 @@
     ctx.copy_delay();
     HIP_CHECK(hipStreamWaitEvent(ctx.claims_stream, ctx.copy_ev[3], 0));
     const size_t n_claims = w.claim_offsets.size() - 1, tot = w.claim_data.size();
-    auto from_caller = [&](void* dst, const void* src, size_t bytes, hipStream_t s) {
-      if (w.pinned)
-        HIP_CHECK(hipMemcpyAsync(dst, src, bytes, hipMemcpyHostToDevice, s));
-      else
-        ctx.bounce_h2d(dst, src, bytes, s);
-    };
+    auto from_caller = [&](void* dst, const void* src, size_t bytes, hipStream_t s) { plain_copy(dst, src, bytes, s); };
     for (size_t ci = 0; ci < C; ci++) {
       const HCircuit& c = sys.circuits[ci];
       const size_t h = w.heights[ci];
@@ -934,7 +956,7 @@
       from_caller(st.claim_offsets.p, w.claim_offsets.data(), (n_claims + 1) * 8, ctx.copy_stream);
       if (tot) from_caller(st.claim_data.p, w.claim_data.data(), tot * 8, ctx.copy_stream);
     }
-    HIP_CHECK(hipEventRecord(st.ev[2], ctx.copy_stream));
+    claims_arrived(st);
     for (size_t ci = 0; ci < C; ci++) {
       const HCircuit& c = sys.circuits[ci];
       const size_t h = w.heights[ci];
@@ -976,6 +998,8 @@
     if (on) HIP_CHECK(hipStreamWaitEvent(ctx.stream, w.stage[w.cur].ev[2], 0));
   }
   ~HostUpload() {
+    if (t_tree) (void)hipEventDestroy(t_tree);
+    if (t_claims) (void)hipEventDestroy(t_claims);
     if (!on) return;
     (void)hipStreamSynchronize(ctx.copy_stream);
     (void)hipStreamSynchronize(ctx.claims_stream);
@@ -1793,9 +1817,7 @@
   }
   DBuf<uint8_t> d_prefix(ctx, ch.input.size());
   ctx.h2d(d_prefix.p, ch.input.data(), ch.input.size());
-  DBuf<u64> d_words(ctx, claim_words);
-  claims_transcript_words(ctx, wit.d_claim_data.p, wit.d_claim_offsets.p, n_claims, claim_elems, d_words.p);
-  Digest d = blake3_device(ctx, d_prefix.p, ch.input.size(), d_words.p, claim_words);
+  Digest d = blake3_device(ctx, d_prefix.p, ch.input.size(), ClaimStream{wit.d_claim_data.p, wit.d_claim_offsets.p, n_claims, claim_elems});
   ch.flush_with(d);
 }
 
@@ -1893,12 +1915,18 @@
   const bool late_chunk0 = device_claims && prefix_chunks == 1 && nchunks >= 2 && !getenv("MSAMD_OLD_CLAIMS_TREE");
   LateChunk0 late0;
   DBuf<uint8_t> d_prefix;
+  const bool claims_as_words = getenv("MSAMD_CLAIMS_WORDS") != nullptr;
+  const ClaimStream claim_stream{wit.d_claim_data.p, wit.d_claim_offsets.p, n_claims, claim_elems};
   auto claims_chunks = [&]() {
     up.wait_claims();
-    d_words = DBuf<u64>(ctx, claim_words);
-    claims_transcript_words(ctx, wit.d_claim_data.p, wit.d_claim_offsets.p, n_claims, claim_elems, d_words.p);
     d_cvs = DBuf<Digest>(ctx, nchunks);
-    blake3_chunk_cvs(ctx, nullptr, ch.input.size(), d_words.p, claim_words, prefix_chunks, nchunks, d_cvs.p);
+    if (claims_as_words) {
+      d_words = DBuf<u64>(ctx, claim_words);
+      claims_transcript_words(ctx, wit.d_claim_data.p, wit.d_claim_offsets.p, n_claims, claim_elems, d_words.p);
+      blake3_chunk_cvs(ctx, nullptr, ch.input.size(), d_words.p, claim_words, prefix_chunks, nchunks, d_cvs.p);
+    } else {
+      blake3_chunk_cvs(ctx, nullptr, ch.input.size(), claim_stream, prefix_chunks, nchunks, d_cvs.p);
+    }
     d_prefix = DBuf<uint8_t>(ctx, ch.input.size());
     ctx.h2d(d_prefix.p, ch.input.data(), ch.input.size());
     if (late_chunk0) blake3_late_chunk0_prepare(ctx, d_cvs.p, nchunks, late0);
@@ -1910,18 +1938,33 @@
   {
     std::vector<DMat> ldes(NA);
     up.wait_traces();
-    fork_side();
+    const bool fork_late = getenv("MSAMD_CLAIMS_FORK_LATE") != nullptr;
+    if (early_claims && !fork_late)
+      ctx.side_fork();
+    else
+      fork_side();
+    if (early_claims && !fork_late && !up.on) {
+      SideScope sc(ctx, true);
+      claims_chunks();
+    }
     for (size_t pos : order) {
       const size_t ci = aidx[pos];
       SideScope sc(ctx, on_side[pos]);
       ldes[pos] = lde_of_host_matrix(ctx, wit.traces[ci].p, wit.heights[ci], sys.circuits[ci].main_width, lb);
     }
-    ctx.side_join();
-    if (early_claims) {
+    if (early_claims && !fork_late && up.on) {
+      ctx.side_pass();
+      SideScope sc(ctx, true);
+      claims_chunks();
+    } else {
+      ctx.side_join();
+    }
+    if (early_claims && fork_late) {
       ctx.side_fork();
       SideScope sc(ctx, true);
       claims_chunks();
     }
+    up.mark_tree_start();
     commit_matrices(ctx, std::move(ldes), (unsigned)prm.cap_height, s1);
   }
   g_probes.mark("stage 1 queued");
@@ -1951,11 +1994,18 @@
       d_bg = DBuf<ChallengeBG>(ctx, 1);
     }
     if (late_chunk0) {
-      blake3_late_chunk0_finish(ctx, d_prefix.p, ch.input.size(), d_words.p, claim_words, d_cap, cap_off, ncap, late0, nchunks, od.digest.p,
-                                dev_outer ? d_bg.p : nullptr, dev_outer ? od.state.p : nullptr);
+      if (claims_as_words)
+        blake3_late_chunk0_finish(ctx, d_prefix.p, ch.input.size(), d_words.p, claim_words, d_cap, cap_off, ncap, late0, nchunks, od.digest.p,
+                                  dev_outer ? d_bg.p : nullptr, dev_outer ? od.state.p : nullptr);
+      else
+        blake3_late_chunk0_finish(ctx, d_prefix.p, ch.input.size(), claim_stream, d_cap, cap_off, ncap, late0, nchunks, od.digest.p,
+                                  dev_outer ? d_bg.p : nullptr, dev_outer ? od.state.p : nullptr);
     } else {
       HIP_CHECK(hipMemcpyAsync(d_prefix.p + cap_off, d_cap, ncap * sizeof(Digest), hipMemcpyDeviceToDevice, ctx.stream));
-      blake3_chunk_cvs(ctx, d_prefix.p, ch.input.size(), d_words.p, claim_words, 0, prefix_chunks, d_cvs.p);
+      if (claims_as_words)
+        blake3_chunk_cvs(ctx, d_prefix.p, ch.input.size(), d_words.p, claim_words, 0, prefix_chunks, d_cvs.p);
+      else
+        blake3_chunk_cvs(ctx, d_prefix.p, ch.input.size(), claim_stream, 0, prefix_chunks, d_cvs.p);
       blake3_from_cvs_async(ctx, d_cvs.p, nchunks, od.digest.p);
     }
     ctx.d2h_queue(s1_cap.data(), d_cap, ncap * sizeof(Digest));
@@ -2205,6 +2255,7 @@
   if (times) times->v[5] = now_ms() - t_begin;
   g_probes.mark("proof bytes complete");
   g_probes.print();
+  up.report_claims_arrival();
   if (getenv("MSAMD_TRACE_HOST")) fprintf(stderr, "[msamd] prove(): %.1f us in all\n", 1e3 * (now_ms() - t_begin));
   return std::move(w.b);
 }
```

After: 156.4 million rows/s. 4.0% lower.
